# graphic-goose/ferreus_rbf_rs

Hardware: AMD Instinct MI355X
Metric: BBFMM matvecs/s (higher is better)
Workload: dtype f64; 1 GPU; 10000000 uniform 3D points, LinearRbf, order 7, 1 rhs, adaptive sparse tree, ACA eps=1e-7, set_weights + evaluate at the sources; points=10000000, kernel=LinearRbf, order=7, nrhs=1, parallelism=single GPU

## Files before the change

ferreus_rbf_rs_amd/_lib.py:

```python
from __future__ import annotations

import ctypes
import os

HERE = os.path.dirname(os.path.abspath(__file__))
LIB_PATH = os.environ.get("FERREUS_BBFMM_HIP_LIB") or os.path.join(HERE, "libferreus_bbfmm_hip.so")

OK, POINT_OUTSIDE_TREE, KERNEL_NO_GRADIENTS, BAD_ARGUMENT, DEVICE_ERROR, UNSUPPORTED, CALLBACK_FAILED = range(7)
FLAG_HOST_ONLY = 1
FLAG_M2L_SHARED_BASIS = 2
FLAG_DIRECT_SMALL_W_LEAVES = 4
FLAG_DETERMINISTIC = 8
N_PHASES = 11
PHASE_NAMES = ["gather", "P2M", "M2M", "M2L_stage1", "M2L_stage2", "P2L", "L2L", "P2P", "M2P",
               "L2P", "scatter"]

c_i32, c_i64, c_f64, c_u32 = ctypes.c_int32, ctypes.c_int64, ctypes.c_double, ctypes.c_uint32
c_p = ctypes.c_void_p


class Params(ctypes.Structure):
    _fields_ = [("max_points_per_cell", c_i64), ("compression_type", c_i32),
                ("epsilon", c_f64), ("eval_chunk_size", c_i64)]

# ... 69 lines not shown
    "bbfmm_isosurface_count": (c_i32, [c_p]),
    "bbfmm_isosurface_size": (ctypes.c_int, [c_p, c_i32, c_p, c_p]),
    "bbfmm_isosurface_copy": (ctypes.c_int, [c_p, c_i32, c_p, c_p]),
    "bbfmm_isosurface_error": (ctypes.c_char_p, [c_p]),
    "bbfmm_isosurface_destroy": (None, [c_p]),
    "bbfmm_prepare_target_subset": (ctypes.c_int, [c_p, c_p, c_i64]),
    "bbfmm_fast_matrix_vector_product": (ctypes.c_int, [c_p, c_p, c_i64, c_i64, c_p, c_i64, c_p,
                                                        c_i64, c_f64, c_p]),
    "bbfmm_matvec_device": (ctypes.c_int, [c_p, c_p, c_i64, c_i32, c_p, c_i64, c_i32]),
    "bbfmm_target_subset_create": (ctypes.c_int, [c_p, c_p, c_i64, c_p]),
    "bbfmm_matvec_subset_device": (ctypes.c_int, [c_p, c_i32, c_p, c_p, c_i32]),
    "bbfmm_stream": (c_p, [c_p]),
    "bbfmm_set_partition": (ctypes.c_int, [c_p, c_i32, c_i32]),
    "bbfmm_partition_row_count": (c_i64, [c_p]),
    "bbfmm_partition_rows": (ctypes.c_int, [c_p, c_p]),
    "bbfmm_partition_coarse_count": (c_i64, [c_p]),
    "bbfmm_matvec_partition_upward": (ctypes.c_int, [c_p, c_p, c_i64, c_i32, c_p, c_p]),
    "bbfmm_matvec_partition_finish": (ctypes.c_int, [c_p, c_p, c_p, c_i64, c_i32, c_p]),
    "bbfmm_partition_world": (c_i32, [c_p]),
    "bbfmm_partition_rank": (c_i32, [c_p]),
    "bbfmm_partition_bounds": (ctypes.c_int, [c_p, c_i32, c_p]),
    "bbfmm_matvec_partition_finish_sorted": (ctypes.c_int, [c_p, c_p, c_p, c_i64, c_p]),
    "bbfmm_partition_scatter": (ctypes.c_int, [c_p, c_p, c_i32, c_i32, c_i64, c_i32, c_p, c_i64]),
    "bbfmm_debug_partition_upward_counts": (ctypes.c_int, [c_p, c_p, c_p, c_p]),
    "bbfmm_debug_host_copy_rates": (ctypes.c_int, [c_i64, c_p]),
    "bbfmm_get_tree_stats": (ctypes.c_int, [c_p, c_p]),
    "bbfmm_tree_built_on_device": (ctypes.c_int, [c_p]),
    "bbfmm_last_evaluate_at_sources": (ctypes.c_int, [c_p]),
    "bbfmm_debug_targets_are_sources": (ctypes.c_int, [c_p, c_p, c_i64, c_i64]),
    "bbfmm_debug_rows_of_sources": (ctypes.c_int, [c_p, c_p, c_i64, c_i64, c_p]),
    "bbfmm_get_cells": (ctypes.c_int, [c_p, c_p, c_p]),
    "bbfmm_get_leaf_sources": (ctypes.c_int, [c_p, c_p, c_p]),
    "bbfmm_get_list": (ctypes.c_int, [c_p, ctypes.c_char, c_p, c_p, c_p]),
    "bbfmm_get_m2l_ranks": (ctypes.c_int, [c_p, c_p, c_p]),
    "bbfmm_get_m2l_operator": (ctypes.c_int, [c_p, c_i32, c_i32, c_p]),
    "bbfmm_get_m2l_factors": (ctypes.c_int, [c_p, c_i32, c_i32, c_p, c_p]),
    "bbfmm_get_permutation_tables": (ctypes.c_int, [c_p, c_p, c_p, c_p, c_p, c_p]),
    "bbfmm_points_to_leaves": (ctypes.c_int, [c_p, c_p, c_i64, c_i64, c_p, c_p]),
    "bbfmm_set_profiling": (ctypes.c_int, [c_p, c_i32]),
    "bbfmm_get_phase_ms": (ctypes.c_int, [c_p, c_p, c_p]),
    "bbfmm_reset_phase_ms": (ctypes.c_int, [c_p]),
    "bbfmm_mfma_f64_selftest": (ctypes.c_int, [c_p, c_p, c_p]),
    "bbfmm_fp64_valu_selftest": (ctypes.c_int, [c_p, c_p]),
    "bbfmm_debug_kernel_values": (ctypes.c_int, [c_i32, c_i32, ctypes.c_double, ctypes.c_double, c_p, c_i64, c_p, c_p, c_p]),
    "bbfmm_debug_math": (ctypes.c_int, [c_i32, c_i32, c_p, c_i64, c_p, c_p]),
    "bbfmm_debug_dense_m2m": (ctypes.c_int, [c_p, c_i32, c_p]),
    "bbfmm_debug_apply_m2l_tables_host": (ctypes.c_int, [c_p, c_p, c_p]),
    "bbfmm_debug_m2l_variants": (ctypes.c_int, [c_p, c_p, c_p]),
    "bbfmm_debug_m2l_pairs": (ctypes.c_int, [c_p, c_p, c_i64, c_p, c_p]),
    "bbfmm_debug_m2l_pairs_axes": (ctypes.c_int, [c_p, c_p, c_i64, c_p]),
    "bbfmm_debug_m2l_pairs_stage2": (ctypes.c_int, [c_p, c_p, c_i64, c_p, c_p]),
    "bbfmm_debug_m2l_pairs_axes_stage2": (ctypes.c_int, [c_p, c_p, c_i64, c_p]),
    "bbfmm_debug_m2l_s2_last_ksplit": (ctypes.c_int, [c_p, c_p]),
    "bbfmm_debug_get_coefficients": (ctypes.c_int, [c_p, ctypes.c_char, c_i32, c_p]),
    "bbfmm_debug_morton_encode": (ctypes.c_uint64, [c_i32, c_p, ctypes.c_uint64]),
    "bbfmm_debug_morton_decode": (None, [c_i32, ctypes.c_uint64, c_p, c_p]),
    "bbfmm_debug_morton_neighbours": (c_i32, [c_i32, ctypes.c_uint64, c_p]),
    "bbfmm_debug_direction_vectors": (c_i32, [c_i32, c_p]),
    "bbfmm_debug_reference_vectors": (ctypes.c_int, [c_p, c_p, c_p]),
    "bbfmm_givens_rotation": (None, [c_f64, c_f64, c_p, c_p, c_p]),
    "bbfmm_fgmres": (ctypes.c_int, [c_i64, c_p, c_p, c_p, c_p, c_p, c_p, c_i32, c_i32, c_i32, c_f64,
                                    c_p, c_p, c_p, c_p, c_p]),
    "bbfmm_schwarz_ddm_solver": (ctypes.c_int, [c_i64, c_p, c_p, c_p, c_p, c_p, c_i32, c_i32, c_f64,
                                                c_p, c_p, c_p, c_p, c_p]),
    "bbfmm_rbf_system_apply": (ctypes.c_int, [c_p, c_p, c_p, c_i64]),
    "bbfmm_ddm_params_defaults": (None, [c_p]),
    "bbfmm_ddm_params_for_points": (None, [c_i64, c_p]),
    "bbfmm_ddm_build": (ctypes.c_int, [c_p, c_i64, c_i32, c_i64, c_p, c_p]),
    "bbfmm_ddm_destroy": (None, [c_p]),
    "bbfmm_ddm_num_levels": (c_i32, [c_p]),
    "bbfmm_ddm_level_size": (c_i64, [c_p, c_i32]),
    "bbfmm_ddm_level_points": (ctypes.c_int, [c_p, c_i32, c_p]),
    "bbfmm_ddm_num_domains": (c_i64, [c_p, c_i32]),
    "bbfmm_ddm_domain_size": (c_i64, [c_p, c_i32, c_i64]),
    "bbfmm_ddm_domain": (ctypes.c_int, [c_p, c_i32, c_i64, c_p, c_p, c_p]),
    "bbfmm_schwarz_create": (ctypes.c_int, [c_p, c_p, c_i64, c_i32, c_i64, c_p, c_p, c_p]),
    "bbfmm_schwarz_create_sharded": (ctypes.c_int, [c_p, c_p, c_i64, c_i32, c_i64, c_p, c_p, c_i32, c_i32, c_p, c_i64, c_p, c_p, c_p]),
    "bbfmm_schwarz_factor_bytes": (c_i64, [c_p]),
    "bbfmm_schwarz_domains_owned": (c_i64, [c_p, c_i32, ctypes.POINTER(c_i64), ctypes.POINTER(c_i64)]),
    "bbfmm_schwarz_destroy": (None, [c_p]),
    "bbfmm_schwarz_basis_size": (c_i64, [c_p]),
    "bbfmm_schwarz_num_levels": (c_i32, [c_p]),
    "bbfmm_schwarz_monomial_matrix": (c_p, [c_p]),
    "bbfmm_debug_evaluate_monomials": (ctypes.c_int, [c_p, c_i64, c_i32, c_i64, c_i32, c_p, c_p, c_p]),
    "bbfmm_schwarz_apply": (ctypes.c_int, [c_p, c_p, c_p, c_i64]),
    "bbfmm_schwarz_level_size": (c_i64, [c_p, c_i32]),
    "bbfmm_schwarz_level_points": (ctypes.c_int, [c_p, c_i32, c_p]),
    "bbfmm_schwarz_debug_level_solve": (ctypes.c_int, [c_p, c_i32, c_p, c_p, c_i64, c_i32]),
    "bbfmm_ddm_debug_level_create": (ctypes.c_int, [c_p, c_i64, c_i32, c_i64, c_i64, c_p, c_p, c_p, c_p, c_i32, c_i32, c_p]),
    "bbfmm_ddm_debug_level_destroy": (None, [c_p]),
    "bbfmm_ddm_debug_level_info": (ctypes.c_int, [c_p, c_p]),
    "bbfmm_ddm_debug_level_layout": (ctypes.c_int, [c_p, c_p, c_p, c_p, c_p, c_p]),
    "bbfmm_ddm_debug_level_assembled": (ctypes.c_int, [c_p, c_p]),
    "bbfmm_ddm_debug_level_factor": (ctypes.c_int, [c_p, c_p]),
    "bbfmm_ddm_debug_level_solve": (ctypes.c_int, [c_p, c_p, c_p, c_i64, c_i32]),
    "bbfmm_schwarz_create_ex": (ctypes.c_int, [c_p, c_p, c_i64, c_i32, c_i64, c_p, c_i64, c_p, c_p, c_p]),
    "bbfmm_schwarz_create_sharded_ex": (ctypes.c_int, [c_p, c_p, c_i64, c_i32, c_i64, c_p, c_i64, c_p, c_p, c_i32, c_i32, c_p, c_i64,
                                                       c_p, c_p, c_p]),
    "bbfmm_ddm_debug_level_create_ex": (ctypes.c_int, [c_p, c_i64, c_i32, c_i64, c_p, c_i64, c_i64, c_p, c_p, c_p, c_p, c_i32, c_i32,
                                                       c_p]),
    "bbfmm_global_trend_transform": (ctypes.c_int, [c_i32, c_p, c_p, c_p, c_p]),
    "bbfmm_duplicate_cutoff_distance": (ctypes.c_int, [c_p, c_f64, c_p]),
    "bbfmm_remove_duplicates": (ctypes.c_int, [c_p, c_i64, c_i32, c_i64, c_f64, c_i32, c_p, c_p, c_p]),
    "bbfmm_debug_interpolant_terms": (ctypes.c_int, [c_i32, c_i32, c_p, c_p, c_i64, c_i64, c_p, c_i64, c_p, c_i64, c_p, c_i64]),
    "bbfmm_evaluate_interpolant": (ctypes.c_int, [c_p, c_i32, c_i32, c_p, c_i64, c_i32, c_i64, c_p, c_i64, c_i64, c_p, c_f64,
                                                  c_p, c_i64, c_p, c_i64, c_p]),
# ... 75 lines not shown
```

ferreus_rbf_rs_amd/build.py:

```python
from __future__ import annotations

import hashlib
import os
import subprocess
import sys

HERE = os.path.dirname(os.path.abspath(__file__))
ROOT = os.path.dirname(HERE)
CSRC = os.path.join(HERE, "csrc")
OBJ = os.path.join(HERE, "_obj")
LIB = os.path.join(HERE, "libferreus_bbfmm_hip.so")

HOST_SOURCES = ["tree.cpp", "operators.cpp", "fmm_tree.cpp", "fmm_m2l_tables.cpp", "fmm_plans.cpp", "device_group.cpp", "capi.cpp", "solver.cpp", "ddm.cpp", "ddm_solver.cpp", "schwarz.cpp", "interpolant.cpp", "closure_triangulate.cpp"]
HIP_SOURCES = ["device_l2p.hip", "device_p2p.hip", "device_wx.hip", "device_p2m.hip", "device_m2l.hip", "device_transfer.hip", "device_gather.hip", "device_selftest.hip",
               "ddm_kernels.hip", "targets.hip", "schwarz_kernels.hip", "tree_device.hip", "tree_lists_device.hip", "isosurface.hip", "isosurface_finish.hip", "isosurface_closure.hip", "isosurface_intersect.hip", "isosurface_follow.hip", "interpolant_terms.hip", "field_program.hip"]
HEADERS = ["morton.hpp", "tree.hpp", "parallel.hpp", "kernels.hpp", "operators.hpp", "device.hpp", "device_common.hpp", "device_direct.hpp",
           "fmm_tree.hpp", "fmm_tree_impl.hpp", "device_group.hpp", "targets.hpp", "ddm.hpp", "ddm_solver.hpp", "ddm_monomials.hpp", "schwarz_kernels.hpp", "tree_device.hpp", "isosurface.hpp", "isosurface_curvature.hpp", "isosurface_intersect.hpp", "isosurface_closure.hpp", "closure_triangulate.hpp", "interpolant_terms.hpp", "field_program.hpp", os.path.join(ROOT, "include", "ferreus_bbfmm_hip.h")]


def _digest(paths: list[str], extra: str = "") -> str:
    h = hashlib.sha256(extra.encode())
    for p in paths:
        with open(p, "rb") as f:
            h.update(os.path.basename(p).encode() + b"\0" + f.read())
    return h.hexdigest()


def _file_digest(path: str) -> str:
    h = hashlib.sha256()
    with open(path, "rb") as f:
        for chunk in iter(lambda: f.read(1 << 20), b""):
            h.update(chunk)
    return h.hexdigest()


def _stale(target: str, stamp: str, digest: str) -> bool:
    if not os.path.exists(target) or not os.path.exists(stamp):
        return True
    with open(stamp) as f:
        want = f.read().split()
    return len(want) != 2 or want[0] != digest or want[1] != _file_digest(target)


def _write_stamp(target: str, stamp: str, digest: str) -> None:
    with open(stamp, "w") as f:
        f.write(digest + " " + _file_digest(target))


_COMPILER_ID = None


def _compiler_id(hipcc: str) -> str:
    global _COMPILER_ID
    if _COMPILER_ID is None:
        try:
            _COMPILER_ID = subprocess.run([hipcc, "--version"], stdout=subprocess.PIPE, stderr=subprocess.STDOUT,
                                          timeout=120).stdout.decode(errors="replace")
        except (OSError, subprocess.SubprocessError):
            _COMPILER_ID = "unknown"
    return _COMPILER_ID


SANITIZERS = {
    "asan": ["-fsanitize=address,undefined", "-fno-sanitize-recover=undefined"],
    "tsan": ["-fsanitize=thread"],
}


def sanitized_lib(kind: str) -> str:
# ... 81 lines not shown
```

ferreus_rbf_rs_amd/csrc/capi.cpp:

```cpp
#include <cmath>
#include <cstddef>
#include <cstring>
#include <new>
#include <string>
#include <vector>

#include <algorithm>
#include <chrono>
#include <cstdlib>
#include <memory>

#include "device_group.hpp"
#include "ferreus_bbfmm_hip.h"
#include "fmm_tree.hpp"
#include "interpolant_terms.hpp"
#include "field_program.hpp"
#include "closure_triangulate.hpp"
#include "isosurface.hpp"
#include "isosurface_closure.hpp"
#include "isosurface_curvature.hpp"
#include "isosurface_intersect.hpp"
#include "morton.hpp"

struct bbfmm_handle {
// ... 1935 lines not shown
int bbfmm_debug_m2l_variants(const bbfmm_handle *h, int64_t *n_variants, int64_t *n_cells) {
    if (!h) return BBFMM_BAD_ARGUMENT;
    int64_t nv = 0, nc = 0;
    h->tree.m2l_variant_stats(&nv, &nc);
    if (n_variants) *n_variants = nv;
    if (n_cells) *n_cells = nc;
    return BBFMM_OK;
}

int bbfmm_debug_m2l_pairs(const bbfmm_handle *h, int32_t *out, int64_t cap, int64_t *n_out, int32_t *pairs_on) {
    if (!h || !n_out) return BBFMM_BAD_ARGUMENT;
    std::vector<int32_t> v;
    h->tree.debug_m2l_pairs(&v);
    *n_out = static_cast<int64_t>(v.size());
    if (pairs_on) *pairs_on = h->tree.m2l_pairs() ? 1 : 0;
    if (out) std::copy(v.begin(), v.begin() + std::min<int64_t>(cap, *n_out), out);
    return BBFMM_OK;
}

int bbfmm_debug_m2l_pairs_axes(const bbfmm_handle *h, int32_t *out, int64_t cap, int64_t *n_out) {
    if (!h || !n_out) return BBFMM_BAD_ARGUMENT;
    std::vector<int32_t> v;
    h->tree.debug_m2l_pairs_axes(&v);
    *n_out = static_cast<int64_t>(v.size());
    if (out) std::copy(v.begin(), v.begin() + std::min<int64_t>(cap, *n_out), out);
    return BBFMM_OK;
}

int bbfmm_debug_m2l_pairs_stage2(const bbfmm_handle *h, int32_t *out, int64_t cap, int64_t *n_out, int32_t *pairs_on) {
    if (!h || !n_out) return BBFMM_BAD_ARGUMENT;
    std::vector<int32_t> v;
    h->tree.debug_m2l_pairs_stage2(&v);
    *n_out = static_cast<int64_t>(v.size());
    if (pairs_on) *pairs_on = h->tree.m2l_pairs_stage2() ? 1 : 0;
    if (out) std::copy(v.begin(), v.begin() + std::min<int64_t>(cap, *n_out), out);
    return BBFMM_OK;
}

int bbfmm_debug_m2l_pairs_axes_stage2(const bbfmm_handle *h, int32_t *out, int64_t cap, int64_t *n_out) {
    if (!h || !n_out) return BBFMM_BAD_ARGUMENT;
    std::vector<int32_t> v;
    h->tree.debug_m2l_pairs_axes_stage2(&v);
    *n_out = static_cast<int64_t>(v.size());
    if (out) std::copy(v.begin(), v.begin() + std::min<int64_t>(cap, *n_out), out);
    return BBFMM_OK;
}

int bbfmm_debug_m2l_s2_last_ksplit(const bbfmm_handle *h, int32_t *ksplit) {
    if (!h || !ksplit) return BBFMM_BAD_ARGUMENT;
    *ksplit = h->tree.debug_m2l_s2_last_ksplit();
    return BBFMM_OK;
}

int bbfmm_debug_get_coefficients(bbfmm_handle *h, char which, int32_t k, double *out) {
    GUARD(h) return h->tree.debug_get_coefficients(which, k, out);
    END_GUARD(h)
}

}

#include "ddm.hpp"
struct bbfmm_ddm {
    bbfmm::DdmTree tree;
};
extern "C" {
void bbfmm_ddm_params_defaults(bbfmm_ddm_params *out) {
    if (!out) return;
    const bbfmm::DdmParams p;
    out->leaf_threshold = p.leaf_threshold;
    out->overlap_quota = p.overlap_quota;
    out->coarse_ratio = p.coarse_ratio;
    out->coarse_threshold = p.coarse_threshold;
}

void bbfmm_ddm_params_for_points(int64_t n, bbfmm_ddm_params *out) {
    if (!out) return;
    bbfmm_ddm_params_defaults(out);
    out->coarse_threshold = std::max<int64_t>(out->coarse_threshold, n / 470 + 1);
}
int bbfmm_ddm_build(const double *points, int64_t n, int32_t d, int64_t ld, const bbfmm_ddm_params *params,
                    bbfmm_ddm **out) {
    if (!out) return BBFMM_BAD_ARGUMENT;
    *out = nullptr;
    bbfmm::DdmParams p;
    if (params) {
        p.leaf_threshold = params->leaf_threshold;
        p.overlap_quota = params->overlap_quota;
        p.coarse_ratio = params->coarse_ratio;
        p.coarse_threshold = params->coarse_threshold;
    }
    bbfmm_ddm *t = new (std::nothrow) bbfmm_ddm();
    if (!t) return BBFMM_DEVICE_ERROR;
    int rc = BBFMM_BAD_ARGUMENT;
    try {
        rc = bbfmm::build_ddm_tree(points, n, d, ld, p, &t->tree);
    } catch (...) {
        rc = BBFMM_DEVICE_ERROR;
    }
    if (rc != BBFMM_OK) {
        delete t;
        return rc;
    }
    *out = t;
    return BBFMM_OK;
}
void bbfmm_ddm_destroy(bbfmm_ddm *t) { delete t; }
// ... 37 lines not shown
```

ferreus_rbf_rs_amd/csrc/device.hpp:

```cpp
#pragma once
#include <hip/hip_runtime.h>

#include <cstdint>

#include "kernels.hpp"

namespace bbfmm {

constexpr int kMaxOrder = 16;
constexpr int kM2lTile = 128;
constexpr int kM2lS1Block = 176;
constexpr int kM2lS1BlockPairs = 160;
constexpr int kM2lSlotWindow = 128;
constexpr int kM2lBlkTwoDst = 1 << 30;

struct DevCheb {
    int p, d, n, n_pad;
    double polyn[kMaxOrder * kMaxOrder];
    double nodes[kMaxOrder];
    double xfer[2 * kMaxOrder * kMaxOrder];
};

struct ChebRef {
    const DevCheb *dev;
    int p, d, n, n_pad;
};

struct M2lClass {
    const double *vt_all;
    const int32_t *row_dst;
    const int32_t *row_dst2;
    const int32_t *blk_t0;
    int32_t yb0;
    int32_t n_rows;
    int32_t r_pad16;
    int32_t n_t;
    const double *u_all;
    int32_t k_pad;
    int32_t kp;
    int32_t kpy;
    const int32_t *cells;
    int32_t n_cells;
    const int32_t *cslot;
    const int64_t *cbase;
};

struct M2lTileDesc {
    int32_t level_class;
    int32_t first;
    int32_t count;
    int32_t q_first;
    int32_t q_count;
    int32_t pad;
};

void launch_gather_weights(const double *w, int64_t ldw, int K, const int32_t *order, int64_t N,
                           double *w_sorted, hipStream_t s);
void launch_gather_weights_subset(const double *w, int64_t ldw, int K, const int32_t *order, const int32_t *pos, int64_t n_pos,
                                  int64_t N, double *w_sorted, hipStream_t s);
constexpr int kMaxScatterParts = 64;
struct ScatterParts {
    int n;
    int64_t bound[kMaxScatterParts + 1];
};
void launch_scatter_parts(const double *all, const ScatterParts &parts, int64_t m_max, int K, const int32_t *order, double *out,
                          int64_t ldo, hipStream_t s);
void launch_sum_slots(const double *slots, int n_slots, int64_t len, double *out, hipStream_t s);
void launch_scatter_output(const double *out_sorted, int64_t n, int K, const int32_t *perm,
                           double *out, int64_t ldo, int accumulate, hipStream_t s);
void launch_gather_rows(const double *src, int64_t ld_src, int ncols, const int32_t *idx, int64_t n,
                        double *dst, int64_t ld_dst, hipStream_t s);

void launch_p2m(const ChebRef &ch, const double *const *src_xyz, const double *w_sorted, int64_t N,
                int K, int64_t C, const int32_t *leaf_cells, int n_leaves, const int32_t *pt_begin,
                const int32_t *pt_end, const double *centers, const double *lengths, double *M,
                hipStream_t s);
int launch_m2m(const ChebRef &ch, int K, int64_t C, const int32_t *parents, int n_parents,
               const int64_t *child_ptr, const int32_t *child_idx, const int32_t *octant, double *M,
               hipStream_t s);
int launch_l2l(const ChebRef &ch, int K, int64_t C, const int32_t *cells, int n_cells,
               const int32_t *parent, const int32_t *octant, const uint8_t *active, double *L,
               hipStream_t s);

void launch_m2l_stage1(const M2lClass *classes, const M2lTileDesc *tiles, const int32_t *tile_idx, int n_tiles,
                       int n_pad, int max_slot_t, int K, int64_t C, const double *M, double *cbuf,
                       int64_t cbuf_len, hipStream_t s, bool own_blocks = false, int max_blocks = 8, int ne16 = 0, int s_ee = 0,
                       int s_eo = 0);
void launch_m2l_parity(const double *M, int n_pad, double *Mp, int n_par, int ne16, int n_e, int n_o, int p, int64_t rows,
                       hipStream_t s);
struct M2lParityOffsets {
    int32_t v[4];
};
void launch_m2l_parity2(const double *M, int n_pad, double *Mp, int n_par, M2lParityOffsets off, int p, int p2, int64_t rows,
                        hipStream_t s);
void launch_m2l_stage2(const M2lClass *classes, const M2lTileDesc *tiles, const int32_t *tile_idx, int n_tiles,
                       int n_pad, int K, int64_t C, const double *cbuf, int64_t cbuf_len,
                       const uint16_t *qlist, double *L, hipStream_t s, bool allow_ksplit = true);
struct M2lS2PairsPlan {
    int ga, gb, ce, co;
    int ya = 0, yb = 0;
    int ne16() const { return 16 * ga * ce; }
    __host__ __device__ int n_par() const { return 16 * (ga * ce + gb * co); }
    __host__ __device__ int col(int part, int j) const {
        const int g = part < 2 ? ga : gb, y = part < 2 ? ya : yb, w = 16 * ((part & 1) ? g - y : y);
        const int jj = j % w, gl = ((part & 1) ? y : 0) + jj / 16, pp = jj % 16, paired = g / 2 * 2;
        const int local = gl < paired ? 32 * (gl / 2) + 2 * pp + (gl & 1) : 16 * paired + pp;
        return (part < 2 ? 0 : 16 * ga * ce) + (j / w) * 16 * g + local;
    }
};
M2lS2PairsPlan m2l_s2_pairs_plan(int groups_even, int groups_odd);
M2lS2PairsPlan m2l_s2_pairs_plan2(const int groups[4]);
bool launch_m2l_stage2_pairs(const M2lClass *classes, const M2lTileDesc *tiles, const int32_t *tile_idx, int n_tiles,
                             const M2lS2PairsPlan &plan, int K, int64_t C, const double *cbuf, int64_t cbuf_len,
                             const uint16_t *qlist, double *Lp, hipStream_t s, bool allow_ksplit = true, int *ksplit_out = nullptr);
void launch_m2l_unparity(const double *Lp, int n_par, int ne16, double *L, int n, int n_pad, int n_e, int n_o, int p, int64_t rows,
                         hipStream_t s);
void launch_m2l_unparity2(const double *Lp, const M2lS2PairsPlan &plan, double *L, int n, int n_pad, int p, int p2, int64_t rows,
                          hipStream_t s);
void launch_m2l_zero_segments(const int32_t *segs, int64_t n_segs, int K, double *cbuf, int64_t cbuf_len, hipStream_t s);
void launch_m2l_basis(const M2lClass *classes, const M2lTileDesc *tiles, int n_tiles, int in_ld, int out_ld, int K,
                      int64_t C, const double *in, double *out, hipStream_t s);
void launch_small_gemm(bool trans_a, int M, int N, int Kd, const double *A, int64_t lda, const double *B, int64_t ldb,
                       double *Cm, int64_t ldc, hipStream_t s);

struct M2lAssembleTv {
    int32_t perm;
    int32_t rank;
    int32_t row;
    int64_t vt_off;
    int64_t u_off;
};
struct M2lAssembleClass {
    const M2lAssembleTv *src, *tgt;
    int32_t n_src, n_tgt, r_pad16, k_pad, max_rank;
    int32_t n_e, n_o, ne16, n_par, p;
    int32_t u_npar, u_ne16, u_rows, u_ne, u_no;
    int32_t s1_axes;
    M2lParityOffsets s1_off;
    M2lS2PairsPlan u_plan;
};
void launch_m2l_assemble(const M2lAssembleClass &c, int n, int n_pad, bool compressed, const double *ops,
                         const int32_t *invperm, double *vt_all, double *u_all, hipStream_t s);

struct DirectJobs {
    int n_jobs;
    const int32_t *job_cell;
    const int32_t *tgt_begin, *tgt_end;
    const int64_t *run_ptr;
    const int32_t *runs;
};
void launch_p2p(const KernelSpec &ks, int d, const DirectJobs &jobs, const double *const *tgt_xyz,
                int64_t n_tgt, const double *const *src_xyz, const double *w_sorted, int64_t N, int K,
                double *out_sorted, double *grad_sorted, hipStream_t s, bool fixed_plan = false);
constexpr int kSymMaxRhs = 4;
void launch_p2p_sym(const KernelSpec &ks, int n_jobs, const int32_t *tgt_begin, const int32_t *tgt_end,
                    const int64_t *run_range, int n_leaf_jobs, const int32_t *l_tgt_begin, const int32_t *l_tgt_end,
                    const int64_t *l_run_range, int n_wave_jobs, const int32_t *w_tgt_begin, const int32_t *w_tgt_end,
                    const int64_t *w_run_range, const int32_t *runs3, int32_t tgt_off, const double *const *src_xyz,
                    const double *w_sorted, int64_t ldw, int K, double *out_sorted, int64_t ldo, hipStream_t s);
int p2p_sym_rows_per_job();
int p2p_sym3_rows_per_job();
int p2p_sym_wave_rows();
int64_t p2p_sym_wave_min_jobs();
int wx_sym_rows_per_job();
int wx_sym3_rows_per_job();
void launch_wx_sym(const KernelSpec &ks, const ChebRef &ch, int n_jobs, const int32_t *tgt_begin, const int32_t *tgt_end,
                   const int64_t *w_range, int n_leaf_jobs, const int32_t *l_tgt_begin, const int32_t *l_tgt_end,
                   const int64_t *l_w_range, const int32_t *w_cells, const double *centers, const double *lengths,
                   const double *const *src_xyz, const double *w_sorted, int64_t ldw, int K, const double *M, double *L,
                   int64_t ld_ml, double *out_sorted, int64_t ldo, int out_off, int out_n, hipStream_t s);
void launch_m2p(const KernelSpec &ks, const ChebRef &ch, int n_jobs, const int32_t *tgt_begin,
                const int32_t *tgt_end, const int64_t *w_begin, const int64_t *w_end,
                const int32_t *w_cells,
                const double *centers, const double *lengths, const double *const *tgt_xyz,
                int64_t n_tgt, int K, int64_t C, const double *M, double *out_sorted,
                double *grad_sorted, hipStream_t s, bool fixed_plan = false);
void launch_p2l(const KernelSpec &ks, const ChebRef &ch, int n_jobs, const int32_t *cells,
                const int64_t *run_ptr, const int32_t *runs, const double *centers,
                const double *lengths, const double *const *src_xyz, const double *w_sorted,
                int64_t N, int K, int64_t C, double *L, hipStream_t s);
void launch_l2p(const ChebRef &ch, int n_jobs, const int32_t *leaf_cells, const int32_t *tgt_begin,
                const int32_t *tgt_end, const double *centers, const double *lengths,
                const double *const *tgt_xyz, int64_t n_tgt, int K, int64_t C, const double *L,
                double *out_sorted, double *grad_sorted, hipStream_t s);

bool l2p_order_supported(int p, int d);

int mfma_f64_selftest(double *tflops, int *layout_errors, double *info);
int valu_f64_selftest(double *tflops, double *mhz);
int debug_kernel_values_device(const KernelSpec &ks, const double *r2, int64_t n, double *value, double *value_g, double *factor);
int debug_math_device(int which, const double *x, int64_t n, double *out, double *out2);

}
```

ferreus_rbf_rs_amd/csrc/device_l2p.hip:

```cpp
#include "device_common.hpp"

namespace bbfmm {

constexpr int L2P_WAVES = 4;
template <int P, int D> constexpr int l2p_waves() { return D == 3 && P > 12 ? (P > 14 ? 1 : 2) : L2P_WAVES; }

template <int P, int D, bool GRAD>
__global__ __launch_bounds__((64 * l2p_waves<P, D>())) void l2p_kernel(const DevCheb *__restrict__ chp, int n_jobs,
                                                             const int32_t *__restrict__ leaf_cells,
                                                             const int32_t *__restrict__ tgt_begin,
                                                             const int32_t *__restrict__ tgt_end,
                                                             const double *__restrict__ centers,
                                                             const double *__restrict__ lengths, Xyz tgt,
                                                             int64_t n_tgt, int K, int64_t C,
                                                             const double *__restrict__ L,
                                                             double *__restrict__ out, double *__restrict__ grad) {
    constexpr int P1 = D > 1 ? P : 1, P2 = D > 2 ? P : 1, N = P * P1 * P2;
    constexpr int WAVES = l2p_waves<P, D>();
    __shared__ double s_L[WAVES][N];
    const int tid = threadIdx.x, wave = tid >> 6, lane = tid & 63;
    __shared__ double s_polyn_lds[GRAD ? P * P : 1];
    if constexpr (GRAD) {
        for (int i = tid; i < P * P; i += 64 * WAVES) s_polyn_lds[i] = chp->polyn[i];
        __syncthreads();
    }
    const double *__restrict__ s_polyn = GRAD ? s_polyn_lds : chp->polyn;
    const int job = blockIdx.x * WAVES + wave;
    if (job >= n_jobs) return;
    const int n_pad = chp->n_pad;
    const int cell = leaf_cells[job];
    const int b = tgt_begin[job], e = tgt_end[job];
    const double len = lengths[cell];
    const double cc[3] = {centers[cell * 3 + 0], centers[cell * 3 + 1], centers[cell * 3 + 2]};
    double *Lw = s_L[wave];
    for (int base = b; base < e; base += 64) {
        const int t = base + lane;
        const bool valid = t < e;
        double S0[P], S1[P1], S2[P2], D0[P], D1[P1], D2[P2];
        {
            const double x0 = valid ? (tgt.x[t] - cc[0]) / (len * 0.5) : 0.0;
            cheb_S_reg<P, GRAD>(x0, s_polyn, S0, D0);
            if (D > 1) {
                const double x1 = valid ? (tgt.y[t] - cc[1]) / (len * 0.5) : 0.0;
                double s[P], d[P];
                cheb_S_reg<P, GRAD>(x1, s_polyn, s, d);
#pragma unroll
                for (int j = 0; j < P1; ++j) { S1[j] = s[j]; D1[j] = d[j]; }
            } else {
                S1[0] = 1.0;
                D1[0] = 0.0;
            }
            if (D > 2) {
                const double x2 = valid ? (tgt.z[t] - cc[2]) / (len * 0.5) : 0.0;
                double s[P], d[P];
                cheb_S_reg<P, GRAD>(x2, s_polyn, s, d);
#pragma unroll
                for (int j = 0; j < P2; ++j) { S2[j] = s[j]; D2[j] = d[j]; }
            } else {
                S2[0] = 1.0;
                D2[0] = 0.0;
            }
        }
        const double gs = 2.0 / len;
        for (int k = 0; k < K; ++k) {
            const double *Lc = L + ((int64_t)k * C + cell) * n_pad;
            for (int I = lane; I < N; I += 64) Lw[I] = Lc[I];
            __builtin_amdgcn_s_waitcnt(0xc07f);
            double y = 0.0, gx = 0.0, gy = 0.0, gz = 0.0;
#pragma unroll
            for (int a = 0; a < P; ++a) {
                double ua = 0.0, uay = 0.0, uaz = 0.0;
#pragma unroll
                for (int bb = 0; bb < P1; ++bb) {
                    double t0 = 0.0, t0z = 0.0;
#pragma unroll
                    for (int c = 0; c < P2; ++c) {
                        const double lv = Lw[(a * P1 + bb) * P2 + c];
                        t0 += S2[c] * lv;
                        if (GRAD) t0z += D2[c] * lv;
                    }
                    ua += S1[bb] * t0;
                    if (GRAD) {
                        uay += D1[bb] * t0;
                        uaz += S1[bb] * t0z;
                    }
                }
                y += S0[a] * ua;
                if (GRAD) {
                    gx += D0[a] * ua;
                    gy += S0[a] * uay;
                    gz += S0[a] * uaz;
                }
            }
            if (valid) {
                out[(int64_t)k * n_tgt + t] += y;
                if (GRAD) {
                    grad[((int64_t)k * D + 0) * n_tgt + t] += gx * gs;
                    if (D > 1) grad[((int64_t)k * D + 1) * n_tgt + t] += gy * gs;
                    if (D > 2) grad[((int64_t)k * D + 2) * n_tgt + t] += gz * gs;
                }
            }
        }
    }
}

template <int P, int D>
static void l2p_launch_pd(const ChebRef &ch, int n_jobs, const int32_t *leaf_cells, const int32_t *tgt_begin,
                          const int32_t *tgt_end, const double *centers, const double *lengths, Xyz tgt,
                          int64_t n_tgt, int K, int64_t C, const double *L, double *out_sorted, double *grad_sorted,
                          hipStream_t s) {
    constexpr int WAVES = l2p_waves<P, D>();
    const int blocks = (n_jobs + WAVES - 1) / WAVES;
    if (grad_sorted)
        hipLaunchKernelGGL((l2p_kernel<P, D, true>), dim3(blocks), dim3(64 * WAVES), 0, s, ch.dev, n_jobs,
                           leaf_cells, tgt_begin, tgt_end, centers, lengths, tgt, n_tgt, K, C, L, out_sorted,
                           grad_sorted);
    else
        hipLaunchKernelGGL((l2p_kernel<P, D, false>), dim3(blocks), dim3(64 * WAVES), 0, s, ch.dev, n_jobs,
                           leaf_cells, tgt_begin, tgt_end, centers, lengths, tgt, n_tgt, K, C, L, out_sorted,
                           grad_sorted);
}

template <int P>
static void l2p_launch_p(const ChebRef &ch, int n_jobs, const int32_t *leaf_cells, const int32_t *tgt_begin,
                         const int32_t *tgt_end, const double *centers, const double *lengths, Xyz tgt, int64_t n_tgt,
                         int K, int64_t C, const double *L, double *out_sorted, double *grad_sorted, hipStream_t s) {
    if (ch.d == 3) {
        l2p_launch_pd<P, 3>(ch, n_jobs, leaf_cells, tgt_begin, tgt_end, centers, lengths, tgt, n_tgt, K, C, L, out_sorted, grad_sorted, s);
    } else if (ch.d == 2) {
        l2p_launch_pd<P, 2>(ch, n_jobs, leaf_cells, tgt_begin, tgt_end, centers, lengths, tgt, n_tgt, K, C, L, out_sorted, grad_sorted, s);
    } else {
        l2p_launch_pd<P, 1>(ch, n_jobs, leaf_cells, tgt_begin, tgt_end, centers, lengths, tgt, n_tgt, K, C, L, out_sorted, grad_sorted, s);
    }
}

bool l2p_order_supported(int p, int d) { return p >= 2 && p <= kMaxOrder && d >= 1 && d <= 3; }

void launch_l2p(const ChebRef &ch, int n_jobs, const int32_t *leaf_cells, const int32_t *tgt_begin,
                const int32_t *tgt_end, const double *centers, const double *lengths, const double *const *tgt_xyz,
                int64_t n_tgt, int K, int64_t C, const double *L, double *out_sorted, double *grad_sorted,
                hipStream_t s) {
    if (n_jobs == 0) return;
    const Xyz tgt = make_xyz(tgt_xyz);
    dispatch_order<2, 16>(ch.p, [&](auto pc) {
        l2p_launch_p<decltype(pc)::value>(ch, n_jobs, leaf_cells, tgt_begin, tgt_end, centers, lengths, tgt, n_tgt, K, C, L,
                                          out_sorted, grad_sorted, s);
    });
}

}
```

ferreus_rbf_rs_amd/csrc/device_m2l.hip:

```cpp
#include "device_common.hpp"

#include <cmath>

namespace bbfmm {

typedef __attribute__((address_space(3))) void *lptr_t;

__device__ inline unsigned lds_offset(const double *p) {
    return static_cast<unsigned>(reinterpret_cast<uintptr_t>((lptr_t)p));
}
__device__ inline unsigned uniform_u32(unsigned v) { return __builtin_amdgcn_readfirstlane(v); }
__device__ inline const double *uniform_ptr(const double *p) {
    const uintptr_t v = reinterpret_cast<uintptr_t>(p);
    const unsigned lo = __builtin_amdgcn_readfirstlane(static_cast<unsigned>(v));
    const unsigned hi = __builtin_amdgcn_readfirstlane(static_cast<unsigned>(v >> 32));
    return reinterpret_cast<const double *>((static_cast<uintptr_t>(hi) << 32) | lo);
}
__device__ inline void dma16(const double *g, unsigned lds_wave_byte_offset) {
    asm volatile("s_mov_b32 m0, %1\n\ts_nop 0\n\tglobal_load_lds_dwordx4 %0, off" ::"v"(g),
                 "s"(uniform_u32(lds_wave_byte_offset))
                 : "memory");
}
__device__ inline void dma4(const int32_t *g, unsigned lds_wave_byte_offset) {
    asm volatile("s_mov_b32 m0, %1\n\ts_nop 0\n\tglobal_load_lds_dword %0, off" ::"v"(g),
                 "s"(uniform_u32(lds_wave_byte_offset))
                 : "memory");
}
__device__ inline void wait_dma_and_barrier() {
    asm volatile("s_waitcnt vmcnt(0)" ::: "memory");
    __syncthreads();
}
template <int N> __device__ inline void wait_dma_keep_stores_and_barrier() {
    asm volatile("s_waitcnt vmcnt(%0)" ::"n"(N < 63 ? N : 63) : "memory");
    __syncthreads();
}
template <int N> __device__ inline double add_row_ror(double v) {
    const int lo = __double2loint(v), hi = __double2hiint(v);
    const int rlo = __builtin_amdgcn_update_dpp(0, lo, 0x120 + N, 0xf, 0xf, false);
    const int rhi = __builtin_amdgcn_update_dpp(0, hi, 0x120 + N, 0xf, 0xf, false);
    return v + __hiloint2double(rhi, rlo);
}

__device__ inline void dma16s(const double *sbase, unsigned voff_bytes, unsigned lds_wave_byte_offset) {
    asm volatile("s_mov_b32 m0, %2\n\ts_nop 0\n\tglobal_load_lds_dwordx4 %0, %1" ::"v"(voff_bytes),
                 "s"(uniform_ptr(sbase)), "s"(uniform_u32(lds_wave_byte_offset))
                 : "memory");
}

template <int NG16, int STAGE, int MINW, bool PAIRS = false>
__global__ __launch_bounds__(512, MINW) void m2l_gemm_k4(const M2lClass *__restrict__ classes,
                                                  const M2lTileDesc *__restrict__ tiles, int n_pad, int g16_0,
                                                  int64_t C, const double *__restrict__ in, int64_t in_len,
                                                  double *__restrict__ out, int64_t out_len,
// ... 623 lines not shown
        const int ce = std::max(1, (groups_even + w[0] - 1) / w[0]), co = std::max(1, (groups_odd + w[1] - 1) / w[1]);
        const int cost = ce * (w[0] + 2) + co * (w[1] + 2);
        if (cost < best_cost) {
            best_cost = cost;
            best = M2lS2PairsPlan{w[0], w[1], ce, co};
        }
    }
    return best;
}

#define M2L_S2_PAIR2_WIDTHS(X) X(13, 7, 10, 6) X(14, 8, 11, 6) X(8, 4, 8, 4) X(5, 3, 4, 2) X(4, 2, 4, 2) X(2, 1, 2, 1)
#define M2L_S2_WIDTH2_ENTRY(A, YA, B, YB) {A, YA, B, YB},
static constexpr int kM2lS2Pair2Widths[][4] = {M2L_S2_PAIR2_WIDTHS(M2L_S2_WIDTH2_ENTRY)};
#undef M2L_S2_WIDTH2_ENTRY

M2lS2PairsPlan m2l_s2_pairs_plan2(const int groups[4]) {
    M2lS2PairsPlan best{2, 2, 1, 1, 1, 1};
    int best_cost = 1 << 30;
    auto chunks = [](int n, int w) { return std::max(1, (n + w - 1) / w); };
    for (const auto &w : kM2lS2Pair2Widths) {
        const int ce = std::max(chunks(groups[0], w[1]), chunks(groups[1], w[0] - w[1]));
        const int co = std::max(chunks(groups[2], w[3]), chunks(groups[3], w[2] - w[3]));
        const int cost = ce * (w[0] + 2) + co * (w[2] + 2);
        if (cost < best_cost) {
            best_cost = cost;
            best = M2lS2PairsPlan{w[0], w[2], ce, co, w[1], w[3]};
        }
    }
    return best;
}

template <int GA, int YA, int GB, int YB>
static void m2l_s2_pairs2_launch(const M2lClass *classes, const M2lTileDesc *tiles, const int32_t *tile_idx, int n_tiles,
                                 const M2lS2PairsPlan &plan, int ksplit, int K, int64_t C, const double *cbuf, int64_t cbuf_len,
                                 const uint16_t *qlist, double *Lp, hipStream_t s) {
    const size_t lds = 2 * sizeof(double) * (size_t)(2 * (GA > GB ? GA : GB) * 128 + 4096);
    static std::atomic<uint64_t> attr_set[4] = {{0}, {0}, {0}, {0}};
    (void)allow_large_dynamic_lds(reinterpret_cast<const void *>(&m2l_s2_pairs2_kernel<GA, YA, GB, YB>), lds, attr_set);
    hipLaunchKernelGGL((m2l_s2_pairs2_kernel<GA, YA, GB, YB>), dim3(n_tiles, K, (plan.ce + plan.co) * ksplit), dim3(512), lds, s, classes,
                       tiles, plan.n_par(), plan.ce, plan.co, ksplit, C, cbuf, cbuf_len, Lp, qlist, tile_idx);
}

template <int GA, int GB>
static void m2l_s2_pairs_launch(const M2lClass *classes, const M2lTileDesc *tiles, const int32_t *tile_idx, int n_tiles,
                                const M2lS2PairsPlan &plan, int ksplit, int K, int64_t C, const double *cbuf, int64_t cbuf_len,
                                const uint16_t *qlist, double *Lp, hipStream_t s) {
    const size_t lds = 2 * sizeof(double) * (size_t)(2 * (GA > GB ? GA : GB) * 128 + 4096);
    static std::atomic<uint64_t> attr_set[4] = {{0}, {0}, {0}, {0}};
    (void)allow_large_dynamic_lds(reinterpret_cast<const void *>(&m2l_s2_pairs_kernel<GA, GB>), lds, attr_set);
    hipLaunchKernelGGL((m2l_s2_pairs_kernel<GA, GB>), dim3(n_tiles, K, (plan.ce + plan.co) * ksplit), dim3(512), lds, s, classes, tiles,
                       plan.n_par(), plan.ce, plan.co, ksplit, C, cbuf, cbuf_len, Lp, qlist, tile_idx);
}

bool launch_m2l_stage2_pairs(const M2lClass *classes, const M2lTileDesc *tiles, const int32_t *tile_idx, int n_tiles,
                             const M2lS2PairsPlan &plan, int K, int64_t C, const double *cbuf, int64_t cbuf_len,
                             const uint16_t *qlist, double *Lp, hipStream_t s, bool allow_ksplit, int *ksplit_out) {
    if (n_tiles == 0) return true;
    const int ksplit = m2l_s2_ksplit(static_cast<int64_t>(n_tiles) * (plan.ce + plan.co) * K, allow_ksplit);
    if (ksplit_out) *ksplit_out = ksplit;
    if (plan.ya > 0) {
#define M2L_S2_DISPATCH2(A, YA, B, YB)                                                                                   \
    if (plan.ga == A && plan.ya == YA && plan.gb == B && plan.yb == YB) {                                                \
        m2l_s2_pairs2_launch<A, YA, B, YB>(classes, tiles, tile_idx, n_tiles, plan, ksplit, K, C, cbuf, cbuf_len, qlist, \
                                           Lp, s);                                                                       \
        return true;                                                                                                     \
    }
        M2L_S2_PAIR2_WIDTHS(M2L_S2_DISPATCH2)
#undef M2L_S2_DISPATCH2
        return false;
    }
#define M2L_S2_DISPATCH(A, B)                                                                                           \
    if (plan.ga == A && plan.gb == B) {                                                                                  \
        m2l_s2_pairs_launch<A, B>(classes, tiles, tile_idx, n_tiles, plan, ksplit, K, C, cbuf, cbuf_len, qlist, Lp, s);  \
        return true;                                                                                                     \
    }
    M2L_S2_PAIR_WIDTHS(M2L_S2_DISPATCH)
#undef M2L_S2_DISPATCH
    return false;
}

__global__ __launch_bounds__(256) void m2l_unparity_kernel(const double *__restrict__ Lp, int n_par, int ne16, double *__restrict__ L,
                                                           int n, int n_pad, int n_e, int n_o, int p, int p1, int64_t rows) {
    const int64_t row = static_cast<int64_t>(blockIdx.x) * 4 + (threadIdx.x >> 6);
    if (row >= rows) return;
    const double *src = Lp + row * n_par;
    double *dst = L + row * n_pad;
    for (int j = threadIdx.x & 63; j < n_e; j += 64) {
        const double e = src[j];
        if (j < n_o) {
            const double o = src[ne16 + j];
            dst[j] = e + o;
            dst[j + (p - 1 - 2 * (j / p1)) * p1] = e - o;
        } else {
            dst[j] = e;
        }
    }
    for (int j = n + (threadIdx.x & 63); j < n_pad; j += 64) dst[j] = 0.0;
}

void launch_m2l_unparity(const double *Lp, int n_par, int ne16, double *L, int n, int n_pad, int n_e, int n_o, int p, int64_t rows,
                         hipStream_t s) {
    if (rows <= 0) return;
    const int p1 = n_e / ((p + 1) / 2);
    hipLaunchKernelGGL(m2l_unparity_kernel, dim3(static_cast<unsigned>((rows + 3) / 4)), dim3(256), 0, s, Lp, n_par, ne16, L, n, n_pad, n_e,
                       n_o, p, p1, rows);
}

__global__ __launch_bounds__(256) void m2l_unparity2_kernel(const double *__restrict__ Lp, M2lS2PairsPlan plan, double *__restrict__ L,
                                                            int n, int n_pad, int p, int p2, int64_t rows) {
    const int64_t row = static_cast<int64_t>(blockIdx.x) * 4 + (threadIdx.x >> 6);
    if (row >= rows) return;
    const int n_par = plan.n_par();
    const double *src = Lp + row * n_par;
    double *dst = L + row * n_pad;
    const int h = (p + 1) / 2, f = p / 2;
    for (int e = threadIdx.x & 63; e < h * h * p2; e += 64) {
        const int i0 = e / (h * p2), i1 = (e - i0 * h * p2) / p2, r = e - (i0 * h + i1) * p2;
        const int m = (i0 * p + i1) * p2 + r;
        const int dx = (p - 1 - 2 * i0) * p * p2, dy = (p - 1 - 2 * i1) * p2;
        const bool cx = i0 >= f, cy = i1 >= f;
        const int je = (i0 * h + i1) * p2 + r, jo = (i0 * f + i1) * p2 + r;
        const double ee = src[plan.col(0, je)];
        const double eo = cy ? 0.0 : src[plan.col(1, jo)];
        const double oe = cx ? 0.0 : src[plan.col(2, je)];
        const double oo = cx || cy ? 0.0 : src[plan.col(3, jo)];
        const double a = cy ? ee : ee + eo, b = ee - eo, c = cy ? oe : oe + oo, d = oe - oo;
        dst[m] = cx ? a : a + c;
        if (!cx) dst[m + dx] = a - c;
        if (!cy) dst[m + dy] = cx ? b : b + d;
        if (!cx && !cy) dst[m + dx + dy] = b - d;
    }
    for (int j = n + (threadIdx.x & 63); j < n_pad; j += 64) dst[j] = 0.0;
}

void launch_m2l_unparity2(const double *Lp, const M2lS2PairsPlan &plan, double *L, int n, int n_pad, int p, int p2, int64_t rows,
                          hipStream_t s) {
    if (rows <= 0) return;
    hipLaunchKernelGGL(m2l_unparity2_kernel, dim3(static_cast<unsigned>((rows + 3) / 4)), dim3(256), 0, s, Lp, plan, L, n, n_pad, p, p2,
                       rows);
}

__global__ __launch_bounds__(256) void m2l_parity_kernel(const double *__restrict__ M, int n_pad, double *__restrict__ Mp, int n_par,
                                                         int ne16, int n_e, int n_o, int p, int p1, int64_t rows) {
    const int64_t row = static_cast<int64_t>(blockIdx.x) * 4 + (threadIdx.x >> 6);
    if (row >= rows) return;
    const double *src = M + row * n_pad;
    double *dst = Mp + row * n_par;
    for (int j = threadIdx.x & 63; j < n_e; j += 64) {
        const double v = src[j];
        if (j < n_o) {
            const double w = src[j + (p - 1 - 2 * (j / p1)) * p1];
            dst[j] = v + w;
            dst[ne16 + j] = v - w;
        } else {
            dst[j] = v;
        }
    }
}

void launch_m2l_parity(const double *M, int n_pad, double *Mp, int n_par, int ne16, int n_e, int n_o, int p, int64_t rows,
                       hipStream_t s) {
    if (rows <= 0) return;
    const int p1 = n_e / ((p + 1) / 2);
    hipLaunchKernelGGL(m2l_parity_kernel, dim3(static_cast<unsigned>((rows + 3) / 4)), dim3(256), 0, s, M, n_pad, Mp, n_par, ne16, n_e,
                       n_o, p, p1, rows);
}

__global__ __launch_bounds__(256) void m2l_parity2_kernel(const double *__restrict__ M, int n_pad, double *__restrict__ Mp, int n_par,
                                                          M2lParityOffsets off, int p, int p2, int64_t rows) {
    const int64_t row = static_cast<int64_t>(blockIdx.x) * 4 + (threadIdx.x >> 6);
    if (row >= rows) return;
    const double *src = M + row * n_pad;
    double *dst = Mp + row * n_par;
    const int h = (p + 1) / 2, f = p / 2;
    for (int e = threadIdx.x & 63; e < h * h * p2; e += 64) {
        const int i0 = e / (h * p2), i1 = (e - i0 * h * p2) / p2, r = e - (i0 * h + i1) * p2;
        const int m = (i0 * p + i1) * p2 + r;
        const int dx = (p - 1 - 2 * i0) * p * p2, dy = (p - 1 - 2 * i1) * p2;
        const bool cx = i0 >= f, cy = i1 >= f;
        const double v = src[m], vx = src[m + dx], vy = src[m + dy], vxy = src[m + dx + dy];
        const double e0 = cx ? v : v + vx, e1 = cx ? vy : vy + vxy, o0 = v - vx, o1 = vy - vxy;
        const int je = (i0 * h + i1) * p2 + r, jo = (i0 * f + i1) * p2 + r;
        dst[off.v[0] + je] = cy ? e0 : e0 + e1;
        if (!cy) dst[off.v[1] + jo] = e0 - e1;
        if (!cx) dst[off.v[2] + je] = cy ? o0 : o0 + o1;
        if (!cx && !cy) dst[off.v[3] + jo] = o0 - o1;
    }
}

void launch_m2l_parity2(const double *M, int n_pad, double *Mp, int n_par, M2lParityOffsets off, int p, int p2, int64_t rows,
                        hipStream_t s) {
    if (rows <= 0) return;
    hipLaunchKernelGGL(m2l_parity2_kernel, dim3(static_cast<unsigned>((rows + 3) / 4)), dim3(256), 0, s, M, n_pad, Mp, n_par, off, p, p2,
                       rows);
}

__global__ __launch_bounds__(256) void m2l_zero_segments_kernel(const int32_t *__restrict__ segs, int64_t n_segs,
                                                                double *__restrict__ cbuf, int64_t cbuf_len) {
    const int64_t sg = (static_cast<int64_t>(blockIdx.x) * 256 + threadIdx.x) >> 4;
    const int l = threadIdx.x & 15;
    if (sg >= n_segs) return;
    const int2 e = reinterpret_cast<const int2 *>(segs)[sg];
    double2 *dst = reinterpret_cast<double2 *>(cbuf + static_cast<int64_t>(blockIdx.y) * cbuf_len) + e.x;
    for (int i = l; i < e.y; i += 16) dst[i] = make_double2(0.0, 0.0);
}

void launch_m2l_zero_segments(const int32_t *segs, int64_t n_segs, int K, double *cbuf, int64_t cbuf_len, hipStream_t s) {
    if (n_segs <= 0) return;
    hipLaunchKernelGGL(m2l_zero_segments_kernel, dim3(static_cast<unsigned>((n_segs * 16 + 255) / 256), K), dim3(256), 0, s, segs,
                       n_segs, cbuf, cbuf_len);
}

void launch_m2l_basis(const M2lClass *classes, const M2lTileDesc *tiles, int n_tiles, int in_ld, int out_ld, int K,
                      int64_t C, const double *in, double *out, hipStream_t s) {
    if (n_tiles == 0) return;
    m2l_dispatch_chunks<3>(out_ld / 16, classes, tiles, n_tiles, out_ld, 2, K, C, in, in_ld, out, 0, nullptr, 0, nullptr, s);
}

template <bool TA>
__global__ __launch_bounds__(256) void small_gemm_kernel(int M, int N, int Kd, const double *__restrict__ A, int64_t lda,
                                                         const double *__restrict__ B, int64_t ldb, double *__restrict__ Cm,
                                                         int64_t ldc) {
    __shared__ double sa[16][64 + 1], sb[16][64 + 1];
    const int tx = threadIdx.x & 15, ty = threadIdx.x >> 4;
    const int i0 = blockIdx.y * 64, j0 = blockIdx.x * 64;
    double acc[4][4] = {};
    for (int k0 = 0; k0 < Kd; k0 += 16) {
        for (int e = threadIdx.x; e < 16 * 64; e += 256) {
            const int kk = TA ? e >> 6 : e & 15, ii = TA ? e & 63 : e >> 4;
            const int k = k0 + kk, i = i0 + ii;
            sa[kk][ii] = (k < Kd && i < M) ? (TA ? A[(int64_t)k * lda + i] : A[(int64_t)i * lda + k]) : 0.0;
        }
        for (int e = threadIdx.x; e < 16 * 64; e += 256) {
            const int kk = e >> 6, jj = e & 63;
            const int k = k0 + kk, j = j0 + jj;
            sb[kk][jj] = (k < Kd && j < N) ? B[(int64_t)k * ldb + j] : 0.0;
        }
        __syncthreads();
#pragma unroll
        for (int kk = 0; kk < 16; ++kk) {
            double a[4], b[4];
#pragma unroll
            for (int r = 0; r < 4; ++r) a[r] = sa[kk][ty + 16 * r];
#pragma unroll
            for (int c = 0; c < 4; ++c) b[c] = sb[kk][tx + 16 * c];
#pragma unroll
            for (int r = 0; r < 4; ++r)
// ... 177 lines not shown
```

ferreus_rbf_rs_amd/csrc/device_transfer.hip:

```cpp
#include "device_common.hpp"

namespace bbfmm {

template <bool FORWARD>
__device__ inline void transfer_pass(const double *in, double *out, const double *xf, int axis, int p, int P0, int P1,
                                     int P2, int n, int tid, int nthreads) {
    const int stride = axis == 0 ? P1 * P2 : (axis == 1 ? P2 : 1);
    for (int I = tid; I < n; I += nthreads) {
        const int ia = (I / stride) % p;
        const int base = I - ia * stride;
        double s = 0.0;
        for (int a = 0; a < p; ++a) {
            const double f = FORWARD ? xf[a * p + ia] : xf[ia * p + a];
            s += f * in[base + a * stride];
        }
        out[I] = s;
    }
}

__global__ __launch_bounds__(256) void m2m_kernel(const DevCheb *__restrict__ chp, int K, int64_t C,
                                                  const int32_t *__restrict__ parents,
                                                  const int64_t *__restrict__ child_ptr,
                                                  const int32_t *__restrict__ child_idx,
                                                  const int32_t *__restrict__ octant, double *__restrict__ M) {
    extern __shared__ double lds[];
    const int p = chp->p, d = chp->d, n = chp->n, n_pad = chp->n_pad;
    int P0, P1, P2;
    axis_sizes(p, d, P0, P1, P2);
    double *bufA = lds, *bufB = lds + n, *acc = lds + 2 * n, *xf = lds + 3 * n;
    const int tid = threadIdx.x;
    for (int i = tid; i < 2 * p * p; i += 256) xf[i] = chp->xfer[i];
    const int P = parents[blockIdx.x];
    const int64_t c0 = child_ptr[P], c1 = child_ptr[P + 1];
    for (int k = 0; k < K; ++k) {
        for (int I = tid; I < n; I += 256) acc[I] = 0.0;
        for (int64_t q = c0; q < c1; ++q) {
            const int ch = child_idx[q];
            const int oct = octant[ch];
            const double *Mc = M + ((int64_t)k * C + ch) * n_pad;
            __syncthreads();
            for (int I = tid; I < n; I += 256) bufA[I] = Mc[I];
            __syncthreads();
            double *in = bufA, *out = bufB;
            for (int axis = d - 1; axis >= 0; --axis) {
                const double *x1 = xf + ((oct >> axis) & 1) * p * p;
                transfer_pass<true>(in, out, x1, axis, p, P0, P1, P2, n, tid, 256);
                __syncthreads();
                double *t = in;
                in = out;
                out = t;
            }
            for (int I = tid; I < n; I += 256) acc[I] += in[I];
        }
// ... 5 lines not shown
}

__global__ __launch_bounds__(256) void l2l_kernel(const DevCheb *__restrict__ chp, int K, int64_t C,
                                                  const int32_t *__restrict__ cells,
                                                  const int32_t *__restrict__ parent,
                                                  const int32_t *__restrict__ octant,
                                                  const uint8_t *__restrict__ active, double *__restrict__ L) {
    extern __shared__ double lds[];
    const int p = chp->p, d = chp->d, n = chp->n, n_pad = chp->n_pad;
    int P0, P1, P2;
    axis_sizes(p, d, P0, P1, P2);
    double *bufA = lds, *bufB = lds + n, *xf = lds + 2 * n;
    const int tid = threadIdx.x;
    const int c = cells[blockIdx.x];
    if (active && !active[c]) return;
    const int P = parent[c];
    if (P < 0) return;
    for (int i = tid; i < 2 * p * p; i += 256) xf[i] = chp->xfer[i];
    const int oct = octant[c];
    for (int k = 0; k < K; ++k) {
        const double *Lp = L + ((int64_t)k * C + P) * n_pad;
        __syncthreads();
        for (int I = tid; I < n; I += 256) bufA[I] = Lp[I];
        __syncthreads();
        double *in = bufA, *out = bufB;
        for (int axis = 0; axis < d; ++axis) {
            const double *x1 = xf + ((oct >> axis) & 1) * p * p;
            transfer_pass<false>(in, out, x1, axis, p, P0, P1, P2, n, tid, 256);
            __syncthreads();
            double *t = in;
            in = out;
            out = t;
        }
        double *Lc = L + ((int64_t)k * C + c) * n_pad;
        for (int I = tid; I < n; I += 256) Lc[I] += in[I];
    }
}

template <int P, bool FORWARD>
__device__ inline void pencil_apply(double (&v)[P], const double *__restrict__ xf) {
    double o[P];
#pragma unroll
    for (int j = 0; j < P; ++j) {
        double s = 0.0;
#pragma unroll
        for (int k = 0; k < P; ++k) s += (FORWARD ? xf[k * P + j] : xf[j * P + k]) * v[k];
        o[j] = s;
    }
#pragma unroll
    for (int j = 0; j < P; ++j) v[j] = o[j];
}

template <int P, bool FORWARD>
__device__ inline void transfer3_wave(const double *__restrict__ in, double *buf, const double *__restrict__ xfer,
                                      int oct, int lane) {
    constexpr int PP = P * P, NPEN = (PP + 63) / 64;
    const double *x0 = xfer + ((oct >> 0) & 1) * PP, *x1 = xfer + ((oct >> 1) & 1) * PP,
                 *x2 = xfer + ((oct >> 2) & 1) * PP;
#pragma unroll
    for (int ps = 0; ps < NPEN; ++ps) {
        const int q = lane + 64 * ps;
        if (q < PP) {
            double v[P];
#pragma unroll
            for (int i = 0; i < P; ++i) v[i] = in[i * PP + q];
            pencil_apply<P, FORWARD>(v, x0);
#pragma unroll
            for (int i = 0; i < P; ++i) buf[i * PP + q] = v[i];
        }
    }
    __builtin_amdgcn_wave_barrier();
#pragma unroll
    for (int ps = 0; ps < NPEN; ++ps) {
        const int r = lane + 64 * ps;
        if (r < PP) {
            const int i0 = r / P, i2 = r - i0 * P;
            double v[P];
#pragma unroll
            for (int i = 0; i < P; ++i) v[i] = buf[i0 * PP + i * P + i2];
            pencil_apply<P, FORWARD>(v, x1);
#pragma unroll
            for (int i = 0; i < P; ++i) buf[i0 * PP + i * P + i2] = v[i];
        }
    }
    __builtin_amdgcn_wave_barrier();
#pragma unroll
    for (int ps = 0; ps < NPEN; ++ps) {
        const int sidx = lane + 64 * ps;
        if (sidx < PP) {
            double v[P];
#pragma unroll
            for (int i = 0; i < P; ++i) v[i] = buf[sidx * P + i];
            pencil_apply<P, FORWARD>(v, x2);
#pragma unroll
            for (int i = 0; i < P; ++i) buf[sidx * P + i] = v[i];
        }
    }
    __builtin_amdgcn_wave_barrier();
}

constexpr int XFER_WAVES = 4;

template <int P>
__global__ __launch_bounds__(64 * XFER_WAVES) void l2l3_kernel(const DevCheb *__restrict__ chp, int K, int64_t C,
                                                               const int32_t *__restrict__ cells, int n_cells,
                                                               const int32_t *__restrict__ parent,
                                                               const int32_t *__restrict__ octant,
                                                               const uint8_t *__restrict__ active,
                                                               double *__restrict__ L) {
    constexpr int N = P * P * P;
    __shared__ double s_buf[XFER_WAVES][N];
    const int wave = threadIdx.x >> 6, lane = threadIdx.x & 63;
    const int job = blockIdx.x * XFER_WAVES + wave;
    if (job >= n_cells) return;
    const int c = __builtin_amdgcn_readfirstlane(cells[job]);
    if (active && !active[c]) return;
    const int Pc = __builtin_amdgcn_readfirstlane(parent[c]);
    if (Pc < 0) return;
    const int oct = __builtin_amdgcn_readfirstlane(octant[c]);
    const int n_pad = chp->n_pad;
    for (int k = 0; k < K; ++k) {
        transfer3_wave<P, false>(L + ((int64_t)k * C + Pc) * n_pad, s_buf[wave], chp->xfer, oct, lane);
        double *Lc = L + ((int64_t)k * C + c) * n_pad;
        for (int I = lane; I < N; I += 64) Lc[I] += s_buf[wave][I];
        __builtin_amdgcn_wave_barrier();
    }
}

template <int P>
__global__ __launch_bounds__(512) void m2m3_kernel(const DevCheb *__restrict__ chp, int K, int64_t C,
                                                   const int32_t *__restrict__ parents,
                                                   const int64_t *__restrict__ child_ptr,
                                                   const int32_t *__restrict__ child_idx,
                                                   const int32_t *__restrict__ octant, double *__restrict__ M) {
    constexpr int N = P * P * P;
    __shared__ double s_buf[8][N];
    const int wave = threadIdx.x >> 6, lane = threadIdx.x & 63;
    const int Pc = parents[blockIdx.x];
    const int64_t c0 = child_ptr[Pc];
    const int n_ch = (int)(child_ptr[Pc + 1] - c0);
    const int n_pad = chp->n_pad;
    for (int k = 0; k < K; ++k) {
        if (wave < n_ch) {
            const int ch = __builtin_amdgcn_readfirstlane(child_idx[c0 + wave]);
            const int oct = __builtin_amdgcn_readfirstlane(octant[ch]);
            transfer3_wave<P, true>(M + ((int64_t)k * C + ch) * n_pad, s_buf[wave], chp->xfer, oct, lane);
        }
        __syncthreads();
        double *Mp = M + ((int64_t)k * C + Pc) * n_pad;
        for (int I = threadIdx.x; I < N; I += 512) {
            double s = 0.0;
            for (int w = 0; w < n_ch; ++w) s += s_buf[w][I];
            Mp[I] = s;
        }
        __syncthreads();
    }
}

int launch_m2m(const ChebRef &ch, int K, int64_t C, const int32_t *parents, int n_parents, const int64_t *child_ptr,
               const int32_t *child_idx, const int32_t *octant, double *M, hipStream_t s) {
    if (n_parents == 0) return 0;
    if (ch.d == 3 && dispatch_order<2, 10>(ch.p, [&](auto pc) {
            hipLaunchKernelGGL((m2m3_kernel<decltype(pc)::value>), dim3(n_parents), dim3(512), 0, s, ch.dev, K, C, parents, child_ptr,
                               child_idx, octant, M);
        }))
        return 0;
    const size_t lds = sizeof(double) * (3 * (size_t)ch.n + 2 * ch.p * ch.p);
    static std::atomic<uint64_t> attr_set[4] = {{0}, {0}, {0}, {0}};
    if (const hipError_t e = allow_large_dynamic_lds(reinterpret_cast<const void *>(&m2m_kernel), lds, attr_set)) return static_cast<int>(e);
    hipLaunchKernelGGL(m2m_kernel, dim3(n_parents), dim3(256), lds, s, ch.dev, K, C, parents, child_ptr, child_idx,
                       octant, M);
    return 0;
}

int launch_l2l(const ChebRef &ch, int K, int64_t C, const int32_t *cells, int n_cells, const int32_t *parent,
               const int32_t *octant, const uint8_t *active, double *L, hipStream_t s) {
    if (n_cells == 0) return 0;
    if (ch.d == 3 && dispatch_order<2, 12>(ch.p, [&](auto pc) {
            hipLaunchKernelGGL((l2l3_kernel<decltype(pc)::value>), dim3((n_cells + XFER_WAVES - 1) / XFER_WAVES), dim3(64 * XFER_WAVES),
                               0, s, ch.dev, K, C, cells, n_cells, parent, octant, active, L);
        }))
        return 0;
    const size_t lds = sizeof(double) * (2 * (size_t)ch.n + 2 * ch.p * ch.p);
    static std::atomic<uint64_t> attr_set[4] = {{0}, {0}, {0}, {0}};
    if (const hipError_t e = allow_large_dynamic_lds(reinterpret_cast<const void *>(&l2l_kernel), lds, attr_set)) return static_cast<int>(e);
    hipLaunchKernelGGL(l2l_kernel, dim3(n_cells), dim3(256), lds, s, ch.dev, K, C, cells, parent, octant, active, L);
    return 0;
}

}
```

ferreus_rbf_rs_amd/csrc/fmm_tree.cpp:

```cpp
#include "fmm_tree_impl.hpp"

namespace bbfmm {

int FmmTree::fail(int code, const std::string &msg) {
    err_ = msg;
    return code;
}
int FmmTree::hip_fail(hipError_t e, const char *what) {
    err_ = std::string("HIP error: ") + hipGetErrorString(e) + " in " + what;
    return BBFMM_DEVICE_ERROR;
}

void FmmTree::arena_begin() {
    arena_active_ = true;
    arena_used_ = 0;
    arena_need_ = 0;
}
int FmmTree::arena_end() {
    arena_active_ = false;
    if (arena_need_ > arena_.n) {
        dfree(&arena_);
        CHK(dalloc(&arena_, arena_need_ + arena_need_ / 4));
    }
    return BBFMM_OK;
// ... 496 lines not shown
                HIPCHK(hipMemcpy(ua.p, hu.data(), hu.size() * sizeof(double), hipMemcpyHostToDevice));
            } else {
                launch_m2l_assemble(ac, ops_.n, cheb_.n_pad, compressed, d_level_ops[h.level].p, d_invperm.p, vt.p, ua.p, stream_);
            }
            assemble_tmp.push_back(d_src);
            assemble_tmp.push_back(d_tgt);
            if (shared_basis_) {
                DevBuf<double> vt2, ua2;
                CHK(dalloc(&vt2, static_cast<size_t>(m2l_len) * h.r_pad16));
                CHK(dalloc(&ua2, static_cast<size_t>(h.k_pad) * m2l_len));
                const double *W = d_basis_c_[static_cast<size_t>(h.level)].p;
                launch_small_gemm(true, m2l_len, h.r_pad16, cheb_.n_pad, W, m2l_len, vt.p, h.r_pad16, vt2.p, h.r_pad16, stream_);
                launch_small_gemm(false, h.k_pad, m2l_len, cheb_.n_pad, ua.p, cheb_.n_pad, W, m2l_len, ua2.p, m2l_len, stream_);
                natural_tmp.push_back(vt);
                natural_tmp.push_back(ua);
                vt = vt2;
                ua = ua2;
            }
        }
        CHK(dupload(&rt, h.row_dst));
        CHK(dupload(&rt2, h.row_dst2));
        CHK(dupload(&ro, h.blk_t0));
        CHK(dupload(&ce, h.cells));
        CHK(dalloc(&cs, h.cslot.size()));
        if (!h.cslot.empty()) HIPCHK(hipMemcpy(cs.p, h.cslot.data(), h.cslot.size() * sizeof(int32_t), hipMemcpyHostToDevice));
        CHK(dupload(&cb, h.cbase));
        c.vt_all = vt.p;
        c.u_all = ua.p;
        c.row_dst = rt.p;
        c.row_dst2 = rt2.p;
        c.blk_t0 = ro.p;
        c.cells = ce.p;
        c.cslot = cs.p;
        c.cbase = cb.p;
        decltype(h.cslot)().swap(h.cslot);
    }
    HIPCHK(hipStreamSynchronize(stream_));
    HIPCHK(hipGetLastError());
    for (auto &b : assemble_tmp) dfree(&b);
    for (auto &b : natural_tmp) dfree(&b);
    for (auto &b : d_level_ops) dfree(&b);
    dfree(&d_invperm);
    ut.lap("  upload: M2L operators, tables");
    CHK(dupload(&d_m2l_classes_, m2l_classes_h_));
    CHK(dupload(&d_m2l_tiles_, m2l_tiles_h_));
    CHK(dupload(&d_m2l_tiles1_, m2l_tiles1_h_));
    CHK(dupload(&d_tile_idx1_, m2l_tile_idx1_h_));
    CHK(dupload(&d_m2l_tiles2_, m2l_tiles2_h_));
    CHK(dupload(&d_m2l_zero_, m2l_zero_h_));
    decltype(m2l_zero_h_)().swap(m2l_zero_h_);
    CHK(dupload(&d_m2l_qlist_, m2l_qlist_h_));
    std::vector<uint8_t> act(static_cast<size_t>(C), 1);
    CHK(dupload(&d_active_, act));
    return BBFMM_OK;
}

int FmmTree::ensure_rhs_capacity(int k) {
    if (k <= k_cap_) return BBFMM_OK;
    const int64_t N = tree_.n_points, C = tree_.n_cells();
    pin_w_k_ = 0;
    dfree(&d_w_sorted_);
    dfree(&d_M_);
    dfree(&d_L_);
    dfree(&d_cbuf_);
    dfree(&d_out_);
    dfree(&src_targets_.out);
    dfree(&src_targets_.grad);
    const size_t coef = static_cast<size_t>(k) * C * cheb_.n_pad;
    CHK(dalloc(&d_w_sorted_, static_cast<size_t>(k) * N));
    CHK(dalloc(&d_M_, coef, true));
    CHK(dalloc(&d_L_, coef, true));
    if (m2l_pairs_) {
        dfree(&d_Mp_);
        CHK(dalloc(&d_Mp_, static_cast<size_t>(k) * C * m2l_npar_, true));
    }
    if (shared_basis_) {
        dfree(&d_Mc_);
        dfree(&d_Lc_);
        CHK(dalloc(&d_Mc_, static_cast<size_t>(k) * C * basis_pad_, true));
        CHK(dalloc(&d_Lc_, static_cast<size_t>(k) * C * basis_pad_, true));
    }
    m2l_rhs_chunk_ = static_cast<int>(std::max<int64_t>(1, std::min<int64_t>(k, m2l_budget_bytes_ / 8 / std::max<int64_t>(cbuf_batch_len_, 1))));
    CHK(dalloc(&d_cbuf_, static_cast<size_t>(m2l_rhs_chunk_) * std::max<int64_t>(cbuf_batch_len_, 1), true));
    if (m2l_pairs2_) {
        dfree(&d_Lp_);
        CHK(dalloc(&d_Lp_, static_cast<size_t>(m2l_rhs_chunk_) * C * m2l_s2_plan_.n_par(), true));
    }
    CHK(dalloc(&d_out_, static_cast<size_t>(k) * N));
    CHK(dalloc(&src_targets_.out, static_cast<size_t>(k) * N));
    k_cap_ = k;
    return BBFMM_OK;
}

int FmmTree::upload_weights(const double *w, int64_t rows, int k, int64_t ldw) {
    const int64_t N = tree_.n_points;
    if (!w || rows < N || ldw < rows || k < 1) return fail(BBFMM_BAD_ARGUMENT, "weights must be rows x k with rows >= N");
    pin_w_k_ = 0;
    CHK(ensure_rhs_capacity(k));
    if (static_cast<size_t>(k) * N > d_w_in_.n) {
        dfree(&d_w_in_);
        CHK(dalloc(&d_w_in_, static_cast<size_t>(k) * N));
    }
    HIPCHK(hipMemcpy2DAsync(d_w_in_.p, N * sizeof(double), w, ldw * sizeof(double), N * sizeof(double), k,
                            hipMemcpyHostToDevice, stream_));
    phase_begin();
    launch_gather_weights(d_w_in_.p, N, k, d_order_.p, N, d_w_sorted_.p, stream_);
    phase_end(kPhGather);
    return BBFMM_OK;
}

int FmmTree::ensure_pinned(size_t n) {
    if (n <= h_pin_n_) return BBFMM_OK;
    if (h_pin_) (void)hipHostFree(h_pin_);
    h_pin_ = nullptr;
    h_pin_n_ = 0;
    pin_w_k_ = 0;
    HIPCHK(hipHostMalloc(reinterpret_cast<void **>(&h_pin_), n * sizeof(double), hipHostMallocPortable));
    h_pin_n_ = n;
    return BBFMM_OK;
}

int FmmTree::stage_weights_to_device(const double *w, int64_t n, int k, int64_t ldw) {
    pin_w_k_ = 0;
    CHK(ensure_pinned(static_cast<size_t>(2) * k * n));
    if (static_cast<size_t>(k) * n > d_w_in_.n) {
        dfree(&d_w_in_);
        CHK(dalloc(&d_w_in_, static_cast<size_t>(k) * n));
// ... 134 lines not shown
            }
        });
    }
    rows->resize(static_cast<size_t>(m));
    int64_t *out = rows->data();
    const int32_t *tab = src_row_table_.data();
    const double *p = pts_.data();
    std::atomic<bool> all{true};
    parallel_for_chunks(m, int64_t(1) << 14, [&](int64_t b, int64_t e) {
        for (int64_t j = b; j < e; ++j) {
            if (!all.load(std::memory_order_relaxed)) return;
            uint64_t s = point_hash(x, ldx, j) & src_row_mask_;
            int64_t found = -1;
            for (;;) {
                const int32_t cur = tab[s];
                if (cur == -1) break;
                bool same = true;
                for (int a = 0; a < d_ && same; ++a)
                    same = std::memcmp(x + static_cast<size_t>(a) * ldx + j, p + static_cast<size_t>(a) * N + cur, sizeof(double)) == 0;
                if (same) {
                    found = cur;
                    break;
                }
                s = (s + 1) & src_row_mask_;
            }
            if (found < 0) {
                all.store(false, std::memory_order_relaxed);
                return;
            }
            out[j] = found;
        }
    });
    return all.load();
}

bool FmmTree::targets_are_sources(const double *x, int64_t m, int64_t ldx) const {
    const int64_t N = tree_.n_points;
    if (!x || m != N || ldx < m || pts_.size() != static_cast<size_t>(N) * d_) return false;
    std::atomic<bool> same{true};
    for (int a = 0; a < d_ && same.load(std::memory_order_relaxed); ++a) {
        const double *xa = x + static_cast<size_t>(a) * ldx, *pa = &pts_[static_cast<size_t>(a) * N];
        parallel_for_chunks(N, kHostPiece, [&](int64_t lo, int64_t hi) {
            if (same.load(std::memory_order_relaxed) && std::memcmp(xa + lo, pa + lo, static_cast<size_t>(hi - lo) * sizeof(double)) != 0)
                same.store(false, std::memory_order_relaxed);
        });
    }
    return same.load();
}

int FmmTree::upward(int k, const DownwardPlan *dp) {
    const HostTree &t = tree_;
    const int64_t C = t.n_cells();
    const bool part = dp && dp->restrict_upward;
    multipoles_partial_ = part;
    phase_begin();
    if (part) {
        for (int j = 0; j < k && dp->coarse_cells > 0; ++j)
            HIPCHK(hipMemsetAsync(d_M_.p + static_cast<size_t>(j) * C * cheb_.n_pad, 0,
                                  static_cast<size_t>(dp->coarse_cells) * cheb_.n_pad * sizeof(double), stream_));
        launch_p2m(cheb_, src_ptr_, d_w_sorted_.p, t.n_points, k, C, dp->d_up_leaves.p, static_cast<int>(dp->up_leaves_h.size()),
                   d_pt_begin_.p, d_pt_end_.p, d_centers_.p, d_lengths_.p, d_M_.p, stream_);
    } else {
        launch_p2m(cheb_, src_ptr_, d_w_sorted_.p, t.n_points, k, C, d_src_leaves_.p, static_cast<int>(src_leaves_.size()),
                   d_pt_begin_.p, d_pt_end_.p, d_centers_.p, d_lengths_.p, d_M_.p, stream_);
    }
    phase_end(kPhP2M);
    phase_begin();
    for (int level = t.depth - 1; level >= 1; --level) {
        const int rc = part ? launch_m2m(cheb_, k, C, dp->d_up_parents[level].p, static_cast<int>(dp->up_parents_h[level].size()),
                                         dp->d_part_child_ptr.p, dp->d_part_child_idx.p, d_octant_.p, d_M_.p, stream_)
                            : launch_m2m(cheb_, k, C, d_m2m_parents_[level].p, static_cast<int>(m2m_parents_[level].size()),
                                         d_child_ptr_.p, d_child_idx_.p, d_octant_.p, d_M_.p, stream_);
        if (rc != 0) return hip_fail(static_cast<hipError_t>(rc), "M2M: dynamic LDS attribute");
    }
    phase_end(kPhM2M);
    HIPCHK(hipGetLastError());
    return BBFMM_OK;
}

int FmmTree::downward(int k, const DownwardPlan *dp, const TargetSet *wx) {
    CHK(downward_m2l(k, dp));
    return downward_tail(k, dp, wx);
}

int FmmTree::downward_m2l(int k, const DownwardPlan *dp) {
    const HostTree &t = tree_;
    const int64_t C = t.n_cells();
    have_locals_ = false;
    const bool s2_pairs = m2l_pairs2_ && !m2l_batches_.empty();
    const int lp_len = m2l_s2_plan_.n_par();
    if (!s2_pairs) HIPCHK(hipMemsetAsync(d_L_.p, 0, static_cast<size_t>(k) * C * cheb_.n_pad * sizeof(double), stream_));
    const int m2l_len = shared_basis_ ? basis_pad_ : cheb_.n_pad;
    const double *m_in = shared_basis_ ? d_Mc_.p : m2l_pairs_ ? d_Mp_.p : d_M_.p;
    const int s1_len = m2l_pairs_ ? m2l_npar_ : m2l_len, s1_ne16 = m2l_pairs_ ? m2l_ne16_ : 0;
    if (m2l_pairs_ && !m2l_batches_.empty()) {
        phase_begin();
        if (m2l_axes_ == 2)
            launch_m2l_parity2(d_M_.p, cheb_.n_pad, d_Mp_.p, m2l_npar_, m2l_s1_off_, ops_.p, ops_.n / (ops_.p * ops_.p), static_cast<int64_t>(k) * C, stream_);
        else
            launch_m2l_parity(d_M_.p, cheb_.n_pad, d_Mp_.p, m2l_npar_, m2l_ne16_, m2l_ne_, m2l_no_, ops_.p, static_cast<int64_t>(k) * C, stream_);
        phase_end(kPhM2L1);
    }
    double *l_out = shared_basis_ ? d_Lc_.p : s2_pairs ? d_Lp_.p : d_L_.p;
    if (shared_basis_) {
        phase_begin();
        launch_m2l_basis(d_basis_classes_.p, d_basis_tiles_c_.p, n_basis_tiles_, cheb_.n_pad, basis_pad_, k, C, d_M_.p, d_Mc_.p, stream_);
        HIPCHK(hipMemsetAsync(d_Lc_.p, 0, static_cast<size_t>(k) * C * basis_pad_ * sizeof(double), stream_));
        phase_end(kPhM2L1);
    }
    const int nb = static_cast<int>(m2l_batches_.size());
    for (int k0 = 0; k0 < k; k0 += m2l_rhs_chunk_) {
        const int kb = std::min(m2l_rhs_chunk_, k - k0);
        const double *m_chunk = m_in + static_cast<size_t>(k0) * C * s1_len;
        double *l_chunk = s2_pairs ? d_Lp_.p : l_out + static_cast<size_t>(k0) * C * m2l_len;
        if (s2_pairs) HIPCHK(hipMemsetAsync(d_Lp_.p, 0, static_cast<size_t>(kb) * C * lp_len * sizeof(double), stream_));
        for (int b = 0; b < nb; ++b) {
            const M2lBatch &mb = m2l_batches_[static_cast<size_t>(b)];
            const int t1_first = dp ? dp->batch_t1[4 * b] : mb.t1_first, t1_count = dp ? dp->batch_t1[4 * b + 1] : mb.t1_count;
            const int t2_first = dp ? dp->batch_t2[2 * b] : mb.t2_first, t2_count = dp ? dp->batch_t2[2 * b + 1] : mb.t2_count;
            if (t2_count == 0) continue;
            phase_begin();
            if (nb > 1)
                launch_m2l_zero_segments(d_m2l_zero_.p + 2 * m2l_zero_ptr_[static_cast<size_t>(b)],
                                         m2l_zero_ptr_[static_cast<size_t>(b) + 1] - m2l_zero_ptr_[static_cast<size_t>(b)], kb, d_cbuf_.p,
                                         cbuf_batch_len_, stream_);
            if (dp) {
                launch_m2l_stage1(d_m2l_classes_.p, dp->d_tiles1.p + t1_first, dp->d_tile_idx.p, t1_count, s1_len, m2l_slot_t_, kb,
                                  C, m_chunk, d_cbuf_.p, cbuf_batch_len_, stream_, false, m2l_max_blocks_, s1_ne16, m2l_s_ee_, m2l_s_eo_);
                launch_m2l_stage1(d_m2l_classes_.p, dp->d_tiles1.p + dp->batch_t1[4 * b + 2], dp->d_tile_idx.p, dp->batch_t1[4 * b + 3],
                                  s1_len, m2l_slot_t_, kb, C, m_chunk, d_cbuf_.p, cbuf_batch_len_, stream_, true, m2l_max_blocks_, s1_ne16, m2l_s_ee_, m2l_s_eo_);
            } else
                launch_m2l_stage1(d_m2l_classes_.p, d_m2l_tiles1_.p + t1_first, d_tile_idx1_.p, t1_count, s1_len, m2l_slot_t_, kb, C,
                                  m_chunk, d_cbuf_.p, cbuf_batch_len_, stream_, false, m2l_max_blocks_, s1_ne16, m2l_s_ee_, m2l_s_eo_);
            phase_end(kPhM2L1);
            phase_begin();
            if (s2_pairs) {
                if (!launch_m2l_stage2_pairs(d_m2l_classes_.p, dp ? dp->d_tiles2.p + t2_first : d_m2l_tiles2_.p + t2_first,
                                             dp ? dp->d_tile_idx.p : nullptr, t2_count, m2l_s2_plan_, kb, C, d_cbuf_.p, cbuf_batch_len_,
                                             dp ? dp->d_qlist.p : d_m2l_qlist_.p, l_chunk, stream_, !deterministic_, &m2l_s2_last_ksplit_))
                    return fail(BBFMM_DEVICE_ERROR, "internal: no stage-2 kernel instance for the parity-basis column plan");
            } else if (dp)
                launch_m2l_stage2(d_m2l_classes_.p, dp->d_tiles2.p + t2_first, dp->d_tile_idx.p, t2_count, m2l_len, kb, C, d_cbuf_.p,
                                  cbuf_batch_len_, dp->d_qlist.p, l_chunk, stream_, !deterministic_);
            else
                launch_m2l_stage2(d_m2l_classes_.p, d_m2l_tiles2_.p + t2_first, nullptr, t2_count, m2l_len, kb, C, d_cbuf_.p,
                                  cbuf_batch_len_, d_m2l_qlist_.p, l_chunk, stream_, !deterministic_);
            phase_end(kPhM2L2);
        }
        if (s2_pairs) {
            phase_begin();
            if (m2l_s2_axes_ == 2)
                launch_m2l_unparity2(d_Lp_.p, m2l_s2_plan_, d_L_.p + static_cast<size_t>(k0) * C * cheb_.n_pad, ops_.n, cheb_.n_pad, ops_.p,
                                     ops_.n / (ops_.p * ops_.p), static_cast<int64_t>(kb) * C, stream_);
            else
                launch_m2l_unparity(d_Lp_.p, lp_len, m2l_s2_plan_.ne16(), d_L_.p + static_cast<size_t>(k0) * C * cheb_.n_pad, ops_.n, cheb_.n_pad,
                                    m2l_ne_, m2l_no_, ops_.p, static_cast<int64_t>(kb) * C, stream_);
            phase_end(kPhM2L2);
        }
    }
    if (shared_basis_) {
        phase_begin();
        launch_m2l_basis(d_basis_classes_.p, d_basis_tiles_e_.p, n_basis_tiles_, basis_pad_, cheb_.n_pad, k, C, d_Lc_.p, d_L_.p, stream_);
        phase_end(kPhM2L2);
    }
    HIPCHK(hipGetLastError());
    (void)t;
    return BBFMM_OK;
}

int FmmTree::downward_tail(int k, const DownwardPlan *dp, const TargetSet *wx) {
    const HostTree &t = tree_;
    const int64_t C = t.n_cells();
    phase_begin();
    if (t.adaptive && wx) {
        launch_wx_sym(kernel_, cheb_, wx->n_wx_jobs, wx->wx_tb.p, wx->wx_te.p, wx->wx_range.p, wx->n_wxl_jobs, wx->wxl_tb.p, wx->wxl_te.p,
                      wx->wxl_range.p, d_w_idx_.p, d_centers_.p,
                      d_lengths_.p, src_ptr_, d_w_sorted_.p, t.n_points, k, d_M_.p, d_L_.p, C * cheb_.n_pad, wx->out.p,
                      static_cast<int64_t>(wx->m), wx->sym_off, static_cast<int>(wx->m), stream_);
    } else if (t.adaptive) {
        if (dp)
            launch_p2l(kernel_, cheb_, dp->n_x_jobs, dp->d_x_cells.p, dp->d_x_ptr.p, dp->d_x_runs.p, d_centers_.p,
                       d_lengths_.p, src_ptr_, d_w_sorted_.p, t.n_points, k, C, d_L_.p, stream_);
        else
            launch_p2l(kernel_, cheb_, static_cast<int>(x_cells_.size()), d_x_cells_.p, d_x_job_run_ptr_.p,
                       d_x_runs_.p, d_centers_.p, d_lengths_.p, src_ptr_, d_w_sorted_.p, t.n_points, k, C, d_L_.p,
                       stream_);
    }
    phase_end(kPhP2L);
    phase_begin();
    for (int level = 2; level <= t.depth; ++level) {
        const int rc = launch_l2l(cheb_, k, C, d_level_cells_[level].p, static_cast<int>(level_cells_[level].size()), d_parent_.p,
                                  d_octant_.p, dp ? dp->d_active.p : d_active_.p, d_L_.p, stream_);
        if (rc != 0) return hip_fail(static_cast<hipError_t>(rc), "L2L: dynamic LDS attribute");
    }
    phase_end(kPhL2L);
    HIPCHK(hipGetLastError());
    have_locals_ = dp == nullptr;
    return BBFMM_OK;
}

hipError_t FmmTree::columns_to_host(double *dst, int64_t ld, const double *d_src, int64_t m, int ncols) {
    if (m <= 0 || ncols <= 0) return hipSuccess;
    if (ld == m) return hipMemcpyAsync(dst, d_src, static_cast<size_t>(m) * ncols * sizeof(double), hipMemcpyDeviceToHost, stream_);
    for (int j = 0; j < ncols; ++j) {
        const hipError_t e = hipMemcpyAsync(dst + static_cast<size_t>(j) * ld, d_src + static_cast<size_t>(j) * m,
                                            static_cast<size_t>(m) * sizeof(double), hipMemcpyDeviceToHost, stream_);
        if (e != hipSuccess) return e;
    }
    return hipSuccess;
}

int FmmTree::leaf_pass(const TargetSet &ts, int k, bool with_grads, bool fixed_plan) {
    CHK(leaf_pass_near(ts, k, with_grads, stream_, 3, false, fixed_plan));
    return leaf_pass_far(ts, k, with_grads);
}

int FmmTree::leaf_pass_near(const TargetSet &ts, int k, bool with_grads, hipStream_t st, int parts, bool wx_done,
                            bool fixed_plan) {
    const HostTree &t = tree_;
    const int64_t C = t.n_cells();
    double *grad = with_grads ? ts.grad.p : nullptr;
    const bool timed = st == stream_;
    if (parts & 1) {
        if (!wx_done)
            HIPCHK(hipMemsetAsync(ts.out.p, 0, static_cast<size_t>(k) * ts.m * sizeof(double), st));
        if (with_grads) HIPCHK(hipMemsetAsync(grad, 0, static_cast<size_t>(k) * d_ * ts.m * sizeof(double), st));
        DirectJobs jobs{ts.n_jobs, ts.job_cell.p, ts.tgt_begin.p, ts.tgt_end.p, d_u_run_ptr_.p, d_u_runs_.p};
        static const bool sym_on = [] {
            const char *e = std::getenv("BBFMM_P2P_SYM");
            return !e || std::atoi(e) != 0;
        }();
        if (timed) phase_begin();
        if (ts.sym && sym_on && !deterministic_ && !with_grads)
            launch_p2p_sym(kernel_, ts.n_sym_jobs, ts.sym_tb.p, ts.sym_te.p, ts.sym_ptr.p, ts.n_syml_jobs, ts.syml_tb.p, ts.syml_te.p,
                           ts.syml_ptr.p, ts.n_symw_jobs, ts.symw_tb.p, ts.symw_te.p,
                           ts.symw_ptr.p, ts.sym_runs.p, ts.sym_off, src_ptr_, d_w_sorted_.p, t.n_points, k, ts.out.p, ts.m, st);
        else
            launch_p2p(kernel_, d_, jobs, ts.xyz_ptr, ts.m, src_ptr_, d_w_sorted_.p, t.n_points, k, ts.out.p, grad, st,
                       fixed_plan);
        if (timed) phase_end(kPhP2P);
    }
    if (parts & 2) {
        if (timed) phase_begin();
        if (t.adaptive && !wx_done)
            launch_m2p(kernel_, cheb_, ts.n_w_jobs, ts.w_tgt_begin.p, ts.w_tgt_end.p, ts.w_begin.p, ts.w_end.p,
                       d_w_idx_.p, d_centers_.p, d_lengths_.p, ts.xyz_ptr, ts.m, k, C, d_M_.p, ts.out.p, grad, st, fixed_plan);
        if (timed) phase_end(kPhM2P);
    }
    HIPCHK(hipGetLastError());
    return BBFMM_OK;
}

int FmmTree::leaf_pass_far(const TargetSet &ts, int k, bool with_grads) {
    const int64_t C = tree_.n_cells();
    double *grad = with_grads ? ts.grad.p : nullptr;
    phase_begin();
    launch_l2p(cheb_, ts.n_jobs, ts.job_cell.p, ts.tgt_begin.p, ts.tgt_end.p, d_centers_.p, d_lengths_.p, ts.xyz_ptr,
               ts.m, k, C, d_L_.p, ts.out.p, grad, stream_);
    phase_end(kPhL2P);
    HIPCHK(hipGetLastError());
    return BBFMM_OK;
}

int FmmTree::set_weights(const double *w, int64_t rows, int k, int64_t ldw) {
    if (host_only_) return fail(BBFMM_DEVICE_ERROR, "handle was created with BBFMM_FLAG_HOST_ONLY");
    part_pending_k_ = 0;
    pin_w_k_ = 0;
    static const bool verbose = std::getenv("BBFMM_VERBOSE") != nullptr;
    const auto t_0 = std::chrono::steady_clock::now();
    CHK(put_weights(w, rows, k, ldw));
    const auto t_1 = std::chrono::steady_clock::now();
    nrhs_ = k;
    have_locals_ = locals_requested_ = false;
    CHK(upward(k));
    const auto t_2 = std::chrono::steady_clock::now();
    HIPCHK(hipStreamSynchronize(stream_));
    if (verbose) {
        const auto t_3 = std::chrono::steady_clock::now();
        auto ms = [](auto a, auto b) { return std::chrono::duration<double, std::milli>(b - a).count(); };
        std::fprintf(stderr, "[bbfmm] set_weights: weights staged and their copies queued %.3f ms, upward pass queued %.3f ms, waited for the device %.3f ms\n",
                     ms(t_0, t_1), ms(t_1, t_2), ms(t_2, t_3));
    }
    return BBFMM_OK;
}

static const char kPartialMultipoles[] =
    "the multipoles are one partition's share (bbfmm_matvec_partition_upward ran last): bbfmm_set_weights must be called first";

int FmmTree::set_local_coefficients(const double *w, int64_t rows, int k, int64_t ldw) {
    if (host_only_) return fail(BBFMM_DEVICE_ERROR, "handle was created with BBFMM_FLAG_HOST_ONLY");
    part_pending_k_ = 0;
    if (nrhs_ == 0) return fail(BBFMM_BAD_ARGUMENT, "set_weights must be called first");
    if (multipoles_partial_) return fail(BBFMM_BAD_ARGUMENT, kPartialMultipoles);
    if (k != nrhs_) return fail(BBFMM_BAD_ARGUMENT, "weights must have the column count given to set_weights");
    CHK(put_weights(w, rows, k, ldw));
    CHK(downward(k));
    HIPCHK(hipStreamSynchronize(stream_));
    locals_requested_ = true;
    return BBFMM_OK;
}

int FmmTree::evaluate(const double *w, int64_t rows, int k, int64_t ldw, const double *x, int64_t m, int64_t ldx,
                      double *out, int64_t ldo, double *grad, int64_t ldg, bool with_grads, bool leaves_only,
                      int64_t *bad_point_index) {
    if (host_only_) return fail(BBFMM_DEVICE_ERROR, "handle was created with BBFMM_FLAG_HOST_ONLY");
    part_pending_k_ = 0;
    if (nrhs_ == 0) return fail(BBFMM_BAD_ARGUMENT, "set_weights must be called first");
    if (multipoles_partial_) return fail(BBFMM_BAD_ARGUMENT, kPartialMultipoles);
    if (k != nrhs_) return fail(BBFMM_BAD_ARGUMENT, "weights must have the column count given to set_weights");
    if (m < 0 || (m > 0 && (!x || !out || ldx < m || ldo < m))) return fail(BBFMM_BAD_ARGUMENT, "bad target/output arrays");
    if (with_grads && m > 0 && (!grad || ldg < m)) return fail(BBFMM_BAD_ARGUMENT, "bad gradient array");
    if (leaves_only && !have_locals_) return fail(BBFMM_BAD_ARGUMENT, "set_local_coefficients must be called first");
    if (m >= (int64_t(1) << 31)) return fail(BBFMM_BAD_ARGUMENT, "more than 2^31-1 target points");
    static const bool verbose = std::getenv("BBFMM_VERBOSE") != nullptr;
    const auto t_begin = std::chrono::steady_clock::now();
    static const bool sources_fast = [] {
        const char *e = std::getenv("BBFMM_EVAL_SOURCES_FAST");
        return !e || std::atoi(e) != 0;
    }();
    bool m2l_queued = false;
    last_eval_at_sources_ = false;
    if (sources_fast && !leaves_only && !with_grads && !have_part_ && !locals_requested_ && m == tree_.n_points && src_targets_.m == m && w && rows >= m &&
        ldw >= rows && static_cast<size_t>(2) * k * m <= kMaxPinnedDoubles) {
        CHK(ensure_rhs_capacity(k));
        CHK(downward_m2l(k, nullptr));
        m2l_queued = true;
        if (targets_are_sources(x, m, ldx)) {
            const int64_t N = m;
            const TargetSet &ts = src_targets_;
            const auto t_cmp = std::chrono::steady_clock::now();
            CHK(put_weights(w, rows, k, ldw));
            const auto t_put = std::chrono::steady_clock::now();
            static const bool wx_on = [] {
                const char *e = std::getenv("BBFMM_WX_FUSED");
                const char *e2 = std::getenv("BBFMM_P2P_SYM");
                return (!e || std::atoi(e) != 0) && (!e2 || std::atoi(e2) != 0);
            }();
            const bool wx = wx_on && !deterministic_ && ts.sym && ts.n_wx_jobs > 0;
            if (wx) HIPCHK(hipMemsetAsync(ts.out.p, 0, static_cast<size_t>(k) * ts.m * sizeof(double), stream_));
            CHK(downward_tail(k, nullptr, wx ? &ts : nullptr));
            CHK(leaf_pass_near(ts, k, false, stream_, 3, wx));
            CHK(leaf_pass_far(ts, k, false));
            phase_begin();
            launch_scatter_output(ts.out.p, ts.m, k, ts.perm.p, d_out_.p, N, 0, stream_);
            phase_end(kPhScatter);
            HIPCHK(hipGetLastError());
            double *pin_out = h_pin_ + static_cast<size_t>(k) * N;
            const auto t_queued = std::chrono::steady_clock::now();
            if (verbose) {
                HIPCHK(hipStreamSynchronize(stream_));
            }
            const auto t_dev = std::chrono::steady_clock::now();
            CHK(download_pieces(d_out_.p, static_cast<int64_t>(k) * N, pin_out, [&](int64_t pb, int64_t pe) {
                while (pb < pe) {
                    const int64_t col = pb / N, row = pb - col * N, len = std::min(pe - pb, N - row);
                    std::memcpy(out + col * ldo + row, pin_out + pb, static_cast<size_t>(len) * sizeof(double));
                    pb += len;
                }
            }));
            last_eval_at_sources_ = true;
            if (verbose) {
                const auto t_end = std::chrono::steady_clock::now();
                auto ms = [](auto a, auto b) { return std::chrono::duration<double, std::milli>(b - a).count(); };
                std::fprintf(stderr, "[bbfmm] evaluate: the %lld targets are the sources (M2L queued and targets compared in %.3f ms beside it, weights "
                                     "compared %.3f ms, rest queued %.3f ms, waited for the device %.3f ms, potentials home %.3f ms); total %.3f ms\n",
                             static_cast<long long>(m), ms(t_begin, t_cmp), ms(t_cmp, t_put), ms(t_put, t_queued), ms(t_queued, t_dev), ms(t_dev, t_end),
                             ms(t_begin, t_end));
            }
            return BBFMM_OK;
        }
    }
    last_eval_rows_of_sources_ = false;
    if (sources_fast && solver_tree_ && !m2l_queued && !leaves_only && !with_grads && (!have_part_ || group_primary_) && !locals_requested_ && k == 1 && w &&
        m < tree_.n_points && m >= std::max<int64_t>(1024, tree_.n_points / 2048) && m <= tree_.n_points / 2) {
        std::vector<int64_t> rows_of;
        bool known = false;
        if (tree_.n_points <= (int64_t(1) << 26) && targets_are_rows_of_sources(x, m, ldx, &rows_of)) {
            const uint64_t key = subset_key(rows_of.data(), m);
            known = subset_plan_cached(rows_of.data(), m, key) || key == last_subset_miss_;
            if (!known) last_subset_miss_ = key;
        }
        if (known) {
            SubsetPlan *sp = nullptr;
            CHK(subset_plan(rows_of.data(), m, &sp));
            CHK(put_weights(w, rows, 1, ldw));
            CHK(downward(1, &sp->dp));
            CHK(leaf_pass(sp->ts, 1, false));
            phase_begin();
            launch_scatter_output(sp->ts.out.p, m, 1, sp->ts.perm.p, d_out_.p, m, 0, stream_);
            phase_end(kPhScatter);
            HIPCHK(hipGetLastError());
            CHK(ensure_pinned(static_cast<size_t>(2) * tree_.n_points));
            double *pin_out = h_pin_ + tree_.n_points;
            CHK(download_pieces(d_out_.p, m, pin_out, [&](int64_t pb, int64_t pe) {
                std::memcpy(out + pb, pin_out + pb, static_cast<size_t>(pe - pb) * sizeof(double));
            }));
            last_eval_rows_of_sources_ = true;
            return BBFMM_OK;
// ... 101 lines not shown
        }
        return rc;
    }
    TargetSet ts;
    arena_begin();
    const double *dx[3] = {d_x0, d_x1, d_x2};
    int rc = build_target_set_device(nullptr, m, m, &ts, bad_point_index, nullptr, dx);
    if (rc == BBFMM_OK) rc = talloc(&ts.out, static_cast<size_t>(m));
    if (rc == BBFMM_OK && d_grad) rc = talloc(&ts.grad, static_cast<size_t>(d_) * m);
    if (rc == BBFMM_OK) rc = leaf_pass(ts, 1, d_grad != nullptr, batch_independent);
    if (rc == BBFMM_OK) {
        phase_begin();
        launch_scatter_output(ts.out.p, m, 1, ts.perm.p, d_out, m, 0, stream_);
        if (d_grad) launch_scatter_output(ts.grad.p, m, d_, ts.perm.p, d_grad, m, 0, stream_);
        phase_end(kPhScatter);
        hipError_t e = hipGetLastError();
        if (e == hipSuccess) e = hipStreamSynchronize(stream_);
        if (e != hipSuccess) rc = hip_fail(e, "scatter device-target values");
    } else if (stream_) {
        (void)hipStreamSynchronize(stream_);
    }
    free_target_set(&ts);
    const int arc = arena_end();
    return rc == BBFMM_OK ? arc : rc;
}

int FmmTree::matvec_device(const double *d_w, int64_t ldw, int k, double *d_out, int64_t ldo, bool sync) {
    if (host_only_) return fail(BBFMM_DEVICE_ERROR, "handle was created with BBFMM_FLAG_HOST_ONLY");
    part_pending_k_ = 0;
    const int64_t N = tree_.n_points;
    if (!d_w || !d_out || k < 1 || ldw < N || ldo < N) return fail(BBFMM_BAD_ARGUMENT, "bad device matvec arguments");
    CHK(ensure_rhs_capacity(k));
    nrhs_ = k;
    pin_w_k_ = 0;
    phase_begin();
    launch_gather_weights(d_w, ldw, k, d_order_.p, N, d_w_sorted_.p, stream_);
    phase_end(kPhGather);
    if (have_part_ && part_targets_.out.n < static_cast<size_t>(k) * part_targets_.m) {
        dfree(&part_targets_.out);
        CHK(dalloc(&part_targets_.out, static_cast<size_t>(k) * part_targets_.m));
    }
    const TargetSet &ts = have_part_ ? part_targets_ : src_targets_;
    const DownwardPlan *plan = have_part_ ? &part_plan_ : nullptr;
    static const bool wx_on = [] {
        const char *e = std::getenv("BBFMM_WX_FUSED");
        const char *e2 = std::getenv("BBFMM_P2P_SYM");
        return (!e || std::atoi(e) != 0) && (!e2 || std::atoi(e2) != 0);
    }();
    const bool wx = wx_on && !deterministic_ && !have_part_ && ts.sym && ts.n_wx_jobs > 0;
    CHK(upward(k, nullptr));
    if (wx) HIPCHK(hipMemsetAsync(ts.out.p, 0, static_cast<size_t>(k) * ts.m * sizeof(double), stream_));
    CHK(downward(k, plan, wx ? &ts : nullptr));
    CHK(leaf_pass_near(ts, k, false, stream_, 3, wx));
    CHK(leaf_pass_far(ts, k, false));
    phase_begin();
    launch_scatter_output(ts.out.p, ts.m, k, ts.perm.p, d_out, ldo, 0, stream_);
    phase_end(kPhScatter);
    HIPCHK(hipGetLastError());
    if (sync) HIPCHK(hipStreamSynchronize(stream_));
    return BBFMM_OK;
}

int64_t FmmTree::partition_coarse_count() const {
    return have_part_ || (host_only_ && part_world_ > 1) ? part_plan_.coarse_cells * static_cast<int64_t>(round_up(ops_.n, 32)) : 0;
}

int FmmTree::matvec_partition_upward(const double *d_w, int64_t ldw, int k, double *d_coarse, hipStream_t comm_stream, bool near_field) {
    if (host_only_) return fail(BBFMM_DEVICE_ERROR, "handle was created with BBFMM_FLAG_HOST_ONLY");
    if (!have_part_) return fail(BBFMM_BAD_ARGUMENT, "bbfmm_set_partition (world > 1) must be called first");
    const int64_t N = tree_.n_points, C = tree_.n_cells();
    const int64_t cnt = partition_coarse_count();
    if (!d_w || k < 1 || ldw < N || (cnt > 0 && !d_coarse)) return fail(BBFMM_BAD_ARGUMENT, "bad partitioned matvec arguments");
    CHK(ensure_rhs_capacity(k));
    nrhs_ = k;
    pin_w_k_ = 0;
    have_locals_ = locals_requested_ = false;
    phase_begin();
    launch_gather_weights_subset(d_w, ldw, k, d_order_.p, part_plan_.d_gather_pos.p, static_cast<int64_t>(part_plan_.gather_pos_h.size()), N,
                                 d_w_sorted_.p, stream_);
    phase_end(kPhGather);
    if (part_targets_.out.n < static_cast<size_t>(k) * part_targets_.m) {
        dfree(&part_targets_.out);
        CHK(dalloc(&part_targets_.out, static_cast<size_t>(k) * part_targets_.m));
    }
    CHK(upward(k, &part_plan_));
    phase_begin();
    for (int j = 0; j < k && cnt > 0; ++j)
        HIPCHK(hipMemcpyAsync(d_coarse + static_cast<size_t>(j) * cnt, d_M_.p + static_cast<size_t>(j) * C * cheb_.n_pad,
                              static_cast<size_t>(cnt) * sizeof(double), hipMemcpyDeviceToDevice, stream_));
    phase_end(kPhM2M);
    if (comm_stream) {
        HIPCHK(hipEventRecord(ev_pack_, stream_));
        HIPCHK(hipStreamWaitEvent(comm_stream, ev_pack_, 0));
    }
    if (near_field) CHK(leaf_pass_near(part_targets_, k, false, stream_, 1));
    part_pending_k_ = near_field ? k : -k;
    return BBFMM_OK;
}

int FmmTree::partition_subset_finish(const double *d_coarse, const int64_t *idx, int64_t n_idx, double *h_out, hipStream_t comm_stream) {
    if (host_only_) return fail(BBFMM_DEVICE_ERROR, "handle was created with BBFMM_FLAG_HOST_ONLY");
    if (!have_part_ || (part_pending_k_ != 1 && part_pending_k_ != -1)) return fail(BBFMM_BAD_ARGUMENT, "bbfmm_matvec_partition_upward (one rhs) must be called first");
    if (n_idx < 0 || (n_idx > 0 && (!idx || !h_out))) return fail(BBFMM_BAD_ARGUMENT, "bad partial product arguments");
    const int64_t C = tree_.n_cells();
    const int64_t cnt = partition_coarse_count();
    if (cnt > 0 && !d_coarse) return fail(BBFMM_BAD_ARGUMENT, "bad partitioned matvec arguments");
    part_pending_k_ = 0;
    SubsetPlan *sp = nullptr;
    if (n_idx > 0) CHK(subset_plan(idx, n_idx, &sp));
    if (comm_stream) {
        HIPCHK(hipEventRecord(ev_comm_, comm_stream));
        HIPCHK(hipStreamWaitEvent(stream_, ev_comm_, 0));
    }
    phase_begin();
    if (cnt > 0)
        HIPCHK(hipMemcpyAsync(d_M_.p, d_coarse, static_cast<size_t>(cnt) * sizeof(double), hipMemcpyDeviceToDevice, stream_));
    phase_end(kPhM2M);
    (void)C;
    if (n_idx == 0) return BBFMM_OK;
    CHK(downward(1, &sp->dp));
    CHK(leaf_pass(sp->ts, 1, false));
    phase_begin();
    launch_scatter_output(sp->ts.out.p, n_idx, 1, sp->ts.perm.p, d_out_.p, n_idx, 0, stream_);
    HIPCHK(hipMemcpyAsync(h_out, d_out_.p, static_cast<size_t>(n_idx) * sizeof(double), hipMemcpyDeviceToHost, stream_));
    phase_end(kPhScatter);
    HIPCHK(hipGetLastError());
    return BBFMM_OK;
}

int FmmTree::partition_finish_core(const double *d_coarse, hipStream_t comm_stream, int *k_out) {
    if (host_only_) return fail(BBFMM_DEVICE_ERROR, "handle was created with BBFMM_FLAG_HOST_ONLY");
    if (!have_part_ || part_pending_k_ < 1) return fail(BBFMM_BAD_ARGUMENT, "bbfmm_matvec_partition_upward must be called first");
    const int64_t C = tree_.n_cells();
    const int64_t cnt = partition_coarse_count();
    const int k = part_pending_k_;
    if (cnt > 0 && !d_coarse) return fail(BBFMM_BAD_ARGUMENT, "bad partitioned matvec arguments");
    part_pending_k_ = 0;
    if (comm_stream) {
        HIPCHK(hipEventRecord(ev_comm_, comm_stream));
        HIPCHK(hipStreamWaitEvent(stream_, ev_comm_, 0));
    }
    phase_begin();
    for (int j = 0; j < k && cnt > 0; ++j)
        HIPCHK(hipMemcpyAsync(d_M_.p + static_cast<size_t>(j) * C * cheb_.n_pad, d_coarse + static_cast<size_t>(j) * cnt,
                              static_cast<size_t>(cnt) * sizeof(double), hipMemcpyDeviceToDevice, stream_));
    phase_end(kPhM2M);
    const TargetSet &ts = part_targets_;
    static const bool wx_on = [] {
        const char *e = std::getenv("BBFMM_WX_FUSED");
        const char *e2 = std::getenv("BBFMM_P2P_SYM");
        return (!e || std::atoi(e) != 0) && (!e2 || std::atoi(e2) != 0);
    }();
    const bool wx = wx_on && !deterministic_ && ts.sym && ts.n_wx_jobs > 0;
    CHK(downward(k, &part_plan_, wx ? &ts : nullptr));
    CHK(leaf_pass_near(ts, k, false, stream_, 2, wx));
    CHK(leaf_pass_far(ts, k, false));
    *k_out = k;
    return BBFMM_OK;
}

int FmmTree::matvec_partition_finish(const double *d_coarse, double *d_out, int64_t ldo, bool sync, hipStream_t comm_stream) {
    if (!d_out || ldo < tree_.n_points) return fail(BBFMM_BAD_ARGUMENT, "bad partitioned matvec arguments");
    int k = 0;
    CHK(partition_finish_core(d_coarse, comm_stream, &k));
    const TargetSet &ts = part_targets_;
    phase_begin();
    launch_scatter_output(ts.out.p, ts.m, k, ts.perm.p, d_out, ldo, 0, stream_);
    phase_end(kPhScatter);
    HIPCHK(hipGetLastError());
    if (sync) HIPCHK(hipStreamSynchronize(stream_));
    return BBFMM_OK;
}

int FmmTree::matvec_partition_finish_sorted(const double *d_coarse, double *d_seg, int64_t ld, hipStream_t comm_stream) {
    if (!d_seg || ld < part_targets_.m) return fail(BBFMM_BAD_ARGUMENT, "bad partitioned matvec arguments");
    int k = 0;
    CHK(partition_finish_core(d_coarse, comm_stream, &k));
    const TargetSet &ts = part_targets_;
    phase_begin();
    if (ts.m > 0)
        HIPCHK(hipMemcpy2DAsync(d_seg, static_cast<size_t>(ld) * sizeof(double), ts.out.p, static_cast<size_t>(ts.m) * sizeof(double),
                                static_cast<size_t>(ts.m) * sizeof(double), static_cast<size_t>(k), hipMemcpyDeviceToDevice, stream_));
    phase_end(kPhScatter);
    HIPCHK(hipGetLastError());
    return BBFMM_OK;
}

int FmmTree::matvec_partition_finish_host(const double *d_coarse, double *h_seg, int64_t ld, hipStream_t comm_stream) {
    if (!h_seg || ld < part_targets_.m) return fail(BBFMM_BAD_ARGUMENT, "bad partitioned matvec arguments");
    int k = 0;
    CHK(partition_finish_core(d_coarse, comm_stream, &k));
    const TargetSet &ts = part_targets_;
    phase_begin();
    if (ts.m > 0)
// ... 138 lines not shown
        }
    });
    return BBFMM_OK;
}

void FmmTree::stats(bbfmm_tree_stats *out) const {
    const HostTree &t = tree_;
    std::memset(out, 0, sizeof *out);
    out->d = d_;
    out->order = order_;
    out->n_nodes = ops_.n;
    out->depth = t.depth;
    out->n_points = t.n_points;
    out->n_cells = t.n_cells();
    for (int64_t c = 0; c < t.n_cells(); ++c) out->n_leaves += t.is_leaf[c];
    out->n_u = static_cast<int64_t>(t.u.idx.size());
    out->n_v = static_cast<int64_t>(t.v.idx.size());
    out->n_w = static_cast<int64_t>(t.w.idx.size());
    out->n_x = static_cast<int64_t>(t.x.idx.size());
    int64_t pairs = 0, tile_bytes = 0;
    const int64_t per_pt = 8 * d_ + 8;
    for (int32_t c : src_leaves_) {
        const int64_t nt = t.pt_end[c] - t.pt_begin[c];
        int64_t ns = 0;
        for (int64_t r = u_runs_.ptr[c]; r < u_runs_.ptr[c + 1]; ++r) ns += u_runs_.idx[2 * r + 1] - u_runs_.idx[2 * r];
        pairs += nt * ns;
        tile_bytes += (nt + ns) * per_pt;
    }
    out->p2p_pairs = pairs;
    out->p2p_tile_bytes_k1 = tile_bytes;
    for (int32_t c : src_leaves_) {
        const int64_t nt = t.pt_end[c] - t.pt_begin[c], nw = t.w.ptr[c + 1] - t.w.ptr[c];
        out->wx_pairs += nt * nw * ops_.n;
        out->wx_tile_bytes_k1 += nw * (nt * per_pt + 2 * static_cast<int64_t>(ops_.n) * 8);
    }
    out->m2l_flops_k1 = m2l_flops_k1_;
    for (int r : basis_rank_) out->m2l_basis_rank = std::max<int32_t>(out->m2l_basis_rank, r);
    out->m2l_basis_len = shared_basis_ ? basis_pad_ : 0;
    out->m2l_batches = static_cast<int32_t>(m2l_batches_.size());
    out->m2l_rhs_per_pass = m2l_rhs_chunk_;
    out->m2l_slots_bytes_per_rhs = cbuf_total_len_ * 8;
    out->m2l_intermediate_bytes = static_cast<int64_t>(d_cbuf_.n) * 8;
    for (int a = 0; a < d_; ++a) out->center[a] = t.center[a];
    out->radius = t.radius;
}

int FmmTree::debug_get_coefficients(char which, int k, double *out) {
    if (host_only_) return fail(BBFMM_DEVICE_ERROR, "handle was created with BBFMM_FLAG_HOST_ONLY");
    if (k < 1 || k > k_cap_ || !out) return fail(BBFMM_BAD_ARGUMENT, "bad coefficient request");
    const double *src = (which == 'M' || which == 'm') ? d_M_.p : d_L_.p;
    const int64_t C = tree_.n_cells();
    const int n = ops_.n, n_pad = cheb_.n_pad;
    HIPCHK(hipStreamSynchronize(stream_));
    HIPCHK(hipMemcpy2D(out, n * sizeof(double), src, n_pad * sizeof(double), n * sizeof(double),
                       static_cast<size_t>(k) * C, hipMemcpyDeviceToHost));
    return BBFMM_OK;
}

}
```

ferreus_rbf_rs_amd/csrc/fmm_tree.hpp:

```cpp
#pragma once
#include <hip/hip_runtime.h>

#include <cstdint>
#include <string>
#include <memory>
#include <vector>

#include "device.hpp"
#include "targets.hpp"
#include "ferreus_bbfmm_hip.h"
#include "kernels.hpp"
#include "operators.hpp"
#include "parallel.hpp"
#include "tree.hpp"
#include "tree_device.hpp"

namespace bbfmm {

enum Phase {
    kPhGather = 0, kPhP2M, kPhM2M, kPhM2L1, kPhM2L2, kPhP2L, kPhL2L, kPhP2P, kPhM2P, kPhL2P, kPhScatter,
    kNumPhases
};
static_assert(kNumPhases == BBFMM_N_PHASES, "phase table");

// ... 136 lines not shown
    int matvec_partition_finish_sorted(const double *d_coarse, double *d_seg, int64_t ld, hipStream_t comm_stream);
    int partition_scatter(const double *d_all, int first_part, int n_parts, int64_t m_max, int k, double *d_out, int64_t ldo);
    int matvec_partition_finish_host(const double *d_coarse, double *h_seg, int64_t ld, hipStream_t comm_stream);
    const std::vector<int64_t> &partition_bounds() const { return part_bounds_; }
    int register_subset(const int64_t *idx, int64_t n_idx, int *id_out);
    int matvec_subset_device(int id, const double *d_w, double *d_y, bool sync);
    int set_partition(int rank, int world);

    const HostTree &tree() const { return tree_; }
    const Operators &ops() const { return ops_; }
    const PodDoubles &source_points() const { return pts_; }
    int order() const { return order_; }
    const char *last_error() const { return err_.c_str(); }
    hipStream_t stream() const { return stream_; }
    bool host_only() const { return host_only_; }
    bool deterministic() const { return deterministic_; }
    bool leaves_ready() const { return nrhs_ == 1 && have_locals_; }
    void bind_device() const {
        if (device_ >= 0) (void)hipSetDevice(device_);
    }
    int device() const { return device_; }
    bool tree_built_on_device() const { return tree_built_on_device_; }
    bool last_evaluate_at_sources() const { return last_eval_at_sources_; }
    int last_evaluate_path() const { return last_eval_at_sources_ ? 1 : (last_eval_rows_of_sources_ ? 2 : 0); }
    bool targets_are_rows_of_sources(const double *x, int64_t m, int64_t ldx, std::vector<int64_t> *rows);
    bool targets_are_sources(const double *x, int64_t m, int64_t ldx) const;
    void stats(bbfmm_tree_stats *out) const;
    void set_profiling(bool on) { profiling_ = on; }
    const double *phase_ms() { collect_phase_times(); return phase_ms_; }
    const int64_t *phase_count() { collect_phase_times(); return phase_count_; }
    void reset_phase_ms() {
        collect_phase_times();
        for (double &v : phase_ms_) v = 0.0;
        for (int64_t &v : phase_count_) v = 0;
    }
    const std::vector<int64_t> &partition_rows() const { return part_rows_; }
    bool partitioned() const { return part_world_ > 1; }
    int partition_rank() const { return part_rank_; }
    const std::vector<HostM2lClass> &m2l_host() const { return m2l_host_; }
    void m2l_variant_stats(int64_t *n_variants, int64_t *n_cells) const {
        *n_variants = static_cast<int64_t>(m2l_variants_.size());
        *n_cells = 0;
        for (const HostM2lClass &v : m2l_variants_) *n_cells += static_cast<int64_t>(v.cells.size());
    }
    void debug_m2l_pairs(std::vector<int32_t> *out) const;
    bool m2l_pairs() const { return m2l_pairs_; }
    void debug_m2l_pairs_axes(std::vector<int32_t> *out) const;
    void debug_m2l_pairs_stage2(std::vector<int32_t> *out) const;
    bool m2l_pairs_stage2() const { return m2l_pairs2_; }
    void debug_m2l_pairs_axes_stage2(std::vector<int32_t> *out) const;
    int debug_m2l_s2_last_ksplit() const { return m2l_s2_last_ksplit_; }
    int debug_apply_m2l_tables_host(const double *M, double *L) const;
    int debug_get_coefficients(char which, int k, double *out);
    int debug_partition_upward_counts(int64_t *counts_out, uint8_t *reads_out, int64_t *info_out) const;

  private:
    int fail(int code, const std::string &msg);
    int hip_fail(hipError_t e, const char *what);
    int upload();
    int build_m2l_tables();
    void fill_m2l_operator_arrays(const HostM2lClass &hc, std::vector<double> *vt_all,
                                  std::vector<double> *u_all) const;
    void fill_m2l_operator_arrays(const HostM2lClass &hc, double *vt_all, double *u_all) const;
    int ensure_rhs_capacity(int k);
    int upward(int k, const DownwardPlan *dp = nullptr);
    int downward(int k, const DownwardPlan *dp = nullptr, const TargetSet *wx = nullptr);
    int downward_m2l(int k, const DownwardPlan *dp);
    int downward_tail(int k, const DownwardPlan *dp, const TargetSet *wx);
    int leaf_pass(const TargetSet &ts, int k, bool with_grads, bool fixed_plan = false);
    int leaf_pass_near(const TargetSet &ts, int k, bool with_grads, hipStream_t st, int parts, bool wx_done = false,
                       bool fixed_plan = false);
    int leaf_pass_far(const TargetSet &ts, int k, bool with_grads);
    int build_target_set(const double *x, int64_t m, int64_t ldx, TargetSet *ts, int64_t *bad_point_index,
                         std::vector<int32_t> *leaves_out = nullptr);
    int build_target_set_device(const double *x, int64_t m, int64_t ldx, TargetSet *ts, int64_t *bad_point_index,
                                std::vector<int32_t> *leaves_out, const double *const *d_x = nullptr);
    int ensure_leaf_lookup();
    int build_target_set_host(const double *x, int64_t m, int64_t ldx, TargetSet *ts, int64_t *bad_point_index,
                              std::vector<int32_t> *leaves_out);
    int build_source_target_set();
    int build_sym_runs(TargetSet *ts, const std::vector<int32_t> &job_cells, int64_t pb, int64_t pe, const std::vector<uint8_t> *part_active = nullptr);
    void free_target_set(TargetSet *ts);
    hipError_t columns_to_host(double *dst, int64_t ld, const double *d_src, int64_t m, int ncols);
    int upload_weights(const double *w, int64_t rows, int k, int64_t ldw);
    void phase_begin();
    void phase_end(int ph);
    void collect_phase_times();
    hipEvent_t get_event();

    std::string err_;
    bool host_only_ = false;
    bool deterministic_ = false;
    bool tree_built_on_device_ = false;
    DevTreePoints dev_points_;
    int order_ = 0, d_ = 0;
    KernelSpec kernel_{};
    bbfmm_params params_{};
    PodDoubles pts_;
    HostTree tree_;
    Operators ops_;
    int nrhs_ = 0;
    bool have_locals_ = false;
    bool locals_requested_ = false;
    Csr u_runs_;
    Csr x_runs_;
    std::vector<int32_t> src_leaves_;
    std::vector<std::vector<int32_t>> m2m_parents_;
    std::vector<std::vector<int32_t>> level_cells_;
    std::vector<int32_t> x_cells_;
    std::vector<HostM2lClass> m2l_host_;
    std::vector<HostM2lClass> m2l_variants_;
    std::vector<M2lTileDesc> m2l_tiles1_h_;
    std::vector<int32_t> m2l_tile_idx1_h_;
    std::vector<M2lClass> m2l_classes_h_;
    std::vector<M2lTileDesc> m2l_tiles_h_;
    std::vector<uint16_t> m2l_qlist_h_;
    std::vector<M2lBatch> m2l_batches_;
    std::vector<int32_t> m2l_batch_of_class_;
    std::vector<std::vector<int32_t>> m2l_group_ops_;
    std::vector<int32_t> m2l_zero_h_;
    std::vector<int64_t> m2l_zero_ptr_;
    int64_t cbuf_batch_len_ = 0;
    int64_t cbuf_total_len_ = 0;
    int64_t m2l_budget_bytes_ = int64_t(16384) << 20;
    int m2l_rhs_chunk_ = 1;
    double m2l_flops_k1_ = 0;
    int n_cu_ = 256;
    int device_ = -1;
    std::vector<M2lTileDesc> m2l_tiles2_h_;
    int m2l_slot_t_ = 1;
    int m2l_max_blocks_ = 1;
    int m2l_s1_block_ = kM2lS1Block;
    bool m2l_pairs_ = false;
    int m2l_ne_ = 0, m2l_no_ = 0;
    int m2l_ne16_ = 0, m2l_npar_ = 0;
    std::vector<int32_t> m2l_partner_;
    int m2l_axes_ = 1;
    M2lParityOffsets m2l_s1_off_{{0, 0, 0, 0}};
    int m2l_s_ee_ = 0, m2l_s_eo_ = 0;
    int64_t m2l_work_[2] = {0, 0};
    std::vector<int32_t> m2l_partner_y_;
    std::vector<int32_t> m2l_par_node_;
    std::vector<int8_t> m2l_par_sign_;
    int m2l_rho_y(int m) const {
        const int p2 = ops_.n / (ops_.p * ops_.p);
        return m + (ops_.p - 1 - 2 * ((m / p2) % ops_.p)) * p2;
    }
    int m2l_rho(int m) const {
        const int p1 = ops_.n / ops_.p;
        return m + (ops_.p - 1 - 2 * (m / p1)) * p1;
    }
    DevBuf<double> d_Mp_;
    bool m2l_pairs2_ = false;
    M2lS2PairsPlan m2l_s2_plan_{1, 1, 1, 1};
    DevBuf<double> d_Lp_;
    int m2l_s2_last_ksplit_ = 0;
    int m2l_s2_axes_ = 1;
    int64_t m2l_s2_work_[2] = {0, 0};
    std::vector<int32_t> m2l_s2_node_;
    std::vector<int8_t> m2l_s2_sign_;
    std::vector<int8_t> m2l_s2_part_;
    int part_rank_ = 0, part_world_ = 1;
    std::vector<int64_t> part_rows_, part_bounds_;
    int partition_finish_core(const double *d_coarse, hipStream_t comm_stream, int *k_out);
    bool part_empty_ = false;
    DownwardPlan part_plan_;
    std::vector<std::unique_ptr<SubsetPlan>> subset_plans_;
    uint64_t subset_clock_ = 0;
    int build_downward_plan(const std::vector<int32_t> &target_leaves, DownwardPlan *dp, bool restrict_upward = false,
                            int64_t own_b = 0, int64_t own_e = 0);
    int part_pending_k_ = 0;
    bool multipoles_partial_ = false;
    void free_downward_plan(DownwardPlan *dp);
    int subset_plan(const int64_t *idx, int64_t n_idx, SubsetPlan **out);
    uint64_t subset_key(const int64_t *idx, int64_t n_idx) const;
    bool subset_plan_cached(const int64_t *idx, int64_t n_idx, uint64_t key) const;
    uint64_t last_subset_miss_ = 0;
    int fill_subset_plan(const int64_t *idx, int64_t n_idx, SubsetPlan *sp);
    std::vector<std::unique_ptr<SubsetPlan>> registered_plans_;

    hipStream_t stream_ = nullptr;
    hipEvent_t ev_pack_ = nullptr, ev_comm_ = nullptr;
    struct PendingPhase {
        int phase;
        hipEvent_t e0, e1;
    };
    std::vector<PendingPhase> pending_;
    std::vector<hipEvent_t> event_pool_;
    hipEvent_t pending_begin_ = nullptr;
    bool profiling_ = false;
    double phase_ms_[kNumPhases] = {0};
    int64_t phase_count_[kNumPhases] = {0};
    std::vector<void *> owned_;
    template <class T> int dalloc(DevBuf<T> *b, size_t n, bool zero = false);
    template <class T> int dupload(DevBuf<T> *b, const std::vector<T> &v);
    template <class T> int talloc(DevBuf<T> *b, size_t n, bool zero = false);
    template <class T> int tupload(DevBuf<T> *b, const std::vector<T> &v);
    void arena_begin();
    int arena_end();
    template <class T> void dfree(DevBuf<T> *b);

    ChebRef cheb_{};
    DevBuf<DevCheb> d_cheb_;
    DevBuf<double> d_src_[3];
    const double *src_ptr_[3] = {nullptr, nullptr, nullptr};
    DevBuf<double> d_zero_axis_;
    DevBuf<uint8_t> arena_;
    size_t arena_used_ = 0, arena_need_ = 0;
    bool arena_active_ = false;
    DevBuf<uint64_t> d_tab_keys_;
    DevBuf<int32_t> d_tab_vals_;
    DevBuf<uint8_t> d_is_leaf_;
    DevBuf<uint8_t> d_tscratch_;
    DevLeafLookup lk_;
// ... 66 lines not shown
```

ferreus_rbf_rs_amd/fmm_tree.py:

```python
from __future__ import annotations

import ctypes
import enum
from typing import Optional

import numpy as np

from . import _lib as L


class KernelType(enum.IntEnum):
    LinearRbf = 0
    ThinPlateSplineRbf = 1
    CubicRbf = 2
    Spheroidal3Rbf = 3
    Spheroidal5Rbf = 4
    Spheroidal7Rbf = 5
    Spheroidal9Rbf = 6
    Laplacian = 7
    OneOverR2 = 8
    OneOverR4 = 9
    GaussianExt = 100
    MultiquadricExt = 101

# ... 466 lines not shown
        self._raise(fn(self._h, buf.ctypes.data, n.value, ctypes.byref(n), ctypes.byref(on)))
        d, ops, i = self.dim, [], 0
        while i < n.value:
            level, octant, kind, ne = (int(v) for v in buf[i:i + 4])
            ent = buf[i + 4:i + 4 + ne * (d + 1)].reshape(ne, d + 1)
            ops.append({"level": level, "octant": octant, "kind": kind,
                        "pairs": [tuple(int(x) for x in e[1:]) for e in ent if e[0] == 1],
                        "singles": [tuple(int(x) for x in e[1:]) for e in ent if e[0] == 0]})
            i += 4 + ne * (d + 1)
        return bool(on.value), ops

    def debug_m2l_pairs_axes(self, stage=1):
        if stage == 2:
            fn = self._lib.bbfmm_debug_m2l_pairs_axes_stage2
            n = ctypes.c_int64()
            self._raise(fn(self._h, None, 0, ctypes.byref(n)))
            buf = np.zeros(max(n.value, 1), dtype=np.int32)
            self._raise(fn(self._h, buf.ctypes.data, n.value, ctypes.byref(n)))
            info = {"axes": int(buf[0]), "work_x": int(buf[1]), "work_xy": int(buf[2])}
            d, ops, i = self.dim, [], 3
            while i < n.value:
                level, octant, kp, kpy, k_pad, pad, ne = (int(v) for v in buf[i:i + 7])
                ent = buf[i + 7:i + 7 + ne * (d + 4)].reshape(ne, d + 4)
                by_kind = [{tuple(int(x) for x in e[4:]): (int(e[1]), int(e[2]), int(e[3])) for e in ent if e[0] == k}
                           for k in range(3)]
                ops.append({"level": level, "octant": octant, "kp": kp, "kpy": kpy, "k_pad": k_pad, "pad": pad,
                            "singles": by_kind[0], "x_pairs": by_kind[1], "y_pairs": by_kind[2]})
                i += 7 + ne * (d + 4)
            return info, ops
        fn = self._lib.bbfmm_debug_m2l_pairs_axes
        n = ctypes.c_int64()
        self._raise(fn(self._h, None, 0, ctypes.byref(n)))
        buf = np.zeros(max(n.value, 1), dtype=np.int32)
        self._raise(fn(self._h, buf.ctypes.data, n.value, ctypes.byref(n)))
        info = {"axes": int(buf[0]), "work_x": int(buf[1]), "work_xy": int(buf[2])}
        d, ops, i = self.dim, [], 3
        while i < n.value:
            level, octant, kind, pad_cols, yb0, n_blk, ne = (int(v) for v in buf[i:i + 7])
            kinds = [int(v) for v in buf[i + 7:i + 7 + n_blk]]
            ent = buf[i + 7 + n_blk:i + 7 + n_blk + ne * (d + 3)].reshape(ne, d + 3)
            by_kind = [{tuple(int(x) for x in e[3:]): (int(e[1]), int(e[2])) for e in ent if e[0] == k} for k in range(3)]
            ops.append({"level": level, "octant": octant, "kind": kind, "pad_cols": pad_cols, "yb0": yb0, "block_kinds": kinds,
                        "singles": by_kind[0], "x_pairs": by_kind[1], "y_pairs": by_kind[2]})
            i += 7 + n_blk + ne * (d + 3)
        return info, ops

    def debug_m2l_s2_last_ksplit(self) -> int:
        ks = ctypes.c_int32()
        self._raise(self._lib.bbfmm_debug_m2l_s2_last_ksplit(self._h, ctypes.byref(ks)))
        return ks.value

    def debug_get_coefficients(self, which: str, k: int) -> np.ndarray:
        s = self.stats()
        out = np.zeros((k, s.n_cells, s.n_nodes))
        self._raise(self._lib.bbfmm_debug_get_coefficients(self._h, which.encode()[0:1], k,
                                                           out.ctypes.data))
        return out

    def debug_apply_m2l_tables_host(self, M: np.ndarray) -> np.ndarray:
        M = np.ascontiguousarray(M, dtype=np.float64)
        Lc = np.zeros_like(M)
        self._raise(self._lib.bbfmm_debug_apply_m2l_tables_host(self._h, M.ctypes.data,
                                                                Lc.ctypes.data))
        return Lc


def fp64_valu_selftest():
    tf, mhz = ctypes.c_double(0), ctypes.c_double(0)
    if L.load().bbfmm_fp64_valu_selftest(ctypes.byref(tf), ctypes.byref(mhz)) != L.OK:
        raise RuntimeError("the FP64 VALU microbenchmark needs a HIP device")
    return tf.value, mhz.value


def mfma_f64_selftest():
    tf = ctypes.c_double(0)
    errs = ctypes.c_int32(-1)
    info = (ctypes.c_double * 6)()
    rc = L.load().bbfmm_mfma_f64_selftest(ctypes.byref(tf), ctypes.byref(errs), info)
    if rc != L.OK:
        raise RuntimeError("MFMA self-test needs a HIP device")
    mfma_f64_selftest.info = dict(zip(["cycles_per_mfma_lone_wave", "clock_mhz_lone_wave",
                                       "cycles_per_mfma_per_simd_busy", "clock_mhz_busy",
                                       "tflops_1wave_per_simd", "tflops_2waves_per_simd"], list(info)))
    return tf.value, errs.value


def debug_kernel_values(where: int, kernel_id: int, base_range: float, total_sill: float, r2):
    x = np.ascontiguousarray(r2, dtype=np.float64).ravel()
    v, vg, f = np.empty_like(x), np.empty_like(x), np.empty_like(x)
    rc = L.load().bbfmm_debug_kernel_values(where, kernel_id, float(base_range), float(total_sill), x.ctypes.data, x.size,
                                            v.ctypes.data, vg.ctypes.data, f.ctypes.data)
    if rc != L.OK:
        raise RuntimeError(f"bbfmm_debug_kernel_values failed with status {rc}")
    return v, vg, f


DEBUG_MATH = {"sqrt": 0, "sqrt_rsqrt": 1, "rcp": 2, "log": 3}


def debug_math(where: int, which: str, x):
    x = np.ascontiguousarray(x, dtype=np.float64).ravel()
    out, out2 = np.empty_like(x), np.empty_like(x)
    rc = L.load().bbfmm_debug_math(where, DEBUG_MATH[which], x.ctypes.data, x.size, out.ctypes.data,
                                   out2.ctypes.data if which == "sqrt_rsqrt" else None)
    if rc != L.OK:
        raise RuntimeError(f"bbfmm_debug_math failed with status {rc}")
    return (out, out2) if which == "sqrt_rsqrt" else out
# ... 1 lines not shown
```

include/ferreus_bbfmm_hip.h:

```cpp
#ifndef FERREUS_BBFMM_HIP_H
#define FERREUS_BBFMM_HIP_H

#include <stdint.h>

#ifdef __cplusplus
extern "C" {
#endif

typedef enum {
    BBFMM_OK = 0,
    BBFMM_POINT_OUTSIDE_TREE = 1,
    BBFMM_KERNEL_NO_GRADIENTS = 2,
    BBFMM_BAD_ARGUMENT = 3,
    BBFMM_DEVICE_ERROR = 4,
    BBFMM_UNSUPPORTED = 5,
    BBFMM_CALLBACK_FAILED = 6
} bbfmm_status;

typedef enum {
    BBFMM_KERNEL_LINEAR_RBF = 0,
    BBFMM_KERNEL_THIN_PLATE_SPLINE_RBF = 1,
    BBFMM_KERNEL_CUBIC_RBF = 2,
    BBFMM_KERNEL_SPHEROIDAL3_RBF = 3,
    BBFMM_KERNEL_SPHEROIDAL5_RBF = 4,
// ... 248 lines not shown
    int64_t wx_pairs;
    int64_t wx_tile_bytes_k1;
    int32_t m2l_basis_rank;
    int32_t m2l_basis_len;
    int32_t m2l_batches;
    int32_t m2l_rhs_per_pass;
    int64_t m2l_slots_bytes_per_rhs;
    int64_t m2l_intermediate_bytes;
} bbfmm_tree_stats;

int bbfmm_get_tree_stats(const bbfmm_handle *h, bbfmm_tree_stats *out);
int bbfmm_tree_built_on_device(const bbfmm_handle *h);

int bbfmm_get_cells(const bbfmm_handle *h, uint64_t *keys, uint8_t *is_leaf);
int bbfmm_get_leaf_sources(const bbfmm_handle *h, int64_t *ptr, int64_t *idx);
int bbfmm_get_list(const bbfmm_handle *h, char which, int64_t *ptr, int32_t *idx,
                   int64_t *n_entries);
int bbfmm_get_m2l_ranks(const bbfmm_handle *h, int32_t *ranks, int32_t *n_ref_out);
int bbfmm_get_m2l_operator(const bbfmm_handle *h, int32_t level, int32_t ref, double *out);
int bbfmm_get_m2l_factors(const bbfmm_handle *h, int32_t level, int32_t ref, double *u, double *vt);
int bbfmm_get_permutation_tables(const bbfmm_handle *h, int32_t *n_perm, int32_t *perm,
                                 int32_t *invperm, int32_t *perm_lookup, int32_t *ref_lookup);
int bbfmm_points_to_leaves(const bbfmm_handle *h, const double *x, int64_t m, int64_t ldx,
                           int32_t *cell_out, int64_t *bad_point_index);

#define BBFMM_N_PHASES 11
int bbfmm_set_profiling(bbfmm_handle *h, int32_t enable);
int bbfmm_get_phase_ms(bbfmm_handle *h, double *ms_out, int64_t *count_out);
int bbfmm_reset_phase_ms(bbfmm_handle *h);

int bbfmm_mfma_f64_selftest(double *tflops, int32_t *layout_errors, double *info6);
int bbfmm_fp64_valu_selftest(double *tflops, double *clock_mhz);

int bbfmm_debug_kernel_values(int32_t where, int32_t kernel_id, double base_range, double total_sill, const double *r2,
                              int64_t n, double *value_out, double *value_g_out, double *factor_out);
int bbfmm_debug_math(int32_t where, int32_t which, const double *x, int64_t n, double *out, double *out2);

int bbfmm_debug_dense_m2m(const bbfmm_handle *h, int32_t child_index, double *out);
int bbfmm_debug_apply_m2l_tables_host(const bbfmm_handle *h, const double *M, double *L);
int bbfmm_debug_m2l_variants(const bbfmm_handle *h, int64_t *n_variants, int64_t *n_cells);
int bbfmm_debug_m2l_pairs(const bbfmm_handle *h, int32_t *out, int64_t cap, int64_t *n_out, int32_t *pairs_on);
int bbfmm_debug_m2l_pairs_axes(const bbfmm_handle *h, int32_t *out, int64_t cap, int64_t *n_out);
int bbfmm_debug_m2l_pairs_stage2(const bbfmm_handle *h, int32_t *out, int64_t cap, int64_t *n_out, int32_t *pairs_on);
int bbfmm_debug_m2l_pairs_axes_stage2(const bbfmm_handle *h, int32_t *out, int64_t cap, int64_t *n_out);
int bbfmm_debug_m2l_s2_last_ksplit(const bbfmm_handle *h, int32_t *ksplit);

uint64_t bbfmm_debug_morton_encode(int32_t d, const uint64_t *anchor, uint64_t level);
void bbfmm_debug_morton_decode(int32_t d, uint64_t key, uint64_t *anchor_out, uint64_t *level_out);
int32_t bbfmm_debug_morton_neighbours(int32_t d, uint64_t key, uint64_t *keys_out);
int32_t bbfmm_debug_direction_vectors(int32_t d, int32_t *out);
int bbfmm_debug_reference_vectors(const bbfmm_handle *h, int32_t *out, int32_t *n_ref_out);

int bbfmm_debug_get_coefficients(bbfmm_handle *h, char which, int32_t k, double *out);


typedef int (*bbfmm_apply_fn)(void *user, const double *x, double *y, int64_t n);
typedef void (*bbfmm_iteration_fn)(void *user, int64_t iter, double residual, double progress);

enum { BBFMM_ACCURACY_ABSOLUTE = 0, BBFMM_ACCURACY_RELATIVE = 1 };

void bbfmm_givens_rotation(double f, double g, double *c, double *s, double *r);

int bbfmm_fgmres(int64_t n, bbfmm_apply_fn a, void *a_user, const double *b, bbfmm_apply_fn m, void *m_user,
                 const double *x0, int32_t max_outer_iterations, int32_t max_inner_iterations,
                 int32_t tolerance_type, double tolerance, bbfmm_iteration_fn callback, void *cb_user,
                 double *x, int64_t *iterations, double *final_residual);

int bbfmm_schwarz_ddm_solver(int64_t n, bbfmm_apply_fn matvec, void *a_user, const double *rhs,
                             bbfmm_apply_fn m, void *m_user, int32_t max_iterations, int32_t tolerance_type,
                             double tolerance, bbfmm_iteration_fn callback, void *cb_user, double *x,
                             int64_t *iterations, double *final_residual);

typedef struct bbfmm_rbf_system {
    bbfmm_handle *tree;
    int64_t basis_size;
    const double *monomial_matrix;
    int64_t ld_monomial;
    double nugget;
} bbfmm_rbf_system;
int bbfmm_rbf_system_apply(void *user, const double *x, double *y, int64_t n);

typedef struct bbfmm_ddm bbfmm_ddm;
typedef struct bbfmm_ddm_params {
    int64_t leaf_threshold;
    double overlap_quota;
    double coarse_ratio;
    int64_t coarse_threshold;
} bbfmm_ddm_params;
void bbfmm_ddm_params_defaults(bbfmm_ddm_params *out);
void bbfmm_ddm_params_for_points(int64_t n, bbfmm_ddm_params *out);
int bbfmm_ddm_build(const double *points, int64_t n, int32_t d, int64_t ld, const bbfmm_ddm_params *params,
                    bbfmm_ddm **out);
void bbfmm_ddm_destroy(bbfmm_ddm *t);
int32_t bbfmm_ddm_num_levels(const bbfmm_ddm *t);
int64_t bbfmm_ddm_level_size(const bbfmm_ddm *t, int32_t level);
int bbfmm_ddm_level_points(const bbfmm_ddm *t, int32_t level, int64_t *out);
int64_t bbfmm_ddm_num_domains(const bbfmm_ddm *t, int32_t level);
int64_t bbfmm_ddm_domain_size(const bbfmm_ddm *t, int32_t level, int64_t domain);
int bbfmm_ddm_domain(const bbfmm_ddm *t, int32_t level, int64_t domain, int64_t *indices, uint8_t *internal,
                     double *extents);

typedef struct bbfmm_schwarz bbfmm_schwarz;
typedef struct bbfmm_interpolant {
    int32_t kernel_type;
    int32_t polynomial_degree;
    double nugget, base_range, total_sill;
// ... 84 lines not shown
```

Measured before the change: 32.85 matvecs/s.

## Fuse M2L parity transforms into M2M/L2L and scatter output from L2P

Moves the M2L parity-basis transform of multipoles into the M2M kernel and the inverse parity transform of locals into the L2L kernel, so the separate full-array parity passes are skipped. L2P can also write straight to the user output through a permutation, which avoids a separate scatter pass. Shared row helpers are pulled into a new header, and masks and flags decide when fusion applies. This adds complexity and cases where the fused path must fall back, for example gradients or cells without M2L.

```diff
diff --git a/ferreus_rbf_rs_amd/_lib.py b/ferreus_rbf_rs_amd/_lib.py
--- a/ferreus_rbf_rs_amd/_lib.py
+++ b/ferreus_rbf_rs_amd/_lib.py
@@ -145,6 +145,7 @@
     "bbfmm_debug_m2l_pairs_stage2": (ctypes.c_int, [c_p, c_p, c_i64, c_p, c_p]),
     "bbfmm_debug_m2l_pairs_axes_stage2": (ctypes.c_int, [c_p, c_p, c_i64, c_p]),
     "bbfmm_debug_m2l_s2_last_ksplit": (ctypes.c_int, [c_p, c_p]),
+    "bbfmm_debug_m2l_parity_len": (ctypes.c_int, [c_p, c_p]),
     "bbfmm_debug_get_coefficients": (ctypes.c_int, [c_p, ctypes.c_char, c_i32, c_p]),
     "bbfmm_debug_morton_encode": (ctypes.c_uint64, [c_i32, c_p, ctypes.c_uint64]),
     "bbfmm_debug_morton_decode": (None, [c_i32, ctypes.c_uint64, c_p, c_p]),
diff --git a/ferreus_rbf_rs_amd/build.py b/ferreus_rbf_rs_amd/build.py
--- a/ferreus_rbf_rs_amd/build.py
+++ b/ferreus_rbf_rs_amd/build.py
@@ -14,7 +14,7 @@
 HOST_SOURCES = ["tree.cpp", "operators.cpp", "fmm_tree.cpp", "fmm_m2l_tables.cpp", "fmm_plans.cpp", "device_group.cpp", "capi.cpp", "solver.cpp", "ddm.cpp", "ddm_solver.cpp", "schwarz.cpp", "interpolant.cpp", "closure_triangulate.cpp"]
 HIP_SOURCES = ["device_l2p.hip", "device_p2p.hip", "device_wx.hip", "device_p2m.hip", "device_m2l.hip", "device_transfer.hip", "device_gather.hip", "device_selftest.hip",
                "ddm_kernels.hip", "targets.hip", "schwarz_kernels.hip", "tree_device.hip", "tree_lists_device.hip", "isosurface.hip", "isosurface_finish.hip", "isosurface_closure.hip", "isosurface_intersect.hip", "isosurface_follow.hip", "interpolant_terms.hip", "field_program.hip"]
-HEADERS = ["morton.hpp", "tree.hpp", "parallel.hpp", "kernels.hpp", "operators.hpp", "device.hpp", "device_common.hpp", "device_direct.hpp",
+HEADERS = ["morton.hpp", "tree.hpp", "parallel.hpp", "kernels.hpp", "operators.hpp", "device.hpp", "device_common.hpp", "device_direct.hpp", "m2l_basis_rows.hpp",
            "fmm_tree.hpp", "fmm_tree_impl.hpp", "device_group.hpp", "targets.hpp", "ddm.hpp", "ddm_solver.hpp", "ddm_monomials.hpp", "schwarz_kernels.hpp", "tree_device.hpp", "isosurface.hpp", "isosurface_curvature.hpp", "isosurface_intersect.hpp", "isosurface_closure.hpp", "closure_triangulate.hpp", "interpolant_terms.hpp", "field_program.hpp", os.path.join(ROOT, "include", "ferreus_bbfmm_hip.h")]
 
 
diff --git a/ferreus_rbf_rs_amd/csrc/capi.cpp b/ferreus_rbf_rs_amd/csrc/capi.cpp
--- a/ferreus_rbf_rs_amd/csrc/capi.cpp
+++ b/ferreus_rbf_rs_amd/csrc/capi.cpp
@@ -2011,6 +2011,12 @@
     return BBFMM_OK;
 }
 
+int bbfmm_debug_m2l_parity_len(const bbfmm_handle *h, int32_t *len) {
+    if (!h || !len) return BBFMM_BAD_ARGUMENT;
+    *len = h->tree.debug_m2l_parity_len();
+    return BBFMM_OK;
+}
+
 int bbfmm_debug_get_coefficients(bbfmm_handle *h, char which, int32_t k, double *out) {
     GUARD(h) return h->tree.debug_get_coefficients(which, k, out);
     END_GUARD(h)
diff --git a/ferreus_rbf_rs_amd/csrc/device.hpp b/ferreus_rbf_rs_amd/csrc/device.hpp
--- a/ferreus_rbf_rs_amd/csrc/device.hpp
+++ b/ferreus_rbf_rs_amd/csrc/device.hpp
@@ -75,12 +75,18 @@
                 int K, int64_t C, const int32_t *leaf_cells, int n_leaves, const int32_t *pt_begin,
                 const int32_t *pt_end, const double *centers, const double *lengths, double *M,
                 hipStream_t s);
+struct M2lParityRowArgs;
+struct M2lUnparityRowArgs;
 int launch_m2m(const ChebRef &ch, int K, int64_t C, const int32_t *parents, int n_parents,
                const int64_t *child_ptr, const int32_t *child_idx, const int32_t *octant, double *M,
-               hipStream_t s);
+               hipStream_t s, const M2lParityRowArgs *par = nullptr, double *Mp = nullptr);
+bool m2m_writes_parity(const ChebRef &ch);
 int launch_l2l(const ChebRef &ch, int K, int64_t C, const int32_t *cells, int n_cells,
                const int32_t *parent, const int32_t *octant, const uint8_t *active, double *L,
-               hipStream_t s);
+               hipStream_t s, const M2lUnparityRowArgs *unp = nullptr, const double *Lp = nullptr,
+               const uint8_t *has_m2l = nullptr, const uint8_t *has_x = nullptr);
+bool l2l_reads_parity(const ChebRef &ch);
+void launch_zero_rows(const int32_t *cells, int n_cells, int n_pad, int K, int64_t C, double *L, hipStream_t s);
 
 void launch_m2l_stage1(const M2lClass *classes, const M2lTileDesc *tiles, const int32_t *tile_idx, int n_tiles,
                        int n_pad, int max_slot_t, int K, int64_t C, const double *M, double *cbuf,
@@ -110,6 +116,26 @@
 };
 M2lS2PairsPlan m2l_s2_pairs_plan(int groups_even, int groups_odd);
 M2lS2PairsPlan m2l_s2_pairs_plan2(const int groups[4]);
+struct M2lParityRowArgs {
+    int axes = 0;
+    int n_par = 0;
+    int p = 0;
+    int ne16 = 0, n_e = 0, n_o = 0, p1 = 0;
+    M2lParityOffsets off{{0, 0, 0, 0}};
+    int p2 = 0;
+};
+
+struct M2lUnparityRowArgs {
+    int axes = 0;
+    int n_par = 0;
+    int p = 0;
+    int ne16 = 0, n_e = 0, n_o = 0, p1 = 0;
+    M2lS2PairsPlan plan{1, 1, 1, 1};
+    int p2 = 0;
+};
+void launch_m2l_parity_cells(const double *M, int n_pad, double *Mp, const M2lParityRowArgs &par, const int32_t *cells, int n_cells,
+                             int K, int64_t C, hipStream_t s);
+int m2l_s2_pairs_ksplit(int n_tiles, const M2lS2PairsPlan &plan, int K, bool allow_ksplit);
 bool launch_m2l_stage2_pairs(const M2lClass *classes, const M2lTileDesc *tiles, const int32_t *tile_idx, int n_tiles,
                              const M2lS2PairsPlan &plan, int K, int64_t C, const double *cbuf, int64_t cbuf_len,
                              const uint16_t *qlist, double *Lp, hipStream_t s, bool allow_ksplit = true, int *ksplit_out = nullptr);
@@ -182,7 +208,8 @@
 void launch_l2p(const ChebRef &ch, int n_jobs, const int32_t *leaf_cells, const int32_t *tgt_begin,
                 const int32_t *tgt_end, const double *centers, const double *lengths,
                 const double *const *tgt_xyz, int64_t n_tgt, int K, int64_t C, const double *L,
-                double *out_sorted, double *grad_sorted, hipStream_t s);
+                double *out_sorted, double *grad_sorted, hipStream_t s, const int32_t *perm = nullptr,
+                double *user_out = nullptr, int64_t ldo = 0);
 
 bool l2p_order_supported(int p, int d);
 
diff --git a/ferreus_rbf_rs_amd/csrc/device_l2p.hip b/ferreus_rbf_rs_amd/csrc/device_l2p.hip
--- a/ferreus_rbf_rs_amd/csrc/device_l2p.hip
+++ b/ferreus_rbf_rs_amd/csrc/device_l2p.hip
@@ -14,7 +14,9 @@
                                                              const double *__restrict__ lengths, Xyz tgt,
                                                              int64_t n_tgt, int K, int64_t C,
                                                              const double *__restrict__ L,
-                                                             double *__restrict__ out, double *__restrict__ grad) {
+                                                             double *__restrict__ out, double *__restrict__ grad,
+                                                             const int32_t *__restrict__ perm, double *__restrict__ user_out,
+                                                             int64_t ldo) {
     constexpr int P1 = D > 1 ? P : 1, P2 = D > 2 ? P : 1, N = P * P1 * P2;
     constexpr int WAVES = l2p_waves<P, D>();
     __shared__ double s_L[WAVES][N];
@@ -93,7 +95,8 @@
                 }
             }
             if (valid) {
-                out[(int64_t)k * n_tgt + t] += y;
+                if (!GRAD && perm) user_out[(int64_t)k * ldo + perm[t]] = out[(int64_t)k * n_tgt + t] + y;
+                else out[(int64_t)k * n_tgt + t] += y;
                 if (GRAD) {
                     grad[((int64_t)k * D + 0) * n_tgt + t] += gx * gs;
                     if (D > 1) grad[((int64_t)k * D + 1) * n_tgt + t] += gy * gs;
@@ -108,29 +111,30 @@
 static void l2p_launch_pd(const ChebRef &ch, int n_jobs, const int32_t *leaf_cells, const int32_t *tgt_begin,
                           const int32_t *tgt_end, const double *centers, const double *lengths, Xyz tgt,
                           int64_t n_tgt, int K, int64_t C, const double *L, double *out_sorted, double *grad_sorted,
-                          hipStream_t s) {
+                          hipStream_t s, const int32_t *perm, double *user_out, int64_t ldo) {
     constexpr int WAVES = l2p_waves<P, D>();
     const int blocks = (n_jobs + WAVES - 1) / WAVES;
     if (grad_sorted)
         hipLaunchKernelGGL((l2p_kernel<P, D, true>), dim3(blocks), dim3(64 * WAVES), 0, s, ch.dev, n_jobs,
                            leaf_cells, tgt_begin, tgt_end, centers, lengths, tgt, n_tgt, K, C, L, out_sorted,
-                           grad_sorted);
+                           grad_sorted, perm, user_out, ldo);
     else
         hipLaunchKernelGGL((l2p_kernel<P, D, false>), dim3(blocks), dim3(64 * WAVES), 0, s, ch.dev, n_jobs,
                            leaf_cells, tgt_begin, tgt_end, centers, lengths, tgt, n_tgt, K, C, L, out_sorted,
-                           grad_sorted);
+                           grad_sorted, perm, user_out, ldo);
 }
 
 template <int P>
 static void l2p_launch_p(const ChebRef &ch, int n_jobs, const int32_t *leaf_cells, const int32_t *tgt_begin,
                          const int32_t *tgt_end, const double *centers, const double *lengths, Xyz tgt, int64_t n_tgt,
-                         int K, int64_t C, const double *L, double *out_sorted, double *grad_sorted, hipStream_t s) {
+                         int K, int64_t C, const double *L, double *out_sorted, double *grad_sorted, hipStream_t s,
+                         const int32_t *perm, double *user_out, int64_t ldo) {
     if (ch.d == 3) {
-        l2p_launch_pd<P, 3>(ch, n_jobs, leaf_cells, tgt_begin, tgt_end, centers, lengths, tgt, n_tgt, K, C, L, out_sorted, grad_sorted, s);
+        l2p_launch_pd<P, 3>(ch, n_jobs, leaf_cells, tgt_begin, tgt_end, centers, lengths, tgt, n_tgt, K, C, L, out_sorted, grad_sorted, s, perm, user_out, ldo);
     } else if (ch.d == 2) {
-        l2p_launch_pd<P, 2>(ch, n_jobs, leaf_cells, tgt_begin, tgt_end, centers, lengths, tgt, n_tgt, K, C, L, out_sorted, grad_sorted, s);
+        l2p_launch_pd<P, 2>(ch, n_jobs, leaf_cells, tgt_begin, tgt_end, centers, lengths, tgt, n_tgt, K, C, L, out_sorted, grad_sorted, s, perm, user_out, ldo);
     } else {
-        l2p_launch_pd<P, 1>(ch, n_jobs, leaf_cells, tgt_begin, tgt_end, centers, lengths, tgt, n_tgt, K, C, L, out_sorted, grad_sorted, s);
+        l2p_launch_pd<P, 1>(ch, n_jobs, leaf_cells, tgt_begin, tgt_end, centers, lengths, tgt, n_tgt, K, C, L, out_sorted, grad_sorted, s, perm, user_out, ldo);
     }
 }
 
@@ -139,12 +143,13 @@
 void launch_l2p(const ChebRef &ch, int n_jobs, const int32_t *leaf_cells, const int32_t *tgt_begin,
                 const int32_t *tgt_end, const double *centers, const double *lengths, const double *const *tgt_xyz,
                 int64_t n_tgt, int K, int64_t C, const double *L, double *out_sorted, double *grad_sorted,
-                hipStream_t s) {
+                hipStream_t s, const int32_t *perm, double *user_out, int64_t ldo) {
     if (n_jobs == 0) return;
+    if (perm && grad_sorted) return;
     const Xyz tgt = make_xyz(tgt_xyz);
     dispatch_order<2, 16>(ch.p, [&](auto pc) {
         l2p_launch_p<decltype(pc)::value>(ch, n_jobs, leaf_cells, tgt_begin, tgt_end, centers, lengths, tgt, n_tgt, K, C, L,
-                                          out_sorted, grad_sorted, s);
+                                          out_sorted, grad_sorted, s, perm, user_out, ldo);
     });
 }
 
diff --git a/ferreus_rbf_rs_amd/csrc/device_m2l.hip b/ferreus_rbf_rs_amd/csrc/device_m2l.hip
--- a/ferreus_rbf_rs_amd/csrc/device_m2l.hip
+++ b/ferreus_rbf_rs_amd/csrc/device_m2l.hip
@@ -1,4 +1,5 @@
 #include "device_common.hpp"
+#include "m2l_basis_rows.hpp"
 
 #include <cmath>
 
@@ -728,11 +729,15 @@
                        plan.n_par(), plan.ce, plan.co, ksplit, C, cbuf, cbuf_len, Lp, qlist, tile_idx);
 }
 
+int m2l_s2_pairs_ksplit(int n_tiles, const M2lS2PairsPlan &plan, int K, bool allow_ksplit) {
+    return m2l_s2_ksplit(static_cast<int64_t>(n_tiles) * (plan.ce + plan.co) * K, allow_ksplit);
+}
+
 bool launch_m2l_stage2_pairs(const M2lClass *classes, const M2lTileDesc *tiles, const int32_t *tile_idx, int n_tiles,
                              const M2lS2PairsPlan &plan, int K, int64_t C, const double *cbuf, int64_t cbuf_len,
                              const uint16_t *qlist, double *Lp, hipStream_t s, bool allow_ksplit, int *ksplit_out) {
     if (n_tiles == 0) return true;
-    const int ksplit = m2l_s2_ksplit(static_cast<int64_t>(n_tiles) * (plan.ce + plan.co) * K, allow_ksplit);
+    const int ksplit = m2l_s2_pairs_ksplit(n_tiles, plan, K, allow_ksplit);
     if (ksplit_out) *ksplit_out = ksplit;
     if (plan.ya > 0) {
 #define M2L_S2_DISPATCH2(A, YA, B, YB)                                                                                   \
@@ -761,16 +766,7 @@
     if (row >= rows) return;
     const double *src = Lp + row * n_par;
     double *dst = L + row * n_pad;
-    for (int j = threadIdx.x & 63; j < n_e; j += 64) {
-        const double e = src[j];
-        if (j < n_o) {
-            const double o = src[ne16 + j];
-            dst[j] = e + o;
-            dst[j + (p - 1 - 2 * (j / p1)) * p1] = e - o;
-        } else {
-            dst[j] = e;
-        }
-    }
+    m2l_unparity_row(src, ne16, n_e, n_o, p, p1, threadIdx.x & 63, [&](int m, double v) { dst[m] = v; });
     for (int j = n + (threadIdx.x & 63); j < n_pad; j += 64) dst[j] = 0.0;
 }
 
@@ -789,23 +785,7 @@
     const int n_par = plan.n_par();
     const double *src = Lp + row * n_par;
     double *dst = L + row * n_pad;
-    const int h = (p + 1) / 2, f = p / 2;
-    for (int e = threadIdx.x & 63; e < h * h * p2; e += 64) {
-        const int i0 = e / (h * p2), i1 = (e - i0 * h * p2) / p2, r = e - (i0 * h + i1) * p2;
-        const int m = (i0 * p + i1) * p2 + r;
-        const int dx = (p - 1 - 2 * i0) * p * p2, dy = (p - 1 - 2 * i1) * p2;
-        const bool cx = i0 >= f, cy = i1 >= f;
-        const int je = (i0 * h + i1) * p2 + r, jo = (i0 * f + i1) * p2 + r;
-        const double ee = src[plan.col(0, je)];
-        const double eo = cy ? 0.0 : src[plan.col(1, jo)];
-        const double oe = cx ? 0.0 : src[plan.col(2, je)];
-        const double oo = cx || cy ? 0.0 : src[plan.col(3, jo)];
-        const double a = cy ? ee : ee + eo, b = ee - eo, c = cy ? oe : oe + oo, d = oe - oo;
-        dst[m] = cx ? a : a + c;
-        if (!cx) dst[m + dx] = a - c;
-        if (!cy) dst[m + dy] = cx ? b : b + d;
-        if (!cx && !cy) dst[m + dx + dy] = b - d;
-    }
+    m2l_unparity2_row(src, plan, p, p2, threadIdx.x & 63, [&](int m, double v) { dst[m] = v; });
     for (int j = n + (threadIdx.x & 63); j < n_pad; j += 64) dst[j] = 0.0;
 }
 
@@ -822,16 +802,7 @@
     if (row >= rows) return;
     const double *src = M + row * n_pad;
     double *dst = Mp + row * n_par;
-    for (int j = threadIdx.x & 63; j < n_e; j += 64) {
-        const double v = src[j];
-        if (j < n_o) {
-            const double w = src[j + (p - 1 - 2 * (j / p1)) * p1];
-            dst[j] = v + w;
-            dst[ne16 + j] = v - w;
-        } else {
-            dst[j] = v;
-        }
-    }
+    m2l_parity_row(src, dst, ne16, n_e, n_o, p, p1, threadIdx.x & 63);
 }
 
 void launch_m2l_parity(const double *M, int n_pad, double *Mp, int n_par, int ne16, int n_e, int n_o, int p, int64_t rows,
@@ -848,20 +819,7 @@
     if (row >= rows) return;
     const double *src = M + row * n_pad;
     double *dst = Mp + row * n_par;
-    const int h = (p + 1) / 2, f = p / 2;
-    for (int e = threadIdx.x & 63; e < h * h * p2; e += 64) {
-        const int i0 = e / (h * p2), i1 = (e - i0 * h * p2) / p2, r = e - (i0 * h + i1) * p2;
-        const int m = (i0 * p + i1) * p2 + r;
-        const int dx = (p - 1 - 2 * i0) * p * p2, dy = (p - 1 - 2 * i1) * p2;
-        const bool cx = i0 >= f, cy = i1 >= f;
-        const double v = src[m], vx = src[m + dx], vy = src[m + dy], vxy = src[m + dx + dy];
-        const double e0 = cx ? v : v + vx, e1 = cx ? vy : vy + vxy, o0 = v - vx, o1 = vy - vxy;
-        const int je = (i0 * h + i1) * p2 + r, jo = (i0 * f + i1) * p2 + r;
-        dst[off.v[0] + je] = cy ? e0 : e0 + e1;
-        if (!cy) dst[off.v[1] + jo] = e0 - e1;
-        if (!cx) dst[off.v[2] + je] = cy ? o0 : o0 + o1;
-        if (!cx && !cy) dst[off.v[3] + jo] = o0 - o1;
-    }
+    m2l_parity2_row(src, dst, off, p, p2, threadIdx.x & 63);
 }
 
 void launch_m2l_parity2(const double *M, int n_pad, double *Mp, int n_par, M2lParityOffsets off, int p, int p2, int64_t rows,
@@ -869,6 +827,22 @@
     if (rows <= 0) return;
     hipLaunchKernelGGL(m2l_parity2_kernel, dim3(static_cast<unsigned>((rows + 3) / 4)), dim3(256), 0, s, M, n_pad, Mp, n_par, off, p, p2,
                        rows);
+}
+
+__global__ __launch_bounds__(256) void m2l_parity_cells_kernel(const double *__restrict__ M, int n_pad, double *__restrict__ Mp,
+                                                               M2lParityRowArgs par, const int32_t *__restrict__ cells, int n_cells,
+                                                               int K, int64_t C) {
+    const int64_t job = static_cast<int64_t>(blockIdx.x) * 4 + (threadIdx.x >> 6);
+    if (job >= static_cast<int64_t>(K) * n_cells) return;
+    const int64_t row = (job / n_cells) * C + cells[job % n_cells];
+    m2l_parity_row_any(par, M + row * n_pad, Mp + row * par.n_par, threadIdx.x & 63);
+}
+
+void launch_m2l_parity_cells(const double *M, int n_pad, double *Mp, const M2lParityRowArgs &par, const int32_t *cells, int n_cells,
+                             int K, int64_t C, hipStream_t s) {
+    if (n_cells <= 0 || K <= 0) return;
+    hipLaunchKernelGGL(m2l_parity_cells_kernel, dim3(static_cast<unsigned>((static_cast<int64_t>(K) * n_cells + 3) / 4)), dim3(256), 0, s, M,
+                       n_pad, Mp, par, cells, n_cells, K, C);
 }
 
 __global__ __launch_bounds__(256) void m2l_zero_segments_kernel(const int32_t *__restrict__ segs, int64_t n_segs,
diff --git a/ferreus_rbf_rs_amd/csrc/device_transfer.hip b/ferreus_rbf_rs_amd/csrc/device_transfer.hip
--- a/ferreus_rbf_rs_amd/csrc/device_transfer.hip
+++ b/ferreus_rbf_rs_amd/csrc/device_transfer.hip
@@ -1,4 +1,5 @@
 #include "device_common.hpp"
+#include "m2l_basis_rows.hpp"
 
 namespace bbfmm {
 
@@ -110,7 +111,7 @@
 }
 
 template <int P, bool FORWARD>
-__device__ inline void transfer3_wave(const double *__restrict__ in, double *buf, const double *__restrict__ xfer,
+__device__ __forceinline__ void transfer3_wave(const double *__restrict__ in, double *buf, const double *__restrict__ xfer,
                                       int oct, int lane) {
     constexpr int PP = P * P, NPEN = (PP + 63) / 64;
     const double *x0 = xfer + ((oct >> 0) & 1) * PP, *x1 = xfer + ((oct >> 1) & 1) * PP,
@@ -159,13 +160,16 @@
 
 constexpr int XFER_WAVES = 4;
 
-template <int P>
+template <int P, int UNP>
 __global__ __launch_bounds__(64 * XFER_WAVES) void l2l3_kernel(const DevCheb *__restrict__ chp, int K, int64_t C,
                                                                const int32_t *__restrict__ cells, int n_cells,
                                                                const int32_t *__restrict__ parent,
                                                                const int32_t *__restrict__ octant,
                                                                const uint8_t *__restrict__ active,
-                                                               double *__restrict__ L) {
+                                                               double *__restrict__ L, M2lUnparityRowArgs unp,
+                                                               const double *__restrict__ Lp,
+                                                               const uint8_t *__restrict__ has_m2l,
+                                                               const uint8_t *__restrict__ has_x) {
     constexpr int N = P * P * P;
     __shared__ double s_buf[XFER_WAVES][N];
     const int wave = threadIdx.x >> 6, lane = threadIdx.x & 63;
@@ -177,20 +181,50 @@
     if (Pc < 0) return;
     const int oct = __builtin_amdgcn_readfirstlane(octant[c]);
     const int n_pad = chp->n_pad;
+    bool hm = false, hx = false;
+    if constexpr (UNP != 0) {
+        hm = __builtin_amdgcn_readfirstlane((int)has_m2l[c]) != 0;
+        hx = __builtin_amdgcn_readfirstlane((int)has_x[c]) != 0;
+    }
     for (int k = 0; k < K; ++k) {
         transfer3_wave<P, false>(L + ((int64_t)k * C + Pc) * n_pad, s_buf[wave], chp->xfer, oct, lane);
         double *Lc = L + ((int64_t)k * C + c) * n_pad;
-        for (int I = lane; I < N; I += 64) Lc[I] += s_buf[wave][I];
+        if constexpr (UNP != 0) {
+            const double *tr = s_buf[wave];
+            const double *src = Lp + ((int64_t)k * C + c) * unp.n_par;
+            const auto add = [&](int m, double v) { Lc[m] = (v + (hx ? Lc[m] : 0.0)) + tr[m]; };
+            if (hm && UNP == 2) m2l_unparity2_row(src, unp.plan, P, P, lane, add);
+            else if (hm) m2l_unparity_row(src, unp.ne16, unp.n_e, unp.n_o, P, P * P, lane, add);
+            else
+                for (int I = lane; I < N; I += 64) Lc[I] = (0.0 + (hx ? Lc[I] : 0.0)) + tr[I];
+        } else {
+            for (int I = lane; I < N; I += 64) Lc[I] += s_buf[wave][I];
+        }
         __builtin_amdgcn_wave_barrier();
     }
 }
 
-template <int P>
+__global__ __launch_bounds__(256) void zero_rows_kernel(const int32_t *__restrict__ cells, int n_cells, int n_pad, int K, int64_t C,
+                                                        double *__restrict__ L) {
+    const int64_t job = static_cast<int64_t>(blockIdx.x) * 4 + (threadIdx.x >> 6);
+    if (job >= static_cast<int64_t>(K) * n_cells) return;
+    double *row = L + ((job / n_cells) * C + cells[job % n_cells]) * n_pad;
+    for (int j = threadIdx.x & 63; j < n_pad; j += 64) row[j] = 0.0;
+}
+
+void launch_zero_rows(const int32_t *cells, int n_cells, int n_pad, int K, int64_t C, double *L, hipStream_t s) {
+    if (n_cells <= 0 || K <= 0) return;
+    hipLaunchKernelGGL(zero_rows_kernel, dim3(static_cast<unsigned>((static_cast<int64_t>(K) * n_cells + 3) / 4)), dim3(256), 0, s, cells,
+                       n_cells, n_pad, K, C, L);
+}
+
+template <int P, bool PAR>
 __global__ __launch_bounds__(512) void m2m3_kernel(const DevCheb *__restrict__ chp, int K, int64_t C,
                                                    const int32_t *__restrict__ parents,
                                                    const int64_t *__restrict__ child_ptr,
                                                    const int32_t *__restrict__ child_idx,
-                                                   const int32_t *__restrict__ octant, double *__restrict__ M) {
+                                                   const int32_t *__restrict__ octant, double *__restrict__ M,
+                                                   M2lParityRowArgs par, double *__restrict__ Mpar) {
     constexpr int N = P * P * P;
     __shared__ double s_buf[8][N];
     const int wave = threadIdx.x >> 6, lane = threadIdx.x & 63;
@@ -202,7 +236,13 @@
         if (wave < n_ch) {
             const int ch = __builtin_amdgcn_readfirstlane(child_idx[c0 + wave]);
             const int oct = __builtin_amdgcn_readfirstlane(octant[ch]);
-            transfer3_wave<P, true>(M + ((int64_t)k * C + ch) * n_pad, s_buf[wave], chp->xfer, oct, lane);
+            const double *Mc = M + ((int64_t)k * C + ch) * n_pad;
+            if constexpr (PAR) {
+                double *dst = Mpar + ((int64_t)k * C + ch) * par.n_par;
+                if (par.axes == 2) m2l_parity2_row(Mc, dst, par.off, P, P, lane);
+                else m2l_parity_row(Mc, dst, par.ne16, par.n_e, par.n_o, P, P * P, lane);
+            }
+            transfer3_wave<P, true>(Mc, s_buf[wave], chp->xfer, oct, lane);
         }
         __syncthreads();
         double *Mp = M + ((int64_t)k * C + Pc) * n_pad;
@@ -215,12 +255,20 @@
     }
 }
 
+bool m2m_writes_parity(const ChebRef &ch) { return ch.d == 3 && ch.p >= 2 && ch.p <= 10; }
+bool l2l_reads_parity(const ChebRef &ch) { return ch.d == 3 && ch.p >= 2 && ch.p <= 12; }
+
 int launch_m2m(const ChebRef &ch, int K, int64_t C, const int32_t *parents, int n_parents, const int64_t *child_ptr,
-               const int32_t *child_idx, const int32_t *octant, double *M, hipStream_t s) {
+               const int32_t *child_idx, const int32_t *octant, double *M, hipStream_t s, const M2lParityRowArgs *par, double *Mp) {
     if (n_parents == 0) return 0;
+    if (par && (!Mp || !m2m_writes_parity(ch))) return static_cast<int>(hipErrorInvalidValue);
     if (ch.d == 3 && dispatch_order<2, 10>(ch.p, [&](auto pc) {
-            hipLaunchKernelGGL((m2m3_kernel<decltype(pc)::value>), dim3(n_parents), dim3(512), 0, s, ch.dev, K, C, parents, child_ptr,
-                               child_idx, octant, M);
+            if (par)
+                hipLaunchKernelGGL((m2m3_kernel<decltype(pc)::value, true>), dim3(n_parents), dim3(512), 0, s, ch.dev, K, C, parents,
+                                   child_ptr, child_idx, octant, M, *par, Mp);
+            else
+                hipLaunchKernelGGL((m2m3_kernel<decltype(pc)::value, false>), dim3(n_parents), dim3(512), 0, s, ch.dev, K, C, parents,
+                                   child_ptr, child_idx, octant, M, M2lParityRowArgs{}, nullptr);
         }))
         return 0;
     const size_t lds = sizeof(double) * (3 * (size_t)ch.n + 2 * ch.p * ch.p);
@@ -232,11 +280,21 @@
 }
 
 int launch_l2l(const ChebRef &ch, int K, int64_t C, const int32_t *cells, int n_cells, const int32_t *parent,
-               const int32_t *octant, const uint8_t *active, double *L, hipStream_t s) {
+               const int32_t *octant, const uint8_t *active, double *L, hipStream_t s, const M2lUnparityRowArgs *unp, const double *Lp,
+               const uint8_t *has_m2l, const uint8_t *has_x) {
     if (n_cells == 0) return 0;
+    if (unp && (!Lp || !has_m2l || !has_x || !l2l_reads_parity(ch))) return static_cast<int>(hipErrorInvalidValue);
     if (ch.d == 3 && dispatch_order<2, 12>(ch.p, [&](auto pc) {
-            hipLaunchKernelGGL((l2l3_kernel<decltype(pc)::value>), dim3((n_cells + XFER_WAVES - 1) / XFER_WAVES), dim3(64 * XFER_WAVES),
-                               0, s, ch.dev, K, C, cells, n_cells, parent, octant, active, L);
+            const dim3 grid((n_cells + XFER_WAVES - 1) / XFER_WAVES), block(64 * XFER_WAVES);
+            if (unp && unp->axes == 2)
+                hipLaunchKernelGGL((l2l3_kernel<decltype(pc)::value, 2>), grid, block, 0, s, ch.dev, K, C, cells, n_cells, parent, octant,
+                                   active, L, *unp, Lp, has_m2l, has_x);
+            else if (unp)
+                hipLaunchKernelGGL((l2l3_kernel<decltype(pc)::value, 1>), grid, block, 0, s, ch.dev, K, C, cells, n_cells, parent, octant,
+                                   active, L, *unp, Lp, has_m2l, has_x);
+            else
+                hipLaunchKernelGGL((l2l3_kernel<decltype(pc)::value, 0>), grid, block, 0, s, ch.dev, K, C, cells, n_cells, parent, octant,
+                                   active, L, M2lUnparityRowArgs{}, nullptr, nullptr, nullptr);
         }))
         return 0;
     const size_t lds = sizeof(double) * (2 * (size_t)ch.n + 2 * ch.p * ch.p);
diff --git a/ferreus_rbf_rs_amd/csrc/fmm_tree.cpp b/ferreus_rbf_rs_amd/csrc/fmm_tree.cpp
--- a/ferreus_rbf_rs_amd/csrc/fmm_tree.cpp
+++ b/ferreus_rbf_rs_amd/csrc/fmm_tree.cpp
@@ -572,7 +572,68 @@
     CHK(dupload(&d_m2l_qlist_, m2l_qlist_h_));
     std::vector<uint8_t> act(static_cast<size_t>(C), 1);
     CHK(dupload(&d_active_, act));
-    return BBFMM_OK;
+    {
+        const char *e = std::getenv("BBFMM_FUSED_PASSES");
+        fused_mask_ = e ? static_cast<unsigned>(std::atoi(e)) & 15u : 15u;
+        if (!(fused_mask_ & 2u)) fused_mask_ &= ~4u;
+        std::vector<uint8_t> has_m2l(static_cast<size_t>(C), 0), has_x(static_cast<size_t>(C), 0);
+        fused_flags_ok_ = true;
+        for (const M2lTileDesc &td : m2l_tiles2_h_) {
+            const size_t lc = static_cast<size_t>(td.level_class);
+            const HostM2lClass &h = lc < m2l_host_.size() ? m2l_host_[lc] : m2l_variants_[lc - m2l_host_.size()];
+            if (td.pad != 0 || td.first < 0 || static_cast<size_t>(td.first) + td.count > h.cells.size()) {
+                fused_flags_ok_ = false;
+                break;
+            }
+            for (int32_t q = 0; q < td.count; ++q) has_m2l[static_cast<size_t>(h.cells[static_cast<size_t>(td.first + q)])] = 1;
+        }
+        for (int32_t c : x_cells_) has_x[static_cast<size_t>(c)] = 1;
+        CHK(dupload(&d_has_m2l_, has_m2l));
+        CHK(dupload(&d_has_x_, has_x));
+        std::vector<int32_t> top;
+        for (size_t l = 0; l < level_cells_.size() && l < 2; ++l) top.insert(top.end(), level_cells_[l].begin(), level_cells_[l].end());
+        n_top_cells_ = static_cast<int>(top.size());
+        CHK(dupload(&d_top_cells_, top));
+    }
+    return BBFMM_OK;
+}
+
+M2lParityRowArgs FmmTree::mp_row_args() const {
+    M2lParityRowArgs a;
+    a.axes = m2l_axes_;
+    a.n_par = m2l_npar_;
+    a.p = ops_.p;
+    a.ne16 = m2l_ne16_;
+    a.n_e = m2l_ne_;
+    a.n_o = m2l_no_;
+    a.p1 = m2l_ne_ / ((ops_.p + 1) / 2);
+    a.off = m2l_s1_off_;
+    a.p2 = ops_.n / (ops_.p * ops_.p);
+    return a;
+}
+
+M2lUnparityRowArgs FmmTree::lp_row_args() const {
+    M2lUnparityRowArgs a;
+    a.axes = m2l_s2_axes_;
+    a.n_par = m2l_s2_plan_.n_par();
+    a.p = ops_.p;
+    a.ne16 = m2l_s2_plan_.ne16();
+    a.n_e = m2l_ne_;
+    a.n_o = m2l_no_;
+    a.p1 = m2l_ne_ / ((ops_.p + 1) / 2);
+    a.plan = m2l_s2_plan_;
+    a.p2 = ops_.n / (ops_.p * ops_.p);
+    return a;
+}
+
+bool FmmTree::m2m_fusable() const {
+    return (fused_mask_ & 1u) && m2l_pairs_ && !m2l_batches_.empty() && !shared_basis_ && ops_.d == 3 && ops_.p == cheb_.p &&
+           m2m_writes_parity(cheb_);
+}
+
+bool FmmTree::l2l_fusable(int k) const {
+    return (fused_mask_ & 2u) && fused_flags_ok_ && m2l_pairs2_ && !m2l_batches_.empty() && !shared_basis_ && ops_.d == 3 &&
+           ops_.p == cheb_.p && l2l_reads_parity(cheb_) && k <= m2l_rhs_chunk_;
 }
 
 int FmmTree::ensure_rhs_capacity(int k) {
@@ -593,6 +654,7 @@
     if (m2l_pairs_) {
         dfree(&d_Mp_);
         CHK(dalloc(&d_Mp_, static_cast<size_t>(k) * C * m2l_npar_, true));
+        mp_current_k_ = 0;
     }
     if (shared_basis_) {
         dfree(&d_Mc_);
@@ -833,6 +895,9 @@
     const HostTree &t = tree_;
     const int64_t C = t.n_cells();
     const bool part = dp && dp->restrict_upward;
+    mp_current_k_ = 0;
+    const bool fuse_mp = !dp && m2m_fusable();
+    const M2lParityRowArgs mp_args = mp_row_args();
     multipoles_partial_ = part;
     phase_begin();
     if (part) {
@@ -851,8 +916,13 @@
         const int rc = part ? launch_m2m(cheb_, k, C, dp->d_up_parents[level].p, static_cast<int>(dp->up_parents_h[level].size()),
                                          dp->d_part_child_ptr.p, dp->d_part_child_idx.p, d_octant_.p, d_M_.p, stream_)
                             : launch_m2m(cheb_, k, C, d_m2m_parents_[level].p, static_cast<int>(m2m_parents_[level].size()),
-                                         d_child_ptr_.p, d_child_idx_.p, d_octant_.p, d_M_.p, stream_);
+                                         d_child_ptr_.p, d_child_idx_.p, d_octant_.p, d_M_.p, stream_, fuse_mp ? &mp_args : nullptr,
+                                         fuse_mp ? d_Mp_.p : nullptr);
         if (rc != 0) return hip_fail(static_cast<hipError_t>(rc), "M2M: dynamic LDS attribute");
+    }
+    if (fuse_mp) {
+        launch_m2l_parity_cells(d_M_.p, cheb_.n_pad, d_Mp_.p, mp_args, d_top_cells_.p, n_top_cells_, k, C, stream_);
+        mp_current_k_ = k;
     }
     phase_end(kPhM2M);
     HIPCHK(hipGetLastError());
@@ -868,13 +938,14 @@
     const HostTree &t = tree_;
     const int64_t C = t.n_cells();
     have_locals_ = false;
+    lp_pending_ = false;
     const bool s2_pairs = m2l_pairs2_ && !m2l_batches_.empty();
     const int lp_len = m2l_s2_plan_.n_par();
     if (!s2_pairs) HIPCHK(hipMemsetAsync(d_L_.p, 0, static_cast<size_t>(k) * C * cheb_.n_pad * sizeof(double), stream_));
     const int m2l_len = shared_basis_ ? basis_pad_ : cheb_.n_pad;
     const double *m_in = shared_basis_ ? d_Mc_.p : m2l_pairs_ ? d_Mp_.p : d_M_.p;
     const int s1_len = m2l_pairs_ ? m2l_npar_ : m2l_len, s1_ne16 = m2l_pairs_ ? m2l_ne16_ : 0;
-    if (m2l_pairs_ && !m2l_batches_.empty()) {
+    if (m2l_pairs_ && !m2l_batches_.empty() && mp_current_k_ < k) {
         phase_begin();
         if (m2l_axes_ == 2)
             launch_m2l_parity2(d_M_.p, cheb_.n_pad, d_Mp_.p, m2l_npar_, m2l_s1_off_, ops_.p, ops_.n / (ops_.p * ops_.p), static_cast<int64_t>(k) * C, stream_);
@@ -890,11 +961,18 @@
         phase_end(kPhM2L1);
     }
     const int nb = static_cast<int>(m2l_batches_.size());
+    const bool fuse_lp = s2_pairs && !dp && l2l_fusable(k);
+    bool clear_lp = true;
+    if (fuse_lp && (fused_mask_ & 4u)) {
+        clear_lp = false;
+        for (const M2lBatch &mb : m2l_batches_)
+            if (mb.t2_count > 0 && m2l_s2_pairs_ksplit(mb.t2_count, m2l_s2_plan_, k, !deterministic_) > 1) clear_lp = true;
+    }
     for (int k0 = 0; k0 < k; k0 += m2l_rhs_chunk_) {
         const int kb = std::min(m2l_rhs_chunk_, k - k0);
         const double *m_chunk = m_in + static_cast<size_t>(k0) * C * s1_len;
         double *l_chunk = s2_pairs ? d_Lp_.p : l_out + static_cast<size_t>(k0) * C * m2l_len;
-        if (s2_pairs) HIPCHK(hipMemsetAsync(d_Lp_.p, 0, static_cast<size_t>(kb) * C * lp_len * sizeof(double), stream_));
+        if (s2_pairs && clear_lp) HIPCHK(hipMemsetAsync(d_Lp_.p, 0, static_cast<size_t>(kb) * C * lp_len * sizeof(double), stream_));
         for (int b = 0; b < nb; ++b) {
             const M2lBatch &mb = m2l_batches_[static_cast<size_t>(b)];
             const int t1_first = dp ? dp->batch_t1[4 * b] : mb.t1_first, t1_count = dp ? dp->batch_t1[4 * b + 1] : mb.t1_count;
@@ -928,7 +1006,9 @@
                                   cbuf_batch_len_, d_m2l_qlist_.p, l_chunk, stream_, !deterministic_);
             phase_end(kPhM2L2);
         }
-        if (s2_pairs) {
+        if (fuse_lp) {
+            lp_pending_ = true;
+        } else if (s2_pairs) {
             phase_begin();
             if (m2l_s2_axes_ == 2)
                 launch_m2l_unparity2(d_Lp_.p, m2l_s2_plan_, d_L_.p + static_cast<size_t>(k0) * C * cheb_.n_pad, ops_.n, cheb_.n_pad, ops_.p,
@@ -952,7 +1032,11 @@
 int FmmTree::downward_tail(int k, const DownwardPlan *dp, const TargetSet *wx) {
     const HostTree &t = tree_;
     const int64_t C = t.n_cells();
-    phase_begin();
+    const bool fuse_lp = lp_pending_ && !dp;
+    lp_pending_ = false;
+    const M2lUnparityRowArgs lp_args = lp_row_args();
+    phase_begin();
+    if (fuse_lp && t.adaptive) launch_zero_rows(d_x_cells_.p, static_cast<int>(x_cells_.size()), cheb_.n_pad, k, C, d_L_.p, stream_);
     if (t.adaptive && wx) {
         launch_wx_sym(kernel_, cheb_, wx->n_wx_jobs, wx->wx_tb.p, wx->wx_te.p, wx->wx_range.p, wx->n_wxl_jobs, wx->wxl_tb.p, wx->wxl_te.p,
                       wx->wxl_range.p, d_w_idx_.p, d_centers_.p,
@@ -971,7 +1055,8 @@
     phase_begin();
     for (int level = 2; level <= t.depth; ++level) {
         const int rc = launch_l2l(cheb_, k, C, d_level_cells_[level].p, static_cast<int>(level_cells_[level].size()), d_parent_.p,
-                                  d_octant_.p, dp ? dp->d_active.p : d_active_.p, d_L_.p, stream_);
+                                  d_octant_.p, dp ? dp->d_active.p : d_active_.p, d_L_.p, stream_, fuse_lp ? &lp_args : nullptr,
+                                  fuse_lp ? d_Lp_.p : nullptr, fuse_lp ? d_has_m2l_.p : nullptr, fuse_lp ? d_has_x_.p : nullptr);
         if (rc != 0) return hip_fail(static_cast<hipError_t>(rc), "L2L: dynamic LDS attribute");
     }
     phase_end(kPhL2L);
@@ -1032,12 +1117,12 @@
     return BBFMM_OK;
 }
 
-int FmmTree::leaf_pass_far(const TargetSet &ts, int k, bool with_grads) {
+int FmmTree::leaf_pass_far(const TargetSet &ts, int k, bool with_grads, double *user_out, int64_t ldo) {
     const int64_t C = tree_.n_cells();
     double *grad = with_grads ? ts.grad.p : nullptr;
     phase_begin();
     launch_l2p(cheb_, ts.n_jobs, ts.job_cell.p, ts.tgt_begin.p, ts.tgt_end.p, d_centers_.p, d_lengths_.p, ts.xyz_ptr,
-               ts.m, k, C, d_L_.p, ts.out.p, grad, stream_);
+               ts.m, k, C, d_L_.p, ts.out.p, grad, stream_, user_out ? ts.perm.p : nullptr, user_out, ldo);
     phase_end(kPhL2P);
     HIPCHK(hipGetLastError());
     return BBFMM_OK;
@@ -1121,10 +1206,13 @@
             if (wx) HIPCHK(hipMemsetAsync(ts.out.p, 0, static_cast<size_t>(k) * ts.m * sizeof(double), stream_));
             CHK(downward_tail(k, nullptr, wx ? &ts : nullptr));
             CHK(leaf_pass_near(ts, k, false, stream_, 3, wx));
-            CHK(leaf_pass_far(ts, k, false));
-            phase_begin();
-            launch_scatter_output(ts.out.p, ts.m, k, ts.perm.p, d_out_.p, N, 0, stream_);
-            phase_end(kPhScatter);
+            const bool l2p_scatters = (fused_mask_ & 8u) != 0;
+            CHK(leaf_pass_far(ts, k, false, l2p_scatters ? d_out_.p : nullptr, N));
+            if (!l2p_scatters) {
+                phase_begin();
+                launch_scatter_output(ts.out.p, ts.m, k, ts.perm.p, d_out_.p, N, 0, stream_);
+                phase_end(kPhScatter);
+            }
             HIPCHK(hipGetLastError());
             double *pin_out = h_pin_ + static_cast<size_t>(k) * N;
             const auto t_queued = std::chrono::steady_clock::now();
@@ -1332,10 +1420,13 @@
     if (wx) HIPCHK(hipMemsetAsync(ts.out.p, 0, static_cast<size_t>(k) * ts.m * sizeof(double), stream_));
     CHK(downward(k, plan, wx ? &ts : nullptr));
     CHK(leaf_pass_near(ts, k, false, stream_, 3, wx));
-    CHK(leaf_pass_far(ts, k, false));
-    phase_begin();
-    launch_scatter_output(ts.out.p, ts.m, k, ts.perm.p, d_out, ldo, 0, stream_);
-    phase_end(kPhScatter);
+    const bool l2p_scatters = (fused_mask_ & 8u) != 0 && !have_part_;
+    CHK(leaf_pass_far(ts, k, false, l2p_scatters ? d_out : nullptr, ldo));
+    if (!l2p_scatters) {
+        phase_begin();
+        launch_scatter_output(ts.out.p, ts.m, k, ts.perm.p, d_out, ldo, 0, stream_);
+        phase_end(kPhScatter);
+    }
     HIPCHK(hipGetLastError());
     if (sync) HIPCHK(hipStreamSynchronize(stream_));
     return BBFMM_OK;
@@ -1393,6 +1484,7 @@
         HIPCHK(hipStreamWaitEvent(stream_, ev_comm_, 0));
     }
     phase_begin();
+    mp_current_k_ = 0;
     if (cnt > 0)
         HIPCHK(hipMemcpyAsync(d_M_.p, d_coarse, static_cast<size_t>(cnt) * sizeof(double), hipMemcpyDeviceToDevice, stream_));
     phase_end(kPhM2M);
@@ -1420,6 +1512,7 @@
         HIPCHK(hipEventRecord(ev_comm_, comm_stream));
         HIPCHK(hipStreamWaitEvent(stream_, ev_comm_, 0));
     }
+    mp_current_k_ = 0;
     phase_begin();
     for (int j = 0; j < k && cnt > 0; ++j)
         HIPCHK(hipMemcpyAsync(d_M_.p + static_cast<size_t>(j) * C * cheb_.n_pad, d_coarse + static_cast<size_t>(j) * cnt,
@@ -1664,6 +1757,11 @@
     const int64_t C = tree_.n_cells();
     const int n = ops_.n, n_pad = cheb_.n_pad;
     HIPCHK(hipStreamSynchronize(stream_));
+    if (which == 'P' || which == 'p') {
+        if (!m2l_pairs_ || !d_Mp_.p) return fail(BBFMM_BAD_ARGUMENT, "no multipoles in the parity basis on this handle");
+        HIPCHK(hipMemcpy(out, d_Mp_.p, static_cast<size_t>(k) * C * m2l_npar_ * sizeof(double), hipMemcpyDeviceToHost));
+        return BBFMM_OK;
+    }
     HIPCHK(hipMemcpy2D(out, n * sizeof(double), src, n_pad * sizeof(double), n * sizeof(double),
                        static_cast<size_t>(k) * C, hipMemcpyDeviceToHost));
     return BBFMM_OK;
diff --git a/ferreus_rbf_rs_amd/csrc/fmm_tree.hpp b/ferreus_rbf_rs_amd/csrc/fmm_tree.hpp
--- a/ferreus_rbf_rs_amd/csrc/fmm_tree.hpp
+++ b/ferreus_rbf_rs_amd/csrc/fmm_tree.hpp
@@ -212,6 +212,7 @@
     int debug_m2l_s2_last_ksplit() const { return m2l_s2_last_ksplit_; }
     int debug_apply_m2l_tables_host(const double *M, double *L) const;
     int debug_get_coefficients(char which, int k, double *out);
+    int debug_m2l_parity_len() const { return m2l_pairs_ ? m2l_npar_ : 0; }
     int debug_partition_upward_counts(int64_t *counts_out, uint8_t *reads_out, int64_t *info_out) const;
 
   private:
@@ -230,7 +231,7 @@
     int leaf_pass(const TargetSet &ts, int k, bool with_grads, bool fixed_plan = false);
     int leaf_pass_near(const TargetSet &ts, int k, bool with_grads, hipStream_t st, int parts, bool wx_done = false,
                        bool fixed_plan = false);
-    int leaf_pass_far(const TargetSet &ts, int k, bool with_grads);
+    int leaf_pass_far(const TargetSet &ts, int k, bool with_grads, double *user_out = nullptr, int64_t ldo = 0);
     int build_target_set(const double *x, int64_t m, int64_t ldx, TargetSet *ts, int64_t *bad_point_index,
                          std::vector<int32_t> *leaves_out = nullptr);
     int build_target_set_device(const double *x, int64_t m, int64_t ldx, TargetSet *ts, int64_t *bad_point_index,
@@ -320,6 +321,17 @@
     std::vector<int32_t> m2l_s2_node_;
     std::vector<int8_t> m2l_s2_sign_;
     std::vector<int8_t> m2l_s2_part_;
+    unsigned fused_mask_ = 15;
+    int mp_current_k_ = 0;
+    bool lp_pending_ = false;
+    bool fused_flags_ok_ = false;
+    M2lParityRowArgs mp_row_args() const;
+    M2lUnparityRowArgs lp_row_args() const;
+    bool m2m_fusable() const;
+    bool l2l_fusable(int k) const;
+    DevBuf<uint8_t> d_has_m2l_, d_has_x_;
+    DevBuf<int32_t> d_top_cells_;
+    int n_top_cells_ = 0;
     int part_rank_ = 0, part_world_ = 1;
     std::vector<int64_t> part_rows_, part_bounds_;
     int partition_finish_core(const double *d_coarse, hipStream_t comm_stream, int *k_out);
diff --git a/ferreus_rbf_rs_amd/csrc/m2l_basis_rows.hpp b/ferreus_rbf_rs_amd/csrc/m2l_basis_rows.hpp
--- /dev/null
+++ b/ferreus_rbf_rs_amd/csrc/m2l_basis_rows.hpp
@@ -0,0 +1,101 @@
+#pragma once
+#include "device.hpp"
+
+namespace bbfmm {
+
+__device__ __forceinline__ void m2l_parity_row(const double *src, double *dst, int ne16, int n_e, int n_o, int p, int p1, int lane) {
+    for (int j = lane; j < n_e; j += 64) {
+        const double v = src[j];
+        if (j < n_o) {
+            const double w = src[j + (p - 1 - 2 * (j / p1)) * p1];
+            dst[j] = v + w;
+            dst[ne16 + j] = v - w;
+        } else {
+            dst[j] = v;
+        }
+    }
+}
+
+__device__ __forceinline__ void m2l_parity2_row(const double *src, double *dst, const M2lParityOffsets &off, int p, int p2, int lane) {
+    const int h = (p + 1) / 2, f = p / 2;
+    for (int e = lane; e < h * h * p2; e += 64) {
+        const int i0 = e / (h * p2), i1 = (e - i0 * h * p2) / p2, r = e - (i0 * h + i1) * p2;
+        const int m = (i0 * p + i1) * p2 + r;
+        const int dx = (p - 1 - 2 * i0) * p * p2, dy = (p - 1 - 2 * i1) * p2;
+        const bool cx = i0 >= f, cy = i1 >= f;
+        const double v = src[m], vx = src[m + dx], vy = src[m + dy], vxy = src[m + dx + dy];
+        const double e0 = cx ? v : v + vx, e1 = cx ? vy : vy + vxy, o0 = v - vx, o1 = vy - vxy;
+        const int je = (i0 * h + i1) * p2 + r, jo = (i0 * f + i1) * p2 + r;
+        dst[off.v[0] + je] = cy ? e0 : e0 + e1;
+        if (!cy) dst[off.v[1] + jo] = e0 - e1;
+        if (!cx) dst[off.v[2] + je] = cy ? o0 : o0 + o1;
+        if (!cx && !cy) dst[off.v[3] + jo] = o0 - o1;
+    }
+}
+
+__device__ __forceinline__ void m2l_parity_row_any(const M2lParityRowArgs &a, const double *src, double *dst, int lane) {
+    if (a.axes == 2) m2l_parity2_row(src, dst, a.off, a.p, a.p2, lane);
+    else m2l_parity_row(src, dst, a.ne16, a.n_e, a.n_o, a.p, a.p1, lane);
+}
+
+__device__ __forceinline__ void m2l_unparity_load(const double *src, int ne16, int n_o, int j, double &e, double &o) {
+    e = src[j];
+    o = j < n_o ? src[ne16 + j] : 0.0;
+}
+
+template <class Emit>
+__device__ __forceinline__ void m2l_unparity_emit(int n_o, int p, int p1, int j, double e, double o, Emit &&emit) {
+    if (j < n_o) {
+        emit(j, e + o);
+        emit(j + (p - 1 - 2 * (j / p1)) * p1, e - o);
+    } else {
+        emit(j, e);
+    }
+}
+
+template <class Emit>
+__device__ __forceinline__ void m2l_unparity_row(const double *src, int ne16, int n_e, int n_o, int p, int p1, int lane, Emit &&emit) {
+    for (int j = lane; j < n_e; j += 64) {
+        double e, o;
+        m2l_unparity_load(src, ne16, n_o, j, e, o);
+        m2l_unparity_emit(n_o, p, p1, j, e, o, emit);
+    }
+}
+
+__device__ __forceinline__ void m2l_unparity2_load(const double *src, const M2lS2PairsPlan &plan, int p, int p2, int e, double (&v)[4]) {
+    const int h = (p + 1) / 2, f = p / 2;
+    const int i0 = e / (h * p2), i1 = (e - i0 * h * p2) / p2, r = e - (i0 * h + i1) * p2;
+    const bool cx = i0 >= f, cy = i1 >= f;
+    const int je = (i0 * h + i1) * p2 + r, jo = (i0 * f + i1) * p2 + r;
+    v[0] = src[plan.col(0, je)];
+    v[1] = cy ? 0.0 : src[plan.col(1, jo)];
+    v[2] = cx ? 0.0 : src[plan.col(2, je)];
+    v[3] = cx || cy ? 0.0 : src[plan.col(3, jo)];
+}
+
+template <class Emit>
+__device__ __forceinline__ void m2l_unparity2_emit(int p, int p2, int e, const double (&v)[4], Emit &&emit) {
+    const int h = (p + 1) / 2, f = p / 2;
+    const int i0 = e / (h * p2), i1 = (e - i0 * h * p2) / p2, r = e - (i0 * h + i1) * p2;
+    const int m = (i0 * p + i1) * p2 + r;
+    const int dx = (p - 1 - 2 * i0) * p * p2, dy = (p - 1 - 2 * i1) * p2;
+    const bool cx = i0 >= f, cy = i1 >= f;
+    const double ee = v[0], eo = v[1], oe = v[2], oo = v[3];
+    const double a = cy ? ee : ee + eo, b = ee - eo, c = cy ? oe : oe + oo, d = oe - oo;
+    emit(m, cx ? a : a + c);
+    if (!cx) emit(m + dx, a - c);
+    if (!cy) emit(m + dy, cx ? b : b + d);
+    if (!cx && !cy) emit(m + dx + dy, b - d);
+}
+
+template <class Emit>
+__device__ __forceinline__ void m2l_unparity2_row(const double *src, const M2lS2PairsPlan &plan, int p, int p2, int lane, Emit &&emit) {
+    const int h = (p + 1) / 2;
+    for (int e = lane; e < h * h * p2; e += 64) {
+        double v[4];
+        m2l_unparity2_load(src, plan, p, p2, e, v);
+        m2l_unparity2_emit(p, p2, e, v, emit);
+    }
+}
+
+}
diff --git a/ferreus_rbf_rs_amd/fmm_tree.py b/ferreus_rbf_rs_amd/fmm_tree.py
--- a/ferreus_rbf_rs_amd/fmm_tree.py
+++ b/ferreus_rbf_rs_amd/fmm_tree.py
@@ -542,7 +542,12 @@
 
     def debug_get_coefficients(self, which: str, k: int) -> np.ndarray:
         s = self.stats()
-        out = np.zeros((k, s.n_cells, s.n_nodes))
+        n = s.n_nodes
+        if which in ("P", "p"):
+            ln = ctypes.c_int32(0)
+            self._raise(self._lib.bbfmm_debug_m2l_parity_len(self._h, ctypes.byref(ln)))
+            n = ln.value
+        out = np.zeros((k, s.n_cells, n))
         self._raise(self._lib.bbfmm_debug_get_coefficients(self._h, which.encode()[0:1], k,
                                                            out.ctypes.data))
         return out
diff --git a/include/ferreus_bbfmm_hip.h b/include/ferreus_bbfmm_hip.h
--- a/include/ferreus_bbfmm_hip.h
+++ b/include/ferreus_bbfmm_hip.h
@@ -324,6 +324,7 @@
 int bbfmm_debug_reference_vectors(const bbfmm_handle *h, int32_t *out, int32_t *n_ref_out);
 
 int bbfmm_debug_get_coefficients(bbfmm_handle *h, char which, int32_t k, double *out);
+int bbfmm_debug_m2l_parity_len(const bbfmm_handle *h, int32_t *len);
 
 
 typedef int (*bbfmm_apply_fn)(void *user, const double *x, double *y, int64_t n);
```

After: 33.70 matvecs/s, median of 6. 2.6% higher.
